# espresso3389/MioTTS-llama.cpp

Measured on AMD Instinct MI355X. Metric: realtime factor (audio s / wall s) + stage ms llm/codec/istft, 1.7B Q4_K_M, higher is better.
Workload: dtype int8-dot (q4_K/q6_K x q8_K) + f32/f16 codec; 1 GPU; MioTTS-1.7B Q4_K_M single utterance, 700 speech tokens -> MioCodec -> iSTFT (28.0 s audio each) per GPU; model=MioTTS-1.7B Q4_K_M, global_batch=1, seq_len=700, parallelism=utterance-sharded x1 (no collective), devices_visible=1

## Files before the change

### miotts-llama.cpp_amd/csrc/hip/llm_attention.h

```cpp
#pragma once
#include "llm_device.h"

namespace mio {
namespace {

__device__ inline float load_resid(const float *x, int lo, int hi) {
    const int lane = threadIdx.x & 63;
    return lo + lane < hi ? x[lo + lane] : 0.0f;
}
__device__ inline float lane_value(float v, int i) {
    return __int_as_float(__builtin_amdgcn_readlane(__float_as_int(v), i));
}

template <int HD, int G, bool DG, bool WQ = false>
__device__ __forceinline__ bool attention_wg(const LlmDims &d, const float *q_norm, const float *k_norm,
                                             const float *bqkv, _Float16 *kc, _Float16 *vc, const LlmBuffers &b,
                                             int ch, int kvh, int pos, int *rdy) {
    static_assert(!WQ || MIO_ATT_MFMA, "the q|k|v wait is on the MFMA attention path");
    constexpr bool kDiag = DG;
    using C = AttCfg<HD>;
    constexpr int PER = HD / 64;
    __shared__ float qs[G][HD];
    __shared__ float knew[HD], vnew[HD];
#if MIO_ATT_MFMA
    using A = AttM<HD>;
    static_assert(C::NT == A::NT, "attention workgroup size");
    __shared__ __attribute__((aligned(16))) char img[2 * A::IMG];
    __shared__ __attribute__((aligned(16))) _Float16 qh[G][HD];
#else
    __shared__ float wres[C::NW][G][HD + 2];
#endif

    const int t0 = ch * ATT_CHUNK;
    if (t0 > pos || b.st->done) return false;
    const int lane = threadIdx.x & 63, wave = threadIdx.x >> 6;
    const float2 *rope = b.rope + (size_t)pos * (HD / 2);
    const bool owner = pos < t0 + ATT_CHUNK;
    auto head_src = [&](int hh, HeadIn<HD> &in) {
        const bool isk = hh == G;
        const size_t so = isk ? (size_t)(d.n_head + kvh) * HD : (size_t)(kvh * G + hh) * HD;
        const size_t vo = (size_t)(d.n_head + d.n_kv + kvh) * HD;
        head_load<HD, WQ ? 16 : 0>(b.qkv + so, bqkv ? bqkv + so : nullptr, isk ? k_norm : q_norm, rope, d, in,
                                   isk ? b.qkv + vo : nullptr, isk && bqkv ? bqkv + vo : nullptr);
    };
    HeadIn<HD> hin;
#if MIO_ATT_MFMA
    h8 kr[A::VI], vr[A::VI];
    if constexpr (WQ) {
        kv_issue<HD>(kc + (size_t)kvh * d.n_ctx * HD, vc + (size_t)kvh * d.n_ctx * HD, t0, pos, kr, vr);
        kv_stage<HD>(kr, vr, owner ? pos - t0 : -1, img, img + A::IMG);
        MIO_TL_MARK(b, 4);
        if (MIO_TIDX == 0)
            wait_count(b.att_cnt + kQkvOff + kQkvStride * kvh, (G + 2) * HD, b.att_cnt + kRdyFlag);
        asm volatile("s_barrier" ::: "memory");
        MIO_TL_MARK(b, 3);
        if (wave < G + (owner ? 1 : 0)) head_src(wave, hin);
    } else {
        if (wave < G + (owner ? 1 : 0)) head_src(wave, hin);
        kv_issue<HD>(kc + (size_t)kvh * d.n_ctx * HD, vc + (size_t)kvh * d.n_ctx * HD, t0, pos, kr, vr);
    }
#else
    if (wave < G + (owner ? 1 : 0)) head_src(wave, hin);
    h8 kr[C::IT], vr[C::IT];
    load_kv_rows<HD>(kc + (size_t)kvh * d.n_ctx * HD, vc + (size_t)kvh * d.n_ctx * HD, t0, pos, kr, vr);
#endif
    MIO_TRACE(b, 1);
    MIO_TL_MARK1(b);
    for (int hh = wave; hh < G + (owner ? 1 : 0); hh += C::NW) {
        const bool isk = hh == G;
        if (hh != wave) head_src(hh, hin);
        head_prep<HD>(hin, d, isk ? knew : qs[hh]);
        if (isk) {
            _Float16 *kd = kc + ((size_t)kvh * d.n_ctx + pos) * HD;
            _Float16 *vd = vc + ((size_t)kvh * d.n_ctx + pos) * HD;
#pragma unroll
            for (int i = 0; i < PER; ++i) {
                const int p = lane + 64 * i;
                const float vr16 = f16r(hin.vv[i]);
                vnew[p] = vr16;
                kd[p] = (_Float16)knew[p];
                vd[p] = (_Float16)vr16;
            }
#if MIO_ATT_MFMA
            __builtin_amdgcn_wave_barrier();
            __builtin_amdgcn_fence(__ATOMIC_SEQ_CST, "wavefront");
            kv_stage_row<HD>(knew, vnew, pos - t0, img, img + A::IMG);
#endif
        }
#if MIO_ATT_MFMA
        else {
            q_to_f16<HD>(qs[hh], qh[hh]);
        }
#endif
    }
#if MIO_ATT_MFMA
    MIO_TRACE(b, 6);
    if constexpr (!WQ) kv_stage<HD>(kr, vr, owner ? pos - t0 : -1, img, img + A::IMG);
    MIO_TRACE(b, 7);
    lds_barrier();
    MIO_TRACE(b, 2);
    MIO_TL_MARK(b, 2);
    const uint32_t gs = (uint32_t)(d.max_splits * C::REC), head0 = (uint32_t)(kvh * G) * gs;
    attend_chunk_mfma<HD, G>(qh, img, img + A::IMG, t0, pos, d.scale, b.part + head0 + (uint32_t)ch * C::REC, gs,
                             DG ? b.trace : nullptr);
#else
    lds_barrier();
    MIO_TRACE(b, 2);
    MIO_TL_MARK(b, 2);
    if (owner) {
        const int sl = threadIdx.x / C::LP, lp = lane % C::LP, r = pos - t0;
        if (sl == r % C::NS) {
            h8 kn, vn;
#pragma unroll
            for (int i = 0; i < 8; ++i) kn[i] = (_Float16)knew[lp * 8 + i], vn[i] = (_Float16)vnew[lp * 8 + i];
#pragma unroll
            for (int it = 0; it < C::IT; ++it)
                if (it == r / C::NS) kr[it] = kn, vr[it] = vn;
        }
    }
    const uint32_t gs = (uint32_t)(d.max_splits * C::REC), head0 = (uint32_t)(kvh * G) * gs;
    attend_chunk<HD, G>(qs, kr, vr, t0, pos, d.scale, wres, b.part + head0 + (uint32_t)ch * C::REC, gs,
                        DG ? b.trace : nullptr, MIO_TL_DIAGSLOT(b));
#endif
    attn_merge_last<HD, G>(b.part, head0, gs, pos / ATT_CHUNK + 1, b.att_cnt + kvh, b.att + (size_t)kvh * G * HD, -1,
                           {}, 0, rdy, (kDiag && b.tl) ? MIO_TL_SLOT(b) : nullptr);
    return true;
}

__device__ __forceinline__ void signal_two_level(int *arr, int *rdy, int r, int n) {
    if (MIO_TIDX < 64) {
        int last = 0;
        if (MIO_TIDX == 0) {
            const int sh = r & (kFfnShards - 1), n_sh = (n - sh + kFfnShards - 1) / kFfnShards;
            last = __hip_atomic_fetch_add((__attribute__((address_space(1))) int *)(arr + kFfnStride * sh), 1,
                                          __ATOMIC_RELAXED, __HIP_MEMORY_SCOPE_AGENT) == n_sh - 1;
        }
        if (__builtin_amdgcn_readfirstlane(last) && MIO_TIDX < kFfnShards)
            __hip_atomic_fetch_add((__attribute__((address_space(1))) int *)(rdy + kFfnStride * MIO_TIDX), 1,
                                   __ATOMIC_RELAXED, __HIP_MEMORY_SCOPE_AGENT);
    }
}
__device__ __forceinline__ void wait_two_level(int *rdy, int r, int n, int *flag) {
    if (MIO_TIDX == 0) wait_count(rdy + kFfnStride * (r & (kFfnShards - 1)), min(n, kFfnShards), flag);
    asm volatile("s_barrier" ::: "memory");
}

__device__ __forceinline__ float load_resid_sc1(const float *x, int lo, int hi) {
    const int lane = threadIdx.x & 63;
    return __uint_as_float(
        __builtin_amdgcn_raw_buffer_load_b32(rsrc(x, (uint32_t)hi * 4u), (uint32_t)(lo + lane) * 4u, 0, 16));
}

template <int NP, int T, int SU, bool DG, bool XS = false>
__device__ __forceinline__ void o_consumer(const LlmDims &d, const QMat &wo, const LlmBuffers &b, int ob, int no) {
    constexpr bool kDiag = DG;
    extern __shared__ __attribute__((aligned(16))) char smem[];
    const int K = wo.k;
    const Smem s = carve(smem, K);
    int lo, hi;
    wave_range(wo.rows, lo, hi, ob, no);
    const float xres = load_resid(b.x, lo, hi);
    Frag ga[Cfg<NP, SU>::U], gb[Cfg<NP, SU>::U];
    load_first<T, NP, 1, SU, MIO_SMALL_AUX>(wo, wo, lo, hi, ga, gb);
    if (MIO_TIDX == 0)
        wait_count(b.att_cnt + kRdyOff + kRdyStride * (blockIdx.x & (kRdyShards - 1)), d.n_kv, b.att_cnt + kRdyFlag);
    asm volatile("s_barrier" ::: "memory");
    MIO_TL_MARK(b, 3);
    XRegs<NP> xr;
    load_x<NP, 16>(b.att, nullptr, K, xr);
    x_after_weights(xr);
    MIO_TL_MARK1(b);
    plain_quant(xr, K, akind(T), s, MIO_TL_DIAGSLOT(b));
    MIO_TL_MARK(b, 2);
    stream_rows<T, NP, 1, SU, MIO_SMALL_AUX>(wo, wo, lo, hi, ga, gb, s.a, [&](int row, float v, float) {
        const float r = lane_value(xres, row - lo);
        if ((threadIdx.x & 63) == 0) {
            if constexpr (XS)
                st1_sc1(b.x, (uint32_t)row * 4u, v + r);
            else
                b.x[row] = v + r;
        }
    });
    if constexpr (XS) {
        asm volatile("s_waitcnt vmcnt(0)" ::: "memory");
        __syncthreads();
        MIO_TL_MARK(b, 6);
        signal_two_level(b.att_cnt + kXOff, b.att_cnt + kXRdy, ob, no);
    }
}

}
}
```

### miotts-llama.cpp_amd/csrc/hip/llm_attn_in.hip

```cpp
#include "llm_device.h"

#pragma clang fp contract(off)

namespace mio {
namespace {

template <int NP, int TQ, int TV, int SU, bool DG, bool FS>
__global__ __launch_bounds__(MT) void k_attn_in(LlmDims d, const float *norm_w, QMat wq, QMat wk, QMat wv,
                                                int g_qk, LlmBuffers b, QMat emb, int nblk) {
    constexpr bool kDiag = DG;
    const int o1 = wq.rows, o2 = wq.rows + wk.rows;
    const int GW = matvec_grid_n(d.n_wg, o2 + wv.rows);
    extern __shared__ __attribute__((aligned(16))) char smem[];
    __shared__ float rs_[MW];
    __shared__ int ri_[MW];
    const int K = d.n_embd;
    const Smem s = carve(smem, K);
    MIO_TRACE(b, 0);
    MIO_TL_BEGIN(b);
    if (blockIdx.x == 2 && MIO_TIDX < 2 * kFfnShards)
        __hip_atomic_store((__attribute__((address_space(1))) int *)(b.att_cnt + kFfnOff + kFfnStride * MIO_TIDX), 0,
                           __ATOMIC_RELAXED, __HIP_MEMORY_SCOPE_AGENT);
    int pend = 0, step = 0;
    if constexpr (FS) {
        pend = b.st->pending;
        step = b.st->step;
        if (b.st->done) return;
    }
    uint32_t dn = 0;
    if constexpr (!FS) dn = done_issue(b);
    XRegs<NP> xr;
    load_x(pend ? nullptr : b.x, norm_w, K, xr);
    x_gate();
    auto sample_prologue = [&]() -> bool {
        if constexpr (FS) {
            if (pend) {
                const SampleCfg sc = *b.cfg;
                const int tok = sample_token<MT>(b.smp, nblk, sc, step, rs_, ri_);
                embed_regs(emb, tok, K, xr);
                if (blockIdx.x == 0) {
#pragma unroll
                    for (int i = 0; i < NP; ++i) {
                        const int e = (MIO_TIDX + i * MT) * 4;
                        if (e < K) *reinterpret_cast<float4 *>(b.x + e) = xr.v[i];
                    }
                    if (MIO_TIDX == 0) {
                        if (step < sc.max_steps) sc.out_tokens[step] = tok;
                        if (tok == sc.eos0 || tok == sc.eos1) b.st->done = 1, signal_host_done(sc);
                        b.st->token = tok;
                    }
                }
                return tok == sc.eos0 || tok == sc.eos1;
            }
        }
        return false;
    };
    auto put = [&](int row, float v) {
        if ((threadIdx.x & 63) == 0) b.qkv[row] = v;
    };
    Frag ga[Cfg<NP, SU>::U], gb[Cfg<NP, SU>::U];
    int lo, hi;
    if ((int)blockIdx.x < g_qk) {
        wave_range(o2, lo, hi, blockIdx.x, g_qk);
        load_first<TQ, NP, 1, SU, MIO_SMALL_AUX>(wq, wk, lo, hi, ga, gb, o1);
        if (sample_prologue()) return;
        x_after_weights(xr);
        if (!FS && done_now(dn)) return;
        MIO_TRACE(b, 1);
        MIO_TL_MARK1(b);
        rmsnorm_quant(xr, K, d.eps, akind(TQ), s, MIO_TL_DIAGSLOT(b));
        MIO_TRACE(b, 2);
        MIO_TL_MARK(b, 2);
        stream_rows<TQ, NP, 1, SU, MIO_SMALL_AUX>(wq, wk, lo, hi, ga, gb, s.a, [&](int row, float v, float) {
            put(row, v);
        }, o1);
        MIO_TL_END(b);
        MIO_TRACE(b, 15);
    } else {
        const int bv = (int)blockIdx.x - g_qk, gv = GW - g_qk;
        wave_range(wv.rows, lo, hi, bv, gv);
        load_first<TV, NP, 1, SU, MIO_SMALL_AUX>(wv, wv, lo, hi, ga, gb);
        if (sample_prologue()) return;
        x_after_weights(xr);
        if (!FS && done_now(dn)) return;
        rmsnorm_quant(xr, K, d.eps, akind(TV), s, MIO_TL_DIAGSLOT(b));
        stream_rows<TV, NP, 1, SU, MIO_SMALL_AUX>(wv, wv, lo, hi, ga, gb, s.a, [&](int row, float v, float) {
            put(o2 + row, v);
        });
        MIO_TL_END(b);
    }
}

template <bool DG>
void launch(const LlmDims &d, const LayerW &L, int il, const QMat &tok_embd, const LlmBuffers &b, hipStream_t s) {
    int GW, g_qk;
    attn_in_grid(d, L, GW, g_qk);
    const size_t lds = matvec_lds(d.n_embd);
    const int np = pick_np(d.n_embd);
    const int un = std::max(max_wave_units(L.wq.rows + L.wk.rows, g_qk, np, 1),
                            max_wave_units(L.wv.rows, GW - g_qk, np, 1));
    const int nblk = lm_head_blocks(d);
    const int grid = GW;
    dispatch_nt(d.n_embd, L.wq.type, [&]<int NP, int TQ>() {
        auto go = [&]<int TV>() {
            dispatch_su<NP>(pick_su(un, NP), [&]<int SU>() {
                if (il == 0)
                    hipLaunchKernelGGL((k_attn_in<NP, TQ, TV, SU, DG, true>), dim3(grid), dim3(MT), lds, s, d,
                                       L.attn_norm, L.wq, L.wk, L.wv, g_qk, b, tok_embd, nblk);
                else
                    hipLaunchKernelGGL((k_attn_in<NP, TQ, TV, SU, DG, false>), dim3(grid), dim3(MT), lds, s, d,
                                       L.attn_norm, L.wq, L.wk, L.wv, g_qk, b, tok_embd, nblk);
            });
        };
        dispatch_v<TQ>(L.wv.type, go);
    });
}

}

void launch_attn_in(const LlmDims &d, const LayerW &L, int il, const QMat &tok_embd, const LlmBuffers &b, bool dg,
                    hipStream_t s) {
    if (dg)
        launch<true>(d, L, il, tok_embd, b, s);
    else
        launch<false>(d, L, il, tok_embd, b, s);
}

}
```

### miotts-llama.cpp_amd/csrc/hip/llm_device.h

```cpp
#pragma once

#include <cfloat>
#include <climits>
#include <cstdio>
#include <cstdlib>
#include <type_traits>

#include "llm_kernels.h"

#pragma clang fp contract(off)

#ifndef MIO_TIDX
#define MIO_TIDX threadIdx.x
#endif

namespace mio {
namespace {
constexpr bool kDiag = true;
#define MIO_TRACE(bufs, k)                                                                    \
    do {                                                                                      \
        if (kDiag && (bufs).trace && blockIdx.x == 0 && blockIdx.y == 0 && MIO_TIDX == 0) { \
            asm volatile("" ::: "memory");                                                    \
            (bufs).trace[k] = __builtin_readcyclecounter();                                   \
            if ((k) == 0 || (k) == 15) (bufs).trace[16 + (k)] = __builtin_amdgcn_s_memrealtime(); \
        }                                                                                     \
    } while (0)

#define MIO_TL_SLOT(bufs) ((bufs).tl + 8 * ((size_t)(bufs).seq * kTlSlots + ((blockIdx.x + blockIdx.y * gridDim.x) & (kTlSlots - 1))))
#define MIO_TL_AT(bufs, k)                                                                      \
    do {                                                                                        \
        if (kDiag && (bufs).tl && MIO_TIDX == 0) MIO_TL_SLOT(bufs)[k] = __builtin_amdgcn_s_memrealtime(); \
    } while (0)
#ifdef MIO_TL_DIAG
#define MIO_TL_BEGIN(bufs)                                                                     \
    do {                                                                                       \
        MIO_TL_AT(bufs, 0);                                                                    \
        if (kDiag && (bufs).tl && MIO_TIDX == blockDim.x - 64) MIO_TL_SLOT(bufs)[6] = __builtin_amdgcn_s_memrealtime(); \
    } while (0)
#else
#define MIO_TL_BEGIN(bufs) MIO_TL_AT(bufs, 0)
#endif
#ifdef MIO_TL_WAVES
#define MIO_TL_MARK(bufs, k)
#define MIO_TL_END(bufs)
#else
#define MIO_TL_MARK(bufs, k) MIO_TL_AT(bufs, k)
#define MIO_TL_END(bufs) MIO_TL_AT(bufs, 7)
#endif
#ifndef MIO_DIAG_WAVE
#define MIO_DIAG_WAVE 7
#endif
#ifdef MIO_TL_DIAG
#define MIO_TL_DIAGSLOT(bufs) ((kDiag && (bufs).tl) ? MIO_TL_SLOT(bufs) : nullptr)
#define MIO_TL_MARK1(bufs)
#else
#define MIO_TL_DIAGSLOT(bufs) nullptr
#define MIO_TL_MARK1(bufs) MIO_TL_MARK(bufs, 1)
#endif
#ifdef MIO_TL_WAVES
#define MIO_DIAG_STAMP(diag, k, v)
#else
#define MIO_DIAG_STAMP(diag, k, v)                                                   \
    do {                                                                             \
        if ((diag) && MIO_TIDX == 0) {                                            \
            asm volatile("" ::"v"(v));                                               \
            (diag)[k] = __builtin_amdgcn_s_memrealtime();                            \
        }                                                                            \
    } while (0)
#endif

constexpr int NT = 256;
constexpr int NWAVE = NT / 64;
constexpr int MT = 512;
constexpr int MW = MT / 64;
constexpr int ATT_CHUNK = kAttChunk;
__host__ __device__ constexpr int part_rec(int hd) { return hd + 4; }

__device__ __forceinline__ float h2f(uint32_t bits16) {
    const uint16_t b = (uint16_t)bits16;
    return (float)__builtin_bit_cast(_Float16, b);
}
__device__ __forceinline__ float f16r(float f) { return (float)(_Float16)f; }
__device__ __forceinline__ int sdot4(int a, int b, int c) { return __builtin_amdgcn_sdot4(a, b, c, false); }
__device__ __forceinline__ uint4 ld16(const uint8_t *p) { return *reinterpret_cast<const uint4 *>(p); }
typedef uint32_t u32x4 __attribute__((ext_vector_type(4)));

__device__ __forceinline__ void lds_barrier() { asm volatile("s_waitcnt lgkmcnt(0)\n\ts_barrier" ::: "memory"); }

template <int CTRL, int RM = 0xF>
__device__ __forceinline__ int dpp_i(int v) {
    return __builtin_amdgcn_update_dpp(0, v, CTRL, RM, 0xF, false);
}
template <int CTRL, int RM = 0xF>
__device__ __forceinline__ float dpp_f(float v) {
    return __int_as_float(__builtin_amdgcn_update_dpp(0, __float_as_int(v), CTRL, RM, 0xF, false));
}
constexpr int ROW_SHR1 = 0x111, ROW_SHR2 = 0x112, ROW_SHR4 = 0x114, ROW_SHR8 = 0x118;
constexpr int ROW_BCAST15 = 0x142, ROW_BCAST31 = 0x143;

__device__ __forceinline__ float wave_max_f(float v, float id) {
    v = fmaxf(v, __int_as_float(__builtin_amdgcn_update_dpp(__float_as_int(id), __float_as_int(v), ROW_SHR1, 0xF, 0xF, false)));
    v = fmaxf(v, __int_as_float(__builtin_amdgcn_update_dpp(__float_as_int(id), __float_as_int(v), ROW_SHR2, 0xF, 0xF, false)));
    v = fmaxf(v, __int_as_float(__builtin_amdgcn_update_dpp(__float_as_int(id), __float_as_int(v), ROW_SHR4, 0xF, 0xF, false)));
    v = fmaxf(v, __int_as_float(__builtin_amdgcn_update_dpp(__float_as_int(id), __float_as_int(v), ROW_SHR8, 0xF, 0xF, false)));
    v = fmaxf(v, __int_as_float(__builtin_amdgcn_update_dpp(__float_as_int(id), __float_as_int(v), ROW_BCAST15, 0xA, 0xF, false)));
    v = fmaxf(v, __int_as_float(__builtin_amdgcn_update_dpp(__float_as_int(id), __float_as_int(v), ROW_BCAST31, 0xC, 0xF, false)));
    return __int_as_float(__builtin_amdgcn_readlane(__float_as_int(v), 63));
}
__device__ __forceinline__ int wave_min_i(int v) {
    const int id = INT_MAX;
    v = min(v, __builtin_amdgcn_update_dpp(id, v, ROW_SHR1, 0xF, 0xF, false));
    v = min(v, __builtin_amdgcn_update_dpp(id, v, ROW_SHR2, 0xF, 0xF, false));
    v = min(v, __builtin_amdgcn_update_dpp(id, v, ROW_SHR4, 0xF, 0xF, false));
    v = min(v, __builtin_amdgcn_update_dpp(id, v, ROW_SHR8, 0xF, 0xF, false));
    v = min(v, __builtin_amdgcn_update_dpp(id, v, ROW_BCAST15, 0xA, 0xF, false));
    v = min(v, __builtin_amdgcn_update_dpp(id, v, ROW_BCAST31, 0xC, 0xF, false));
    return __builtin_amdgcn_readlane(v, 63);
}
template <int CTRL, int RM = 0xF>
__device__ __forceinline__ double dpp_d(double v) {
    const int2 p = __builtin_bit_cast(int2, v);
    int2 r;
    r.x = __builtin_amdgcn_update_dpp(0, p.x, CTRL, RM, 0xF, false);
    r.y = __builtin_amdgcn_update_dpp(0, p.y, CTRL, RM, 0xF, false);
    return __builtin_bit_cast(double, r);
}
__device__ __forceinline__ double wave_sum_d(double v) {
    v += dpp_d<ROW_SHR1>(v);
    v += dpp_d<ROW_SHR2>(v);
    v += dpp_d<ROW_SHR4>(v);
    v += dpp_d<ROW_SHR8>(v);
    v += dpp_d<ROW_BCAST15, 0xA>(v);
    v += dpp_d<ROW_BCAST31, 0xC>(v);
    const int2 p = __builtin_bit_cast(int2, v);
    int2 r;
    r.x = __builtin_amdgcn_readlane(p.x, 63);
    r.y = __builtin_amdgcn_readlane(p.y, 63);
    return __builtin_bit_cast(double, r);
}
__device__ __forceinline__ float group8_max(float v) {
    v = fmaxf(v, dpp_f<0xB1>(v));
    v = fmaxf(v, dpp_f<0x4E>(v));
    v = fmaxf(v, dpp_f<0x141>(v));
    return v;
}
__device__ __forceinline__ int quad_sum_i(int v) {
    v += dpp_i<0xB1>(v);
    v += dpp_i<0x4E>(v);
    return v;
}

struct ActL {
    int8_t *qs;
    float *d;
    int16_t *bs;
};

struct Smem {
    ActL a;
    double *red;
};

__host__ __device__ inline size_t smem_bytes(int K) {
    return (size_t)K * 2 + (size_t)(K / 32 + 8) * 4 + (size_t)(K / 16 + 8) * 2 + 128;
}

__device__ inline Smem carve(char *base, int K) {
    Smem s;
    s.a.qs = (int8_t *)base;
    s.a.d = (float *)(base + (size_t)K * 2);
    s.a.bs = (int16_t *)(base + (size_t)K * 2 + (size_t)(K / 32 + 8) * 4);
    s.red = (double *)(base + smem_bytes(K) - 128);
    return s;
}

__host__ __device__ inline size_t act_bytes(int K) {
    return ((size_t)K + (size_t)(K / 32 + 8) * 4 + (size_t)(K / 16 + 8) * 2 + 15) & ~(size_t)15;
}
__host__ __device__ inline size_t act_base(int) { return 0; }
__device__ inline Smem carve_t(char *base, int K, int t) {
    Smem s;
    s.red = nullptr;
    char *a = base + act_base(K) + act_bytes(K) * t;
    s.a.qs = (int8_t *)a;
    s.a.d = (float *)(a + K);
    s.a.bs = (int16_t *)(a + K + (size_t)(K / 32 + 8) * 4);
    return s;
}

__device__ double block_sum(double v, double *red) {
    v = wave_sum_d(v);
    if ((MIO_TIDX & 63) == 0) red[MIO_TIDX >> 6] = v;
    lds_barrier();
    double t = 0.0;
#pragma unroll
    for (int w = 0; w < MW; ++w) t += red[w];
    return t;
}

__device__ __forceinline__ void q8k_store(const float (&v)[4], float am, int b, const ActL &a) {
    const int lane = MIO_TIDX & 63;
    int q[4] = {0, 0, 0, 0};
    float dd = 0.0f;
    if (am > 0.0f) {
        float sel = 0.0f;
        bool has = false;
#pragma unroll
        for (int i = 3; i >= 0; --i)
            if (fabsf(v[i]) == am) sel = v[i], has = true;
        const int src = __builtin_ctzll(__ballot(has));
        const float mx = __int_as_float(__builtin_amdgcn_readlane(__float_as_int(sel), src));
        const float iscale = -127.f / mx;
#pragma unroll
        for (int i = 0; i < 4; ++i) {
            const int t = (int)rintf(iscale * v[i]);
            q[i] = t < 127 ? t : 127;
        }
        dd = 1.0f / iscale;
    }
    const int packed = (q[0] & 0xFF) | ((q[1] & 0xFF) << 8) | ((q[2] & 0xFF) << 16) | ((q[3] & 0xFF) << 24);
    *reinterpret_cast<int *>(a.qs + b * 256 + 4 * lane) = packed;
    const int sm = quad_sum_i(q[0] + q[1] + q[2] + q[3]);
    if ((lane & 3) == 0) a.bs[b * 16 + (lane >> 2)] = (int16_t)sm;
    if (lane == 0) a.d[b] = dd;
}
__device__ __forceinline__ float abs_max4(const float (&v)[4]) {
    return wave_max_f(fmaxf(fmaxf(fabsf(v[0]), fabsf(v[1])), fmaxf(fabsf(v[2]), fabsf(v[3]))), 0.0f);
}

__device__ __forceinline__ void q80_store(const float (&v)[4], int b, bool ok, const ActL &a) {
    const int lane = MIO_TIDX & 63;
    float am = 0.0f;
#pragma unroll
    for (int i = 0; i < 4; ++i) am = fmaxf(am, fabsf(v[i]));
    am = group8_max(am);
    const float dd = am / 127.0f;
    const float id = dd != 0.0f ? 1.0f / dd : 0.0f;
    int q[4];
#pragma unroll
    for (int i = 0; i < 4; ++i) q[i] = (int)roundf(v[i] * id);
    if (ok) {
        *reinterpret_cast<int *>(a.qs + b * 32 + 4 * (lane & 7)) =
            (q[0] & 0xFF) | ((q[1] & 0xFF) << 8) | ((q[2] & 0xFF) << 16) | ((q[3] & 0xFF) << 24);
        if ((lane & 7) == 0) a.d[b] = f16r(dd);
    }
}

#ifndef MIO_X_FIRST
#define MIO_X_FIRST 0
#endif
__device__ __forceinline__ void x_gate() {
#if MIO_X_FIRST == 1
    asm volatile("s_waitcnt vmcnt(0)" ::: "memory");
#elif MIO_X_FIRST == 2
    asm volatile("s_barrier" ::: "memory");
#endif
}

template <int XV>
struct XRegs {
    float4 v[XV];
    float4 w[XV];
};

template <int XV>
__device__ __forceinline__ void x_after_weights(XRegs<XV> &xr) {
#pragma unroll
    for (int i = 0; i < XV; ++i)
        asm volatile("" : "+v"(xr.v[i].x), "+v"(xr.v[i].y), "+v"(xr.v[i].z), "+v"(xr.v[i].w), "+v"(xr.w[i].x),
                     "+v"(xr.w[i].y), "+v"(xr.w[i].z), "+v"(xr.w[i].w));
}

template <int XV, int XAUX = 0>
__device__ inline void load_x(const float *x, const float *w, int K, XRegs<XV> &xr) {
    const auto rx = __builtin_amdgcn_make_buffer_rsrc(const_cast<float *>(x), 0, x ? K * 4 : 0, 0x00020000);
    const auto rw = __builtin_amdgcn_make_buffer_rsrc(const_cast<float *>(w), 0, w ? K * 4 : 0, 0x00020000);
#pragma unroll
    for (int i = 0; i < XV; ++i) {
        const int e = (MIO_TIDX + i * MT) * 4;
        const u32x4 a = __builtin_amdgcn_raw_buffer_load_b128(rx, e * 4, 0, XAUX);
        const u32x4 c = __builtin_amdgcn_raw_buffer_load_b128(rw, e * 4, 0, 0);
        xr.v[i] = make_float4(__uint_as_float(a.x), __uint_as_float(a.y), __uint_as_float(a.z), __uint_as_float(a.w));
        xr.w[i] = make_float4(__uint_as_float(c.x), __uint_as_float(c.y), __uint_as_float(c.z), __uint_as_float(c.w));
    }
}

__host__ __device__ constexpr int akind(int T) { return T == 30 ? 2 : (T == 8 ? 0 : 1); }

__device__ __forceinline__ uint32_t f32_to_bf16(float f) {
    const uint32_t u = __float_as_uint(f);
    if ((u & 0x7fffffffu) > 0x7f800000u) return (u >> 16) | 64u;
    return (u + (0x7fffu + ((u >> 16) & 1u))) >> 16;
}

template <int XV>
__device__ __forceinline__ void quant_regs(const float4 (&v)[XV], int K, int ak, const ActL &a) {
    const int lane = MIO_TIDX & 63, wave = __builtin_amdgcn_readfirstlane(MIO_TIDX >> 6);
    if (ak == 1) {
        const int nsb = K >> 8;
#pragma unroll
        for (int j = 0; j < XV; ++j) {
            const int b = wave + MW * j;
            if (b >= nsb) break;
            const float vv[4] = {v[j].x, v[j].y, v[j].z, v[j].w};
            q8k_store(vv, abs_max4(vv), b, a);
        }
    } else if (ak == 2) {
#pragma unroll
        for (int j = 0; j < XV; ++j) {
            const int e = (MIO_TIDX + j * MT) * 4;
            if (e < K)
                *reinterpret_cast<uint2 *>(a.qs + 2 * e) =
                    make_uint2(f32_to_bf16(v[j].x) | (f32_to_bf16(v[j].y) << 16),
                               f32_to_bf16(v[j].z) | (f32_to_bf16(v[j].w) << 16));
        }
    } else {
        const int nb = K / 32;
#pragma unroll
        for (int j = 0; j < XV; ++j) {
            const int b = wave * 8 + MW * 8 * j + (lane >> 3);
            const float vv[4] = {v[j].x, v[j].y, v[j].z, v[j].w};
            q80_store(vv, b, b < nb, a);
        }
    }
    lds_barrier();
}

__device__ __forceinline__ float rms_scale(double tot, int K, float eps) {
    const float mean = (float)((K & (K - 1)) == 0 ? tot * (1.0 / K) : tot / K);
    return 1.0f / sqrtf(mean + eps);
}

template <int XV>
__device__ void rmsnorm_quant(const XRegs<XV> &xr, int K, float eps, int kquant, const Smem &s,
                              unsigned long long *diag = nullptr) {
    double acc = 0.0;
#pragma unroll
    for (int i = 0; i < XV; ++i) {
        const int e = (MIO_TIDX + i * MT) * 4;
        if (e < K) {
            const float4 v = xr.v[i];
            acc += (double)(v.x * v.x);
            acc += (double)(v.y * v.y);
            acc += (double)(v.z * v.z);
            acc += (double)(v.w * v.w);
        }
    }
#ifdef MIO_TL_WAVES
    if (diag && (MIO_TIDX & 63) == 0 && MIO_TIDX > 0) {
        asm volatile("" ::"v"(acc));
        diag[MIO_TIDX >> 6] = __builtin_amdgcn_s_memrealtime();
    }
    if (diag && MIO_TIDX == 0) {
        asm volatile("" ::"v"(acc));
        diag[0] = __builtin_amdgcn_s_memrealtime() - 0;
    }
#else
    MIO_DIAG_STAMP(diag, 3, acc);
    if (diag && MIO_TIDX == MIO_DIAG_WAVE * 64) {
        asm volatile("" ::"v"(acc));
        diag[1] = __builtin_amdgcn_s_memrealtime();
    }
#endif
    const double tot = block_sum(acc, s.red);
    MIO_DIAG_STAMP(diag, 4, tot);
    const float scale = rms_scale(tot, K, eps);
    float4 y[XV];
#pragma unroll
    for (int i = 0; i < XV; ++i) {
        const float4 v = xr.v[i], ww = xr.w[i];
        float t;
        t = v.x * scale, y[i].x = t * ww.x;
        t = v.y * scale, y[i].y = t * ww.y;
        t = v.z * scale, y[i].z = t * ww.z;
        t = v.w * scale, y[i].w = t * ww.w;
    }
    MIO_DIAG_STAMP(diag, 5, scale);
    quant_regs<XV>(y, K, kquant, s.a);
}

template <int XV>
__device__ inline void plain_quant(const XRegs<XV> &xr, int K, int kquant, const Smem &s,
                                   unsigned long long *diag = nullptr) {
    MIO_DIAG_STAMP(diag, 5, 0);
    quant_regs<XV>(xr.v, K, kquant, s.a);
}

struct ConvPrev {
    const float *p;
    int bcx;
};
template <int XV>
struct ConvRegs {
    float4 b[XV], c[XV], x[XV], p1[XV], p2[XV], w[XV][3];
};
__device__ __forceinline__ float4 ld4(const float *p) { return *reinterpret_cast<const float4 *>(p); }
__device__ __forceinline__ float4 mul4(float4 a, float4 b) {
    return make_float4(a.x * b.x, a.y * b.y, a.z * b.z, a.w * b.w);
}
__device__ __forceinline__ float4 conv_prev4(const ConvPrev &pv, int K, int e) {
    if (!pv.p) return make_float4(0.f, 0.f, 0.f, 0.f);
    if (!pv.bcx) return ld4(pv.p + e);
    return mul4(ld4(pv.p + e), ld4(pv.p + 2 * K + e));
}
template <int XV>
__device__ inline void conv_load(const float *bcx, const ConvPrev &p1, const ConvPrev &p2, const float *conv_w, int K,
                                 ConvRegs<XV> &r) {
#pragma unroll
    for (int i = 0; i < XV; ++i) {
        const int e = (MIO_TIDX + i * MT) * 4;
        if (e < K) {
            r.b[i] = ld4(bcx + e), r.c[i] = ld4(bcx + K + e), r.x[i] = ld4(bcx + 2 * K + e);
            r.p1[i] = conv_prev4(p1, K, e), r.p2[i] = conv_prev4(p2, K, e);
#pragma unroll
            for (int j = 0; j < 3; ++j) r.w[i][j] = ld4(conv_w + (size_t)e * kConvL + 4 * j);
        }
    }
}
template <int XV>
__device__ inline void conv_quant(const ConvRegs<XV> &r, int K, int kquant, const Smem &s, float *bx_out,
                                  unsigned long long *diag = nullptr) {
    float4 y[XV];
#pragma unroll
    for (int i = 0; i < XV; ++i) {
        const int e = (MIO_TIDX + i * MT) * 4;
        y[i] = make_float4(0.f, 0.f, 0.f, 0.f);
        if (e < K) {
            const float4 bx = mul4(r.b[i], r.x[i]);
            const float v2[4] = {r.p2[i].x, r.p2[i].y, r.p2[i].z, r.p2[i].w};
            const float v1[4] = {r.p1[i].x, r.p1[i].y, r.p1[i].z, r.p1[i].w};
            const float v0[4] = {bx.x, bx.y, bx.z, bx.w};
            const float c[4] = {r.c[i].x, r.c[i].y, r.c[i].z, r.c[i].w};
            const float w[12] = {r.w[i][0].x, r.w[i][0].y, r.w[i][0].z, r.w[i][0].w, r.w[i][1].x, r.w[i][1].y,
                                 r.w[i][1].z, r.w[i][1].w, r.w[i][2].x, r.w[i][2].y, r.w[i][2].z, r.w[i][2].w};
            float o[4];
#pragma unroll
            for (int j = 0; j < 4; ++j) {
                float acc = 0.0f;
                acc = acc + v2[j] * w[j * 3 + 0];
                acc = acc + v1[j] * w[j * 3 + 1];
                acc = acc + v0[j] * w[j * 3 + 2];
                o[j] = c[j] * acc;
            }
            y[i] = make_float4(o[0], o[1], o[2], o[3]);
            if (bx_out) *reinterpret_cast<float4 *>(bx_out + e) = bx;
        }
    }
    MIO_DIAG_STAMP(diag, 5, 0);
    quant_regs<XV>(y, K, kquant, s.a);
}
template <int XV>
__device__ __forceinline__ void conv_after_weights(ConvRegs<XV> &r) {
#pragma unroll
    for (int i = 0; i < XV; ++i) {
        asm volatile("" : "+v"(r.b[i].x), "+v"(r.b[i].y), "+v"(r.b[i].z), "+v"(r.b[i].w));
        asm volatile("" : "+v"(r.x[i].x), "+v"(r.x[i].y), "+v"(r.x[i].z), "+v"(r.x[i].w));
    }
}

__device__ __forceinline__ int sum8_i(int v) {
    v += dpp_i<ROW_SHR1>(v);
    v += dpp_i<ROW_SHR2>(v);
    v += dpp_i<ROW_SHR4>(v);
    return v;
}
__device__ __forceinline__ float sum8_f(float v) {
    v += dpp_f<ROW_SHR1>(v);
    v += dpp_f<ROW_SHR2>(v);
    v += dpp_f<ROW_SHR4>(v);
    return v;
}
__device__ __forceinline__ float sum_lanes7(float v) {
    v += dpp_f<ROW_SHR8>(v);
    v += dpp_f<ROW_BCAST15, 0xA>(v);
    v += dpp_f<ROW_BCAST31, 0xC>(v);
    return __int_as_float(__builtin_amdgcn_readlane(__float_as_int(v), 63));
}

__device__ inline float wave_sum(float v) {
#pragma unroll
    for (int o = 32; o >= 1; o >>= 1) v += __shfl_xor(v, o);
    return v;
}

constexpr uint32_t M4 = 0x0F0F0F0Fu, M2 = 0x03030303u;

struct Frag {
    uint4 a, b;
    uint32_t c, e;
    uint4 a2, b2;
};

struct ALane {
    int4 lo, hi;
    int b0, b1;
    float d;
    int4 lo2, hi2;
};

__device__ __forceinline__ __amdgpu_buffer_rsrc_t rsrc(const void *p, uint32_t bytes) {
    return __builtin_amdgcn_make_buffer_rsrc(const_cast<void *>(p), 0, (int)min(bytes, 0x7FFFFFF0u), 0x00020000);
}
#ifndef MIO_WEIGHT_AUX
#define MIO_WEIGHT_AUX 2
#endif
#ifndef MIO_LM_AUX
#define MIO_LM_AUX MIO_WEIGHT_AUX
#endif
#ifndef MIO_SMALL_AUX
#define MIO_SMALL_AUX MIO_WEIGHT_AUX
#endif
template <int AUX = MIO_WEIGHT_AUX>
__device__ __forceinline__ uint4 bld16(const uint8_t *base, uint32_t bytes, uint32_t voff, uint32_t soff) {
    const u32x4 v = __builtin_amdgcn_raw_buffer_load_b128(rsrc(base, bytes), voff, soff, AUX);
    return make_uint4(v.x, v.y, v.z, v.w);
}
template <int AUX = MIO_WEIGHT_AUX>
__device__ __forceinline__ uint32_t bld4(const uint8_t *base, uint32_t bytes, uint32_t voff, uint32_t soff) {
    return __builtin_amdgcn_raw_buffer_load_b32(rsrc(base, bytes), voff, soff, AUX);
}
template <int AUX = MIO_WEIGHT_AUX>
__device__ __forceinline__ uint32_t bld2(const uint8_t *base, uint32_t bytes, uint32_t voff, uint32_t soff) {
    return __builtin_amdgcn_raw_buffer_load_b16(rsrc(base, bytes), voff, soff, AUX);
}

template <int T, int AUX = MIO_WEIGHT_AUX>
__device__ __forceinline__ Frag load_frag(const QMat W, int row, int pass) {
    const int lane = MIO_TIDX & 63;
    const uint32_t R = (uint32_t)W.rows,
                   r = (uint32_t)__builtin_amdgcn_readfirstlane(min(max(row, 0), W.rows - 1));
    Frag f;
    if constexpr (T == 12) {
        const int nsb = W.k >> 8, sb = min(pass * 8 + (lane >> 3), nsb - 1), pc = lane & 7;
        const uint32_t qb = (uint32_t)(W.k / 2), hb = (uint32_t)nsb * 16;
        f.a = bld16<AUX>(W.p0, R * qb, sb * 128 + pc * 16, r * qb);
        f.c = bld4<AUX>(W.p1, R * hb, sb * 16 + 4 * (pc & 3), r * hb);
        f.b = make_uint4(0, 0, 0, 0);
        f.e = 0;
    } else if constexpr (T == 13) {
        const int nsb = W.k >> 8, sb = min(pass * 8 + (lane >> 3), nsb - 1), pc = lane & 7;
        const uint32_t qb = (uint32_t)(W.k / 2), fb = (uint32_t)(W.k / 8), hb = (uint32_t)nsb * 16;
        f.a = bld16<AUX>(W.p0, R * qb, sb * 128 + pc * 16, r * qb);
        f.b = bld16<AUX>(W.p1, R * fb, sb * 32 + 16 * (pc & 1), r * fb);
        f.c = bld4<AUX>(W.p2, R * hb, sb * 16 + 4 * (pc & 3), r * hb);
        f.e = 0;
    } else if constexpr (T == 14) {
        const int nsb = W.k >> 8, sb = min(pass * 8 + (lane >> 3), nsb - 1), pc = lane & 7;
        const uint32_t lb = (uint32_t)(W.k / 2), hb = (uint32_t)(W.k / 4), sbb = (uint32_t)(W.k / 16),
                       db = (uint32_t)nsb * 2;
        f.a = bld16<AUX>(W.p0, R * lb, sb * 128 + pc * 16, r * lb);
        f.b = bld16<AUX>(W.p1, R * hb, sb * 64 + 32 * (pc >> 2) + 16 * (pc & 1), r * hb);
        f.c = bld2<AUX>(W.p2, R * sbb, sb * 16 + 2 * pc, r * sbb);
        f.e = bld2<AUX>(W.p3, R * db, sb * 2, r * db);
    } else if constexpr (T == 30) {
        const uint32_t rb = (uint32_t)W.k * 2;
        auto off = [&](int i) { return (uint32_t)min(pass * 2048 + 512 * i + 8 * lane, W.k - 8) * 2u; };
        f.a = bld16<AUX>(W.p0, R * rb, off(0), r * rb);
        f.b = bld16<AUX>(W.p0, R * rb, off(1), r * rb);
        f.a2 = bld16<AUX>(W.p0, R * rb, off(2), r * rb);
        f.b2 = bld16<AUX>(W.p0, R * rb, off(3), r * rb);
        f.c = 0;
        f.e = 0;
    } else {
        const int nb = W.k >> 5, b = min(pass * 64 + lane, nb - 1);
        const uint32_t qb = (uint32_t)W.k, db = (uint32_t)nb * 2;
        f.a = bld16<AUX>(W.p0, R * qb, 32 * b, r * qb);
        f.b = bld16<AUX>(W.p0, R * qb, 32 * b + 16, r * qb);
        f.c = 0;
        f.e = bld2<AUX>(W.p1, R * db, 2 * b, r * db);
    }
    return f;
}

template <int T>
__device__ __forceinline__ ALane load_alane(const ActL &a, int K, int pass) {
    const int lane = MIO_TIDX & 63;
    ALane r;
    if constexpr (T == 12 || T == 13 || T == 14) {
        const int nsb = K >> 8, sb = pass * 8 + (lane >> 3), pc = lane & 7;
        const int sbc = sb < nsb ? sb : 0;
        int e, e2;
        if constexpr (T == 12 || T == 13) {
            e = sbc * 256 + 64 * (pc >> 1) + 16 * (pc & 1);
            e2 = e + 32;
        } else {
            const int n = pc >> 2, qq = pc & 3;
            e = sbc * 256 + 128 * n + 32 * (qq >> 1) + 16 * (qq & 1);
            e2 = e + 64;
        }
        r.lo = *reinterpret_cast<const int4 *>(a.qs + e);
        r.hi = *reinterpret_cast<const int4 *>(a.qs + e2);
        r.b0 = a.bs[e >> 4];
        r.b1 = a.bs[e2 >> 4];
        r.d = a.d[sbc];
    } else if constexpr (T == 30) {
        auto at = [&](int i) {
            const int e = min(pass * 2048 + 512 * i + 8 * lane, K - 8);
            return *reinterpret_cast<const int4 *>(a.qs + 2 * e);
        };
        r.lo = at(0), r.hi = at(1), r.lo2 = at(2), r.hi2 = at(3);
        r.b0 = r.b1 = 0;
        r.d = 0.0f;
    } else {
        const int nb = K >> 5, b = pass * 64 + lane, bc = b < nb ? b : 0;
        r.lo = *reinterpret_cast<const int4 *>(a.qs + 32 * bc);
        r.hi = *reinterpret_cast<const int4 *>(a.qs + 32 * bc + 16);
        r.b0 = r.b1 = 0;
        r.d = a.d[bc];
    }
    return r;
}

template <int T>
__device__ __forceinline__ float dot_frag(const Frag &f, const ALane &al, int K, int pass) {
    const int lane = MIO_TIDX & 63;
    if constexpr (T == 12 || T == 13) {
        const int jj = (lane & 7) >> 1;
        uint4 h;
        h.x = (uint32_t)dpp_i<0x00>((int)f.c);
        h.y = (uint32_t)dpp_i<0x55>((int)f.c);
        h.z = (uint32_t)dpp_i<0xAA>((int)f.c);
        h.w = (uint32_t)dpp_i<0xFF>((int)f.c);
        const uint32_t wlo = jj < 2 ? h.y : (jj == 2 ? h.z : h.w);
        const uint32_t whi = jj < 2 ? h.z : h.w;
        const uint32_t F = __builtin_amdgcn_alignbit(whi, wlo, (24 * jj) & 31);
        const int sc0 = F & 63, m0 = (F >> 6) & 63, sc1 = (F >> 12) & 63, m1 = (F >> 18) & 63;
        auto lo = [&](uint32_t q, uint32_t h) {
            if constexpr (T == 13) return (int)((q & M4) | (((h >> (2 * jj)) & 0x01010101u) << 4));
            else return (int)(q & M4);
        };
        auto hi = [&](uint32_t q, uint32_t h) {
            if constexpr (T == 13) return (int)(((q >> 4) & M4) | (((h >> (2 * jj + 1)) & 0x01010101u) << 4));
            else return (int)((q >> 4) & M4);
        };
        int dlo = 0, dhi = 0;
        dlo = sdot4(lo(f.a.x, f.b.x), al.lo.x, dlo);
        dlo = sdot4(lo(f.a.y, f.b.y), al.lo.y, dlo);
        dlo = sdot4(lo(f.a.z, f.b.z), al.lo.z, dlo);
        dlo = sdot4(lo(f.a.w, f.b.w), al.lo.w, dlo);
        dhi = sdot4(hi(f.a.x, f.b.x), al.hi.x, dhi);
        dhi = sdot4(hi(f.a.y, f.b.y), al.hi.y, dhi);
        dhi = sdot4(hi(f.a.z, f.b.z), al.hi.z, dhi);
        dhi = sdot4(hi(f.a.w, f.b.w), al.hi.w, dhi);
        int isum = __mul24(sc0, dlo) + __mul24(sc1, dhi);
        int imin = __mul24(m0, al.b0) + __mul24(m1, al.b1);
        isum = sum8_i(isum);
        imin = sum8_i(imin);
        const float d = h2f(h.x & 0xFFFF) * al.d;
        const float dmin = h2f(h.x >> 16) * al.d;
        float v = d * (float)isum;
        v = v - dmin * (float)imin;
        return pass * 8 + (lane >> 3) < (K >> 8) ? v : 0.0f;
    } else if constexpr (T == 14) {
        const int shl = 2 * ((lane & 3) >> 1);
        auto lo = [&](uint32_t l, uint32_t h) { return (int)((l & M4) | ((h << (4 - shl)) & 0x30303030u)); };
        auto hi = [&](uint32_t l, uint32_t h) { return (int)(((l >> 4) & M4) | ((h >> shl) & 0x30303030u)); };
        int dlo = 0, dhi = 0;
        dlo = sdot4(lo(f.a.x, f.b.x), al.lo.x, dlo);
        dlo = sdot4(lo(f.a.y, f.b.y), al.lo.y, dlo);
        dlo = sdot4(lo(f.a.z, f.b.z), al.lo.z, dlo);
        dlo = sdot4(lo(f.a.w, f.b.w), al.lo.w, dlo);
        dhi = sdot4(hi(f.a.x, f.b.x), al.hi.x, dhi);
        dhi = sdot4(hi(f.a.y, f.b.y), al.hi.y, dhi);
        dhi = sdot4(hi(f.a.z, f.b.z), al.hi.z, dhi);
        dhi = sdot4(hi(f.a.w, f.b.w), al.hi.w, dhi);
        const int sa = (int)(int8_t)(f.c & 0xFF), sb = (int)(int8_t)(f.c >> 8);
        int isum = __mul24(sa, dlo - 32 * al.b0) + __mul24(sb, dhi - 32 * al.b1);
        isum = sum8_i(isum);
        const float d = h2f(f.e) * al.d;
        const float v = d * (float)isum;
        return pass * 8 + (lane >> 3) < (K >> 8) ? v : 0.0f;
    } else if constexpr (T == 30) {
        typedef __bf16 bf2 __attribute__((ext_vector_type(2)));
        float acc = 0.0f;
        auto dot8 = [&](const uint4 &w, const int4 &x, int i) {
            const bool ok = pass * 2048 + 512 * i + 8 * lane < K;
            const uint4 ww = ok ? w : make_uint4(0, 0, 0, 0);
            const uint4 xx = ok ? make_uint4((uint32_t)x.x, (uint32_t)x.y, (uint32_t)x.z, (uint32_t)x.w)
                                : make_uint4(0, 0, 0, 0);
            acc = __builtin_amdgcn_fdot2_f32_bf16(__builtin_bit_cast(bf2, ww.x), __builtin_bit_cast(bf2, xx.x), acc, false);
            acc = __builtin_amdgcn_fdot2_f32_bf16(__builtin_bit_cast(bf2, ww.y), __builtin_bit_cast(bf2, xx.y), acc, false);
            acc = __builtin_amdgcn_fdot2_f32_bf16(__builtin_bit_cast(bf2, ww.z), __builtin_bit_cast(bf2, xx.z), acc, false);
            acc = __builtin_amdgcn_fdot2_f32_bf16(__builtin_bit_cast(bf2, ww.w), __builtin_bit_cast(bf2, xx.w), acc, false);
        };
        dot8(f.a, al.lo, 0);
        dot8(f.b, al.hi, 1);
        dot8(f.a2, al.lo2, 2);
        dot8(f.b2, al.hi2, 3);
        return acc;
    } else {
        int s = 0;
        s = sdot4((int)f.a.x, al.lo.x, s);
        s = sdot4((int)f.a.y, al.lo.y, s);
        s = sdot4((int)f.a.z, al.lo.z, s);
        s = sdot4((int)f.a.w, al.lo.w, s);
        s = sdot4((int)f.b.x, al.hi.x, s);
        s = sdot4((int)f.b.y, al.hi.y, s);
        s = sdot4((int)f.b.z, al.hi.z, s);
        s = sdot4((int)f.b.w, al.hi.w, s);
        const float v = (float)s * (h2f(f.e) * al.d);
        return pass * 64 + lane < (K >> 5) ? v : 0.0f;
    }
}

template <int T>
__device__ __forceinline__ float row_total(float acc) {
    if constexpr (T == 8 || T == 30) acc = sum8_f(acc);
    return sum_lanes7(acc);
}

template <int NP, int SU = 0>
struct Cfg {
    static constexpr int U = SU ? SU : (NP == 1 ? 4 : 3);
    static constexpr int NG = SU ? 1 : 2;
    static constexpr bool AREG = NP <= 3;
};

template <int T, int NP, int NM, int SU = 0, int AUX = MIO_WEIGHT_AUX>
__device__ __forceinline__ void load_group(const QMat W0, const QMat W1, int lo, int n, int u0,
                                           Frag (&f)[Cfg<NP, SU>::U], int split = INT_MAX) {
#pragma unroll
    for (int j = 0; j < Cfg<NP, SU>::U; ++j) {
        const int u = __builtin_amdgcn_readfirstlane(max(0, min(u0 + j, n - 1)));
        const int p = u % NP, m = (u / NP) % NM, i = u / (NP * NM);
        if constexpr (NM == 1) {
            const int r = __builtin_amdgcn_readfirstlane(lo + i);
            f[j] = load_frag<T, AUX>(r >= split ? W1 : W0, r >= split ? r - split : r, p);
        } else {
            f[j] = load_frag<T, AUX>(m ? W1 : W0, lo + i, p);
        }
    }
}

template <int T, int NP, int NM, int SU = 0, int AUX = MIO_WEIGHT_AUX, class Epi>
__device__ __forceinline__ void stream_rows(const QMat W0, const QMat W1, int lo, int hi, Frag (&A)[Cfg<NP, SU>::U],
                                            Frag (&B)[Cfg<NP, SU>::U], const ActL &a, Epi &&epi, int split = INT_MAX,
                                            unsigned long long *trace = nullptr) {
    constexpr int U = Cfg<NP, SU>::U;
    const int K = W0.k;
    const int n = (hi - lo) * NM * NP;
    if (n <= 0) return;
    ALane al[Cfg<NP, SU>::AREG ? NP : 1];
    if constexpr (Cfg<NP, SU>::AREG) {
#pragma unroll
        for (int p = 0; p < NP; ++p) al[p] = load_alane<T>(a, K, p);
    }
    float acc = 0.0f, g = 0.0f;
    auto consume = [&](const Frag (&F)[U], int u0) {
#pragma unroll
        for (int j = 0; j < U; ++j) {
            const int u = u0 + j;
            if (u < n) {
                int p;
                ALane av;
                if constexpr (NP == 1) {
                    p = 0;
                    av = al[0];
                } else if constexpr (NP == U) {
                    p = j;
                    av = al[j];
                } else {
                    p = u % NP;
                    av = load_alane<T>(a, K, p);
                }
                acc += dot_frag<T>(F[j], av, K, p);
                if (p == NP - 1) {
                    const float v = row_total<T>(acc);
                    acc = 0.0f;
                    const int i = u / (NP * NM);
                    if constexpr (NM == 1) {
                        epi(lo + i, v, 0.0f);
                    } else {
                        if ((u / NP) % NM == 0)
                            g = v;
                        else
                            epi(lo + i, g, v);
                    }
                }
            }
        }
    };
    for (int u0 = 0;;) {
        consume(A, u0);
        if (trace && u0 == 0 && blockIdx.x == 0 && MIO_TIDX == 0) trace[3] = __builtin_readcyclecounter();
        if constexpr (Cfg<NP, SU>::NG == 1) break;
        u0 += U;
        if (u0 >= n) break;
        load_group<T, NP, NM, SU, AUX>(W0, W1, lo, n, u0 + U, A, split);
        consume(B, u0);
        u0 += U;
        if (u0 >= n) break;
        load_group<T, NP, NM, SU, AUX>(W0, W1, lo, n, u0 + U, B, split);
    }
}

template <int T, int NP, int NM, int SU = 0, int AUX = MIO_WEIGHT_AUX>
__device__ __forceinline__ void load_first(const QMat W0, const QMat W1, int lo, int hi, Frag (&A)[Cfg<NP, SU>::U],
                                           Frag (&B)[Cfg<NP, SU>::U], int split = INT_MAX) {
    const int n = (hi - lo) * NM * NP;
    load_group<T, NP, NM, SU, AUX>(W0, W1, lo, n, 0, A, split);
    if constexpr (Cfg<NP, SU>::NG == 2) load_group<T, NP, NM, SU, AUX>(W0, W1, lo, n, Cfg<NP, SU>::U, B, split);
}

__device__ inline void wave_range(int R, int &lo, int &hi, int b, int G) {
    const int w = __builtin_amdgcn_readfirstlane(MIO_TIDX >> 6);
    const int ra = (R * b) / G, rb = (R * (b + 1)) / G;
    lo = ra + (rb - ra) * w / MW;
    hi = ra + (rb - ra) * (w + 1) / MW;
}
__device__ inline void wave_range_n(int R, int &lo, int &hi, int b, int G, int w0, int NW) {
    const int w = __builtin_amdgcn_readfirstlane(MIO_TIDX >> 6) - w0;
    const int ra = (R * b) / G, rb = (R * (b + 1)) / G;
    if (w < 0 || w >= NW) {
        lo = hi = ra;
        return;
    }
    lo = ra + (rb - ra) * w / NW;
    hi = ra + (rb - ra) * (w + 1) / NW;
}
__device__ inline void wave_range(const LlmDims &d, int R, int &lo, int &hi) {
    wave_range(R, lo, hi, blockIdx.x, matvec_grid_n(d.n_wg, R));
}


__device__ float dequant_elem(const QMat &W, int row, int e) {
    if (W.type == 12 || W.type == 13) {
        const int nsb = W.k >> 8, sb = e >> 8, c = e & 255, j = c >> 6, w = c & 63, hi = w >> 5, l = w & 31;
        const uint8_t q = W.p0[(size_t)row * (W.k / 2) + sb * 128 + 32 * j + l];
        const uint8_t *hd = (W.type == 13 ? W.p2 : W.p1) + ((size_t)row * nsb + sb) * 16;
        const uint32_t F = (uint32_t)hd[4 + 3 * j] | ((uint32_t)hd[5 + 3 * j] << 8) | ((uint32_t)hd[6 + 3 * j] << 16);
        const int sc = (F >> (12 * hi)) & 63, m = (F >> (12 * hi + 6)) & 63;
        const float d1 = h2f(hd[0] | (hd[1] << 8)) * sc, m1 = h2f(hd[2] | (hd[3] << 8)) * m;
        int code = hi ? (q >> 4) : (q & 0xF);
        if (W.type == 13) code += ((W.p1[(size_t)row * (W.k / 8) + sb * 32 + l] >> (2 * j + hi)) & 1) << 4;
        return d1 * (float)code - m1;
    } else if (W.type == 14) {
        const int nsb = W.k >> 8, sb = e >> 8, c = e & 255, n = c >> 7, w = c & 127, g = w >> 5, l = w & 31;
        const uint8_t ql = W.p0[(size_t)row * (W.k / 2) + sb * 128 + 64 * n + l + 32 * (g & 1)];
        const uint8_t qh = W.p1[(size_t)row * (W.k / 4) + sb * 64 + 32 * n + l];
        const int q = (int)((g < 2 ? (ql & 0xF) : (ql >> 4)) | (((qh >> (2 * g)) & 3) << 4)) - 32;
        const int is = c >> 4, sn = is >> 3, sw = is & 7;
        const int sc = ((const int8_t *)W.p2)[(size_t)row * (W.k / 16) + sb * 16 + 2 * (4 * sn + (sw & 3)) + (sw >> 2)];
        const float dd = h2f(((const uint16_t *)W.p3)[(size_t)row * nsb + sb]);
        return dd * (float)sc * (float)q;
    } else if (W.type == 30) {
        const uint16_t h = ((const uint16_t *)W.p0)[(size_t)row * W.k + e];
        return __uint_as_float((uint32_t)h << 16);
    } else {
        const int nb = W.k >> 5;
        const int8_t q = ((const int8_t *)W.p0)[(size_t)row * W.k + e];
        return (float)q * h2f(((const uint16_t *)W.p1)[(size_t)row * nb + (e >> 5)]);
    }
}

constexpr int ST = 1024;

__device__ inline void embed_row(const QMat &emb, int tok, int n, float *x) {
    float v[4];
#pragma unroll
    for (int i = 0; i < 4; ++i) {
        const int e = MIO_TIDX + i * ST;
        v[i] = e < n ? dequant_elem(emb, tok, e) : 0.0f;
    }
#pragma unroll
    for (int i = 0; i < 4; ++i) {
        const int e = MIO_TIDX + i * ST;
        if (e < n) x[e] = v[i];
    }
}


inline void attn_in_grid(const LlmDims &d, const LayerW &L, int &G, int &g_qk) {
    const int rows = L.wq.rows + L.wk.rows + L.wv.rows, qk = L.wq.rows + L.wk.rows;
    G = matvec_grid(d, rows);
    g_qk = (G * qk + rows / 2) / rows;
    g_qk = g_qk < 1 ? 1 : (g_qk > G - 1 ? G - 1 : g_qk);
}


template <int LP>
__device__ __forceinline__ float group_sum(float v) {
    v += dpp_f<0xB1>(v);
    v += dpp_f<0x4E>(v);
    v += dpp_f<0x141>(v);
    if constexpr (LP == 16) v += dpp_f<0x140>(v);
    return v;
}

__device__ inline float silu_f(float x) { return x / (1.0f + expf(-x)); }

__device__ inline uint64_t mix64(uint64_t x) {
    x += 0x9E3779B97F4A7C15ull;
    x = (x ^ (x >> 30)) * 0xBF58476D1CE4E5B9ull;
    x = (x ^ (x >> 27)) * 0x94D049BB133111EBull;
    return x ^ (x >> 31);
}

__device__ inline float gumbel(uint64_t seed, int step, int idx) {
    const uint64_t h = mix64(seed ^ mix64(((uint64_t)(uint32_t)step << 32) | (uint32_t)idx));
    const float u = fminf(((float)(h >> 40) + 0.5f) * (1.0f / 16777216.0f), 0x1.fffffep-1f);
    return -logf(-logf(u));
}



__device__ __forceinline__ int cur_pos(const StepState *st, const LlmDims &d) {
    return min(st->pos + st->pending, d.n_ctx - 1);
}

template <class B>
__device__ __forceinline__ uint32_t done_issue(const B &b) {
    return __builtin_amdgcn_raw_buffer_load_b32(rsrc(&b.st->done, 4), 0, 0, 0);
}
__device__ __forceinline__ bool done_now(uint32_t v) { return __builtin_amdgcn_readfirstlane(v) != 0; }
__device__ __forceinline__ void signal_host_done(const SampleCfg &sc) {
    if (sc.host_done) __hip_atomic_store(sc.host_done, 1, __ATOMIC_RELAXED, __HIP_MEMORY_SCOPE_SYSTEM);
}

template <int NTH>
__device__ int sample_token(const float *smp, int nblk, const SampleCfg &sc, int step, float *rs, int *ri) {
    const int tid = MIO_TIDX, lane = tid & 63, wave = tid >> 6;
    float best = -INFINITY;
    int bi = INT_MAX;
    const bool forced = sc.force && step < sc.n_force;
    const int ft = forced ? sc.force[step] : -1;
    for (int i = tid; i < nblk; i += NTH) {
        const float v = smp[2 * i];
        const int ix = __float_as_int(smp[2 * i + 1]);
        if (v > best || (v == best && ix < bi)) best = v, bi = ix;
    }
#pragma unroll
    for (int o = 32; o >= 1; o >>= 1) {
        const float v = __shfl_xor(best, o);
        const int ix = __shfl_xor(bi, o);
        if (v > best || (v == best && ix < bi)) best = v, bi = ix;
    }
    if (lane == 0) rs[wave] = best, ri[wave] = bi;
    lds_barrier();
    best = rs[0], bi = ri[0];
    for (int w = 1; w < NTH / 64; ++w)
        if (rs[w] > best || (rs[w] == best && ri[w] < bi)) best = rs[w], bi = ri[w];
    int tok = bi == INT_MAX ? sc.lo : bi;
    if (ft >= 0) tok = ft;
    return tok;
}

template <int XV>
__device__ inline void embed_regs(const QMat &emb, int tok, int K, XRegs<XV> &xr) {
#pragma unroll
    for (int i = 0; i < XV; ++i) {
        const int e = (MIO_TIDX + i * MT) * 4;
        float v[4] = {0.f, 0.f, 0.f, 0.f};
        if (e < K)
#pragma unroll
            for (int q = 0; q < 4; ++q) v[q] = dequant_elem(emb, tok, e + q);
        xr.v[i] = make_float4(v[0], v[1], v[2], v[3]);
    }
}

[[noreturn]] inline void no_kernel(const char *what, int type, int k) {
    fprintf(stderr, "miotts: no %s kernel for ggml type %d (%d)\n", what, type, k);
    abort();
}

template <bool BF = true, class F>
void dispatch_nt(int K, int type, F &&f) {
    const int np = pick_np(K);
#define NT_CASE(NPV, TV) \
    if (np == NPV && type == TV) return f.template operator()<NPV, TV>();
    NT_CASE(1, 8) NT_CASE(1, 12) NT_CASE(1, 13) NT_CASE(1, 14) NT_CASE(3, 8) NT_CASE(3, 12) NT_CASE(3, 13)
    NT_CASE(3, 14) NT_CASE(6, 8) NT_CASE(6, 12) NT_CASE(6, 13) NT_CASE(6, 14)
    if constexpr (BF) {
        NT_CASE(1, 30) NT_CASE(3, 30) NT_CASE(6, 30)
    }
#undef NT_CASE
    no_kernel("matvec", type, K);
}

template <int TQ, class F>
void dispatch_v(int tv, F &&f) {
    if (tv == TQ) return f.template operator()<TQ>();
    if constexpr (TQ == 12 || TQ == 13) {
        if (tv == 14) return f.template operator()<14>();
    }
    if constexpr (TQ == 14) {
        if (tv == 12) return f.template operator()<12>();
    }
    no_kernel("attn_v beside q|k", tv, TQ);
}


typedef _Float16 h8 __attribute__((ext_vector_type(8)));

#ifndef MIO_ATT_NT
#define MIO_ATT_NT 256
#endif
template <int HD>
struct AttCfg {
    static constexpr int LP = HD / 8;
    static constexpr int NT = ATT_CHUNK * LP < MIO_ATT_NT ? ATT_CHUNK * LP : MIO_ATT_NT;
    static constexpr int NW = NT / 64;
    static constexpr int NS = NT / LP;
    static constexpr int IT = ATT_CHUNK / NS;
    static constexpr int REC = part_rec(HD);
};

__device__ __forceinline__ void st1_sc1(float *base, uint32_t off, float v) {
    __builtin_amdgcn_raw_buffer_store_b32(__float_as_uint(v), rsrc(base, 0x7FFFFFF0u), off, 0, 16);
}
__device__ __forceinline__ void st4_sc1(float *base, uint32_t off, float4 v) {
    u32x4 u;
    u.x = __float_as_uint(v.x), u.y = __float_as_uint(v.y), u.z = __float_as_uint(v.z), u.w = __float_as_uint(v.w);
    __builtin_amdgcn_raw_buffer_store_b128(u, rsrc(base, 0x7FFFFFF0u), off, 0, 16);
}
__device__ __forceinline__ void wait_count(int *c, int target, int *flag) {
    auto *p = (__attribute__((address_space(1))) int *)c;
    auto *f = (__attribute__((address_space(1))) int *)flag;
    for (int it = 0; it < (1 << 16); ++it) {
        if (__hip_atomic_load(p, __ATOMIC_RELAXED, __HIP_MEMORY_SCOPE_AGENT) >= target) return;
        if ((it & 1023) == 1023 && __hip_atomic_load(f, __ATOMIC_RELAXED, __HIP_MEMORY_SCOPE_AGENT)) return;
        __builtin_amdgcn_s_sleep(1);
    }
    __hip_atomic_store(f, 1, __ATOMIC_RELAXED, __HIP_MEMORY_SCOPE_AGENT);
}
__device__ __forceinline__ float4 ld4_sc1(const float *base, uint32_t off) {
    const u32x4 v = __builtin_amdgcn_raw_buffer_load_b128(rsrc(base, 0x7FFFFFF0u), off, 0, 16);
    return make_float4(__uint_as_float(v.x), __uint_as_float(v.y), __uint_as_float(v.z), __uint_as_float(v.w));
}
__device__ __forceinline__ float2 ld2_sc1(const float *base, uint32_t off) {
    const auto v = __builtin_amdgcn_raw_buffer_load_b64(rsrc(base, 0x7FFFFFF0u), off, 0, 16);
    return make_float2(__uint_as_float(v[0]), __uint_as_float(v[1]));
}

__device__ __forceinline__ float4 merge_out4(const float *part, uint32_t head, int nch, int rec, int hd, int dd) {
    float M = -INFINITY, L = 0.0f;
    float4 O = make_float4(0.f, 0.f, 0.f, 0.f);
    constexpr int CB = 8;
    for (int c0 = 0; c0 < nch; c0 += CB) {
        float2 ml[CB];
        float4 oc[CB];
#pragma unroll
        for (int j = 0; j < CB; ++j) {
            const int c = c0 + j;
            if (c < nch) {
                ml[j] = ld2_sc1(part, (head + (uint32_t)(c * rec + hd)) * 4u);
                oc[j] = ld4_sc1(part, (head + (uint32_t)(c * rec + dd)) * 4u);
            } else {
                ml[j] = make_float2(-INFINITY, 0.0f);
                oc[j] = make_float4(0.f, 0.f, 0.f, 0.f);
            }
        }
        float mb = M;
#pragma unroll
        for (int j = 0; j < CB; ++j) mb = fmaxf(mb, ml[j].x);
        const float a = M == -INFINITY ? 0.0f : expf(M - mb);
        L *= a;
        O.x *= a, O.y *= a, O.z *= a, O.w *= a;
#pragma unroll
        for (int j = 0; j < CB; ++j) {
            const float w = c0 + j < nch ? expf(ml[j].x - mb) : 0.0f;
            L += w * ml[j].y;
            O.x += w * oc[j].x, O.y += w * oc[j].y, O.z += w * oc[j].z, O.w += w * oc[j].w;
        }
        M = mb;
    }
    return make_float4(O.x / L, O.y / L, O.z / L, O.w / L);
}

template <int O>
__device__ __forceinline__ float xor_lane(float v) {
    const int lane = MIO_TIDX & 63;
    if constexpr (O == 32) {
        const auto r = __builtin_amdgcn_permlane32_swap(__float_as_uint(v), __float_as_uint(v), false, false);
        return __uint_as_float(lane < 32 ? r[1] : r[0]);
    } else if constexpr (O == 16) {
        const auto r = __builtin_amdgcn_permlane16_swap(__float_as_uint(v), __float_as_uint(v), false, false);
        return __uint_as_float(((lane >> 4) & 1) == 0 ? r[1] : r[0]);
    } else {
        return __shfl_xor(v, O);
    }
}

template <int HD>
struct HeadIn {
    static constexpr int PER = HD / 64;
    float v[PER], w[PER], vv[PER];
    float2 cs[PER];
};
template <int HD, int AUX = 0>
__device__ __forceinline__ void head_load(const float *src, const float *bias, const float *nw, const float2 *rope,
                                          const LlmDims &d, HeadIn<HD> &in, const float *vsrc = nullptr,
                                          const float *vbias = nullptr) {
    constexpr int PER = HD / 64;
    const int lane = MIO_TIDX & 63;
    auto ld = [&](const float *base, int p) {
        if constexpr (AUX == 0) return base[p];
        return __uint_as_float(__builtin_amdgcn_raw_buffer_load_b32(rsrc(base, HD * 4), p * 4, 0, AUX));
    };
// ... 465 lines not shown
```

### miotts-llama.cpp_amd/csrc/hip/llm_kernels.h

```cpp
#pragma once

#include <hip/hip_runtime.h>

#include <cstdint>

namespace mio {

#ifndef MIO_ATT_CHUNK
#define MIO_ATT_CHUNK 64
#endif
constexpr int kAttChunk = MIO_ATT_CHUNK;
constexpr int kTlSlots = 2048;
static_assert(kAttChunk == 32 || kAttChunk == 64 || kAttChunk == 128, "attention chunk");

struct QMat {
    int type;
    int rows, k;
    const uint8_t *p0, *p1, *p2, *p3;
};

inline QMat qmat_rows(const QMat &q, int r0, int n) {
    size_t rb[4] = {0, 0, 0, 0};
    switch (q.type) {
        case 8: rb[0] = (size_t)q.k, rb[1] = (size_t)q.k / 32 * 2; break;
        case 12: rb[0] = (size_t)q.k / 2, rb[1] = (size_t)q.k / 256 * 16; break;
        case 13: rb[0] = (size_t)q.k / 2, rb[1] = (size_t)q.k / 8, rb[2] = (size_t)q.k / 256 * 16; break;
        case 14: rb[0] = (size_t)q.k / 2, rb[1] = (size_t)q.k / 4, rb[2] = (size_t)q.k / 16, rb[3] = (size_t)q.k / 256 * 2; break;
        default: break;
    }
    QMat v = q;
    v.rows = n;
    v.p0 = q.p0 + rb[0] * r0, v.p1 = q.p1 + rb[1] * r0, v.p2 = q.p2 + rb[2] * r0, v.p3 = q.p3 + rb[3] * r0;
    return v;
}

inline bool attn_v_supported(int tq, int tv) {
    return tv == tq || ((tq == 12 || tq == 13) && tv == 14) || (tq == 14 && tv == 12);
}

struct StepState {
    int pos;
    int step;
    int token;
    int done;
    int pending;
};

struct SampleCfg {
    float temp;
    uint32_t seed_lo, seed_hi;
    int lo, hi;
    int eos0, eos1;
    const int *force;
    int n_force;
    int *out_tokens;
    int max_steps;
    int *host_done;
    int top_k;
    float top_p, min_p;
    float repeat_penalty, frequency_penalty, presence_penalty;
    int repeat_last_n;
    int first_step;
};
constexpr int kChainHistMax = 256;

constexpr int kConvL = 3;
constexpr int kConvSlots = 4;

struct LayerW {
    const float *attn_norm, *q_norm, *k_norm, *ffn_norm;
    const float *bqkv;
    QMat wq, wk, wv, wo, gate, up, down;
    int conv;
    QMat in_proj, out_proj;
    const float *conv_w;
};

struct LlmDims {
    int n_embd, n_head, n_kv, hd, n_ff, n_vocab, n_ctx;
    float eps, scale;
    int neox, qk_norm;
    int split;
    int max_splits;
    int n_wg;
    int n_layer;
};

struct LlmBuffers {
    float *x;
    float *qkv;
    float *h;
    float *logits;
    float *part;
    float *att;
    int *att_cnt;
    float *smp;
    const float2 *rope;
    StepState *st;
    const SampleCfg *cfg;
    unsigned long long *trace;
    unsigned long long *tl;
    int seq;
    float *ring;
};

constexpr int kPrefillB = 128;
constexpr int kBatchMax = 16;

struct PrefillBuffers {
    float *x;
    float *qkv;
    float *h;
    float *part;
    float *att;
    int *att_cnt;
    const float2 *rope;
    const int *tokens;
    const int *pos;
    const int *seq;
    int pos_stride, seq_stride;
    size_t seq_kv;
    float *ring;
    size_t seq_ring;
    char *act;
    int *qcnt;
};
constexpr int kQcntFlag = 1024, kQcntInts = kQcntFlag + 64;
size_t prefill_act_bytes(int k_max);
int prefill_rec_k(int K, int type);

void launch_prefill_chunk(const LlmDims &d, const LayerW *layers, int n_layer, _Float16 *kcache,
                          _Float16 *vcache, const QMat &tok_embd, const PrefillBuffers &pb, int p0, int nt,
                          int n_chunks, hipStream_t s);

struct BatchBuffers {
    StepState *st;
    const SampleCfg *cfg;
    float *logits;
    float *smp;
};
void launch_batch_step(const LlmDims &d, const LayerW *layers, int n_layer, _Float16 *kcache, _Float16 *vcache,
                       const float *out_norm, const QMat &lm, const QMat &tok_embd, const PrefillBuffers &pb,
                       const BatchBuffers &bb, int B, bool chain, hipStream_t s);
bool batch_supported(const LlmDims &d, int B, int lm_type);
void launch_batch_embed(const LlmDims &d, const QMat &tok_embd, const PrefillBuffers &pb, const BatchBuffers &bb,
                        int B, hipStream_t s);

enum StepKind : int {
    kAttnIn = 0,
    kAttention = 1,
    kAttnOut = 2,
    kFfnIn = 3,
    kFfnDown = 4,
    kLmHead = 6,
    kSample = 7,
    kConvIn = 8,
    kConvOut = 9,
    kAttO = 10,
    kLayerAtt = 11,
    kFfn = 12,
    kLayer = 13,
    kSampleChain = 14,
    kStepKindEnd = 15,
};
struct StepCtx {
    LlmDims dims;
    const LayerW *layers;
    _Float16 *kc, *vc;
    const float *out_norm;
    QMat lm, tok;
};
struct ChainArgs {
    float *logits;
    size_t stride;
    const StepState *st;
    const SampleCfg *cfg;
    float *smp;
    int nblk;
    int *dbg;
    int keep;
};
void launch_sample_chain(const ChainArgs &a, int B, hipStream_t s);
void launch_nop(hipStream_t s);
void launch_step_kernel(StepKind which, const StepCtx &c, int il, const LlmBuffers &b, hipStream_t s);
void launch_embed_token(const LlmDims &d, const QMat &tok_embd, const LlmBuffers &b, hipStream_t s);
int lm_head_blocks(const LlmDims &d);
__host__ __device__ inline int matvec_grid_n(int n_wg, int rows) {
    int g = rows / 8;
    g = g < n_wg ? g : n_wg;
    return g < 2 ? 2 : g;
}
int matvec_grid(const LlmDims &d, int rows);
bool att_o_supported(int hd, int G);
bool layer_att_supported(const LlmDims &d, const LayerW &L);
bool ffn_fused_supported(const LlmDims &d, const LayerW &L);
void launch_layer_att(const LlmDims &d, const LayerW &L, _Float16 *kc, _Float16 *vc, const LlmBuffers &b, bool dg,
                      hipStream_t s);
bool layer_fused_supported(const LlmDims &d, const LayerW &L);
void launch_layer(const LlmDims &d, const LayerW &L, int il, _Float16 *kc, _Float16 *vc, const LlmBuffers &b,
                  bool dg, hipStream_t s);
int layer_ffn_gate();
constexpr int kRdyOff = 64, kRdyShards = 8, kRdyStride = 64;
constexpr int kRdyFlag = kRdyOff + kRdyShards * kRdyStride;
constexpr int kQkvOff = kRdyFlag + 64, kQkvStride = 64, kQkvMax = 64;
constexpr int kFfnOff = kQkvOff + kQkvStride * kQkvMax, kFfnShards = 8, kFfnStride = 64;
constexpr int kFfnRdy = kFfnOff + kFfnShards * kFfnStride;
constexpr int kXOff = kFfnRdy + kFfnShards * kFfnStride, kXRdy = kXOff + kFfnShards * kFfnStride;
constexpr int kLaySet = kXRdy + kFfnShards * kFfnStride;
constexpr int kLayOff = kLaySet;
constexpr int kAttCntInts = kLayOff + 2 * kLaySet;
int pick_np(int K);
size_t matvec_lds(int K);
int max_wave_units(int rows, int grid, int np, int nm);
int pick_su(int units, int np);
void launch_attn_in(const LlmDims &d, const LayerW &L, int il, const QMat &tok_embd, const LlmBuffers &b, bool dg,
                    hipStream_t s);
void launch_debug_matvec(const QMat &W, const float *x, float *y, int n_wg, hipStream_t s);
size_t debug_act_bytes(int K);
void launch_debug_mmq(const QMat &W, const QMat &up, int mode, const float *x, int nt, char *act, float *y,
                      hipStream_t s);

}
```

### miotts-llama.cpp_amd/csrc/hip/llm_kernels.hip

```cpp
#include "llm_attention.h"

#include <algorithm>
#include <cstdlib>

#pragma clang fp contract(off)

namespace mio {
namespace {



template <int NP, int T, int SU, bool DG>
__global__ __launch_bounds__(MT) void k_attn_out(LlmDims d, QMat wo, LlmBuffers b) {
    constexpr bool kDiag = DG;
    extern __shared__ __attribute__((aligned(16))) char smem[];
    MIO_TRACE(b, 0);
    MIO_TL_BEGIN(b);
    const int K = wo.k;
    const Smem s = carve(smem, K);
    int lo, hi;
    wave_range(d, wo.rows, lo, hi);
    const uint32_t dn = done_issue(b);
    XRegs<NP> xr;
    load_x(b.att, nullptr, K, xr);
    const float xres = load_resid(b.x, lo, hi);
    x_gate();
    Frag ga[Cfg<NP, SU>::U], gb[Cfg<NP, SU>::U];
    load_first<T, NP, 1, SU, MIO_SMALL_AUX>(wo, wo, lo, hi, ga, gb);
    x_after_weights(xr);
    if (done_now(dn)) return;
    MIO_TRACE(b, 1);
    MIO_TL_MARK1(b);
    plain_quant(xr, K, akind(T), s, MIO_TL_DIAGSLOT(b));
    MIO_TRACE(b, 2);
    MIO_TL_MARK(b, 2);
    stream_rows<T, NP, 1, SU, MIO_SMALL_AUX>(wo, wo, lo, hi, ga, gb, s.a, [&](int row, float v, float) {
        const float r = lane_value(xres, row - lo);
        if ((threadIdx.x & 63) == 0) b.x[row] = v + r;
    });
    MIO_TL_END(b);
    MIO_TRACE(b, 15);
}

template <int NP, int T, int SU, bool DG>
__global__ __launch_bounds__(MT) void k_conv_out(LlmDims d, QMat wo, const float *conv_w, float *ring, LlmBuffers b) {
    constexpr bool kDiag = DG;
    extern __shared__ __attribute__((aligned(16))) char smem[];
    MIO_TRACE(b, 0);
    MIO_TL_BEGIN(b);
    const int K = wo.k;
    const Smem s = carve(smem, K);
    const uint32_t dn = done_issue(b);
    const int pos = cur_pos(b.st, d);
    const ConvPrev p1{pos >= 1 ? ring + (size_t)((pos - 1) & (kConvSlots - 1)) * K : nullptr, 0};
    const ConvPrev p2{pos >= 2 ? ring + (size_t)((pos - 2) & (kConvSlots - 1)) * K : nullptr, 0};
    ConvRegs<NP> cr;
    conv_load(b.qkv, p1, p2, conv_w, K, cr);
    int lo, hi;
    wave_range(d, wo.rows, lo, hi);
    const float xres = load_resid(b.x, lo, hi);
    x_gate();
    Frag ga[Cfg<NP, SU>::U], gb[Cfg<NP, SU>::U];
    load_first<T, NP, 1, SU>(wo, wo, lo, hi, ga, gb);
    conv_after_weights(cr);
    if (done_now(dn)) return;
    MIO_TRACE(b, 1);
    MIO_TL_MARK1(b);
    conv_quant(cr, K, akind(T), s, blockIdx.x == 0 ? ring + (size_t)(pos & (kConvSlots - 1)) * K : nullptr,
               MIO_TL_DIAGSLOT(b));
    MIO_TRACE(b, 2);
    MIO_TL_MARK(b, 2);
    stream_rows<T, NP, 1, SU>(wo, wo, lo, hi, ga, gb, s.a, [&](int row, float v, float) {
        const float r = lane_value(xres, row - lo);
        if ((threadIdx.x & 63) == 0) b.x[row] = v + r;
    });
    MIO_TL_END(b);
    MIO_TRACE(b, 15);
}

__device__ __forceinline__ void advance_state(StepState *st, const LlmDims &d) {
    const int p = st->pending;
    st->pos = min(st->pos + p, d.n_ctx - 1);
    st->step = st->step + p;
    st->pending = 0;
}

__device__ __forceinline__ void zero_layer_sets(int *cnt) {
    constexpr int n = kRdyShards + kQkvMax + 4 * kFfnShards;
    for (int i = MIO_TIDX; i < 2 * n; i += MT) {
        const int j = i % n;
        const int o = j < kRdyShards ? kRdyOff + kRdyStride * j
                    : j < kRdyShards + kQkvMax ? kQkvOff + kQkvStride * (j - kRdyShards)
                                               : kFfnOff + kFfnStride * (j - kRdyShards - kQkvMax);
        __hip_atomic_store((__attribute__((address_space(1))) int *)(cnt + kLayOff + (i / n) * kLaySet + o), 0,
                           __ATOMIC_RELAXED, __HIP_MEMORY_SCOPE_AGENT);
    }
}

template <int NP, int T, int SU, bool DG>
__global__ __launch_bounds__(MT) void k_ffn_in(LlmDims d, const float *norm_w, QMat gate, QMat up,
                                               LlmBuffers b, int adv) {
    constexpr bool kDiag = DG;
    extern __shared__ __attribute__((aligned(16))) char smem[];
    MIO_TRACE(b, 0);
    MIO_TL_BEGIN(b);
    const int K = d.n_embd;
    const Smem s = carve(smem, K);
    const uint32_t dn = done_issue(b);
    XRegs<NP> xr;
    load_x(b.x, norm_w, K, xr);
    x_gate();
    if (blockIdx.x == 0 && MIO_TIDX < kRdyShards)
        __hip_atomic_store((__attribute__((address_space(1))) int *)(b.att_cnt + kRdyOff + kRdyStride * MIO_TIDX), 0,
                           __ATOMIC_RELAXED, __HIP_MEMORY_SCOPE_AGENT);
    if (blockIdx.x == 1 && MIO_TIDX < d.n_kv)
        __hip_atomic_store((__attribute__((address_space(1))) int *)(b.att_cnt + kQkvOff + kQkvStride * MIO_TIDX), 0,
                           __ATOMIC_RELAXED, __HIP_MEMORY_SCOPE_AGENT);
    int lo, hi;
    wave_range(d, gate.rows, lo, hi);
    Frag ga[Cfg<NP, SU>::U], gb[Cfg<NP, SU>::U];
    load_first<T, NP, 2, SU>(gate, up, lo, hi, ga, gb);
    x_after_weights(xr);
    if (done_now(dn)) {
        if (adv && blockIdx.x == 0 && MIO_TIDX == 0) advance_state(b.st, d);
        return;
    }
    MIO_TRACE(b, 1);
    MIO_TL_MARK1(b);
    rmsnorm_quant(xr, K, d.eps, akind(T), s, MIO_TL_DIAGSLOT(b));
    MIO_TRACE(b, 2);
    MIO_TL_MARK(b, 2);
    stream_rows<T, NP, 2, SU>(gate, up, lo, hi, ga, gb, s.a, [&](int row, float g, float u) {
        if ((threadIdx.x & 63) == 0) b.h[row] = silu_f(g) * u;
    }, INT_MAX, DG ? b.trace : nullptr);
    if (adv && blockIdx.x == 0 && MIO_TIDX == 0) advance_state(b.st, d);
    MIO_TL_END(b);
    MIO_TRACE(b, 15);
}

template <int NP, int T, int SU, bool DG>
__global__ __launch_bounds__(MT) void k_ffn_down(LlmDims d, QMat down, LlmBuffers b) {
    constexpr bool kDiag = DG;
    extern __shared__ __attribute__((aligned(16))) char smem[];
    MIO_TRACE(b, 0);
    MIO_TL_BEGIN(b);
    const int K = down.k;
    const Smem s = carve(smem, K);
    const uint32_t dn = done_issue(b);
    XRegs<NP> xr;
    load_x(b.h, nullptr, K, xr);
    int lo, hi;
    wave_range(d, down.rows, lo, hi);
    const float xres = load_resid(b.x, lo, hi);
    x_gate();
    Frag ga[Cfg<NP, SU>::U], gb[Cfg<NP, SU>::U];
    load_first<T, NP, 1, SU>(down, down, lo, hi, ga, gb);
    x_after_weights(xr);
    if (done_now(dn)) return;
    MIO_TRACE(b, 1);
    MIO_TL_MARK1(b);
    plain_quant(xr, K, akind(T), s, MIO_TL_DIAGSLOT(b));
    MIO_TRACE(b, 2);
    MIO_TL_MARK(b, 2);
    stream_rows<T, NP, 1, SU>(down, down, lo, hi, ga, gb, s.a, [&](int row, float v, float) {
        const float r = lane_value(xres, row - lo);
        if ((threadIdx.x & 63) == 0) b.x[row] = v + r;
    }, INT_MAX, DG ? b.trace : nullptr);
    MIO_TL_END(b);
    MIO_TRACE(b, 15);
}

template <int NP, int T, int SU, int NPD, int TD, int SUD, bool DG>
__global__ __launch_bounds__(MT) void k_ffn(LlmDims d, const float *norm_w, QMat gate, QMat up, QMat down,
                                            LlmBuffers b, int adv, int GI) {
    constexpr bool kDiag = DG;
    extern __shared__ __attribute__((aligned(16))) char smem[];
    MIO_TRACE(b, 0);
    MIO_TL_BEGIN(b);
    const uint32_t dn = done_issue(b);
    if ((int)blockIdx.x < GI) {
        const int K = d.n_embd;
        const Smem s = carve(smem, K);
        XRegs<NP> xr;
        load_x(b.x, norm_w, K, xr);
        x_gate();
        if (blockIdx.x == 0 && MIO_TIDX < kRdyShards)
            __hip_atomic_store((__attribute__((address_space(1))) int *)(b.att_cnt + kRdyOff + kRdyStride * MIO_TIDX),
                               0, __ATOMIC_RELAXED, __HIP_MEMORY_SCOPE_AGENT);
        if (blockIdx.x == 1 && MIO_TIDX < d.n_kv)
            __hip_atomic_store((__attribute__((address_space(1))) int *)(b.att_cnt + kQkvOff + kQkvStride * MIO_TIDX),
                               0, __ATOMIC_RELAXED, __HIP_MEMORY_SCOPE_AGENT);
        int lo, hi;
        wave_range(gate.rows, lo, hi, blockIdx.x, GI);
        Frag ga[Cfg<NP, SU>::U], gb[Cfg<NP, SU>::U];
        load_first<T, NP, 2, SU>(gate, up, lo, hi, ga, gb);
        x_after_weights(xr);
        if (done_now(dn)) {
            if (adv && blockIdx.x == 0 && MIO_TIDX == 0) advance_state(b.st, d);
            return;
        }
        MIO_TL_MARK1(b);
        rmsnorm_quant(xr, K, d.eps, akind(T), s, MIO_TL_DIAGSLOT(b));
        MIO_TL_MARK(b, 2);
        stream_rows<T, NP, 2, SU>(gate, up, lo, hi, ga, gb, s.a, [&](int row, float g, float u) {
            if ((threadIdx.x & 63) == 0) st1_sc1(b.h, (uint32_t)row * 4u, silu_f(g) * u);
        });
        if (adv && blockIdx.x == 0 && MIO_TIDX == 0) advance_state(b.st, d);
        asm volatile("s_waitcnt vmcnt(0)" ::: "memory");
        __syncthreads();
        if (MIO_TIDX < 64) {
            int last = 0;
            if (MIO_TIDX == 0) {
                const int sh = blockIdx.x & (kFfnShards - 1), n_sh = (GI - sh + kFfnShards - 1) / kFfnShards;
                last = __hip_atomic_fetch_add((__attribute__((address_space(1))) int *)(b.att_cnt + kFfnOff + kFfnStride * sh),
                                              1, __ATOMIC_RELAXED, __HIP_MEMORY_SCOPE_AGENT) == n_sh - 1;
            }
            if (__builtin_amdgcn_readfirstlane(last) && MIO_TIDX < kFfnShards)
                __hip_atomic_fetch_add((__attribute__((address_space(1))) int *)(b.att_cnt + kFfnRdy + kFfnStride * MIO_TIDX),
                                       1, __ATOMIC_RELAXED, __HIP_MEMORY_SCOPE_AGENT);
        }
    } else {
        const int K = down.k;
        const Smem s = carve(smem, K);
        const int GD = (int)gridDim.x - GI, ob = (int)blockIdx.x - GI;
        int lo, hi;
        wave_range(down.rows, lo, hi, ob, GD);
        const float xres = load_resid(b.x, lo, hi);
        Frag ga[Cfg<NPD, SUD>::U], gb[Cfg<NPD, SUD>::U];
        load_first<TD, NPD, 1, SUD>(down, down, lo, hi, ga, gb);
        if (done_now(dn)) return;
        if (MIO_TIDX == 0)
            wait_count(b.att_cnt + kFfnRdy + kFfnStride * (blockIdx.x & (kFfnShards - 1)), min(GI, kFfnShards),
                       b.att_cnt + kRdyFlag);
        asm volatile("s_barrier" ::: "memory");
        MIO_TL_MARK(b, 3);
        XRegs<NPD> xr;
        load_x<NPD, 16>(b.h, nullptr, K, xr);
        x_after_weights(xr);
        MIO_TL_MARK1(b);
        plain_quant(xr, K, akind(TD), s, MIO_TL_DIAGSLOT(b));
        MIO_TL_MARK(b, 2);
        stream_rows<TD, NPD, 1, SUD>(down, down, lo, hi, ga, gb, s.a, [&](int row, float v, float) {
            const float r = lane_value(xres, row - lo);
            if ((threadIdx.x & 63) == 0) b.x[row] = v + r;
        });
    }
    MIO_TL_END(b);
    MIO_TRACE(b, 15);
}

#define MIO_FFN_SHAPES(X) \
    X(1, 12, 6, 3, 12, 3)  \
    X(1, 12, 6, 3, 14, 3)  \
    X(1, 13, 6, 3, 13, 3)  \
    X(1, 13, 6, 3, 14, 3)  \
    X(1, 30, 6, 3, 30, 3)  \
    X(1, 8, 2, 1, 8, 1)    \
    X(1, 8, 0, 6, 8, 0)

struct FfnShape {
    int np, t, su, npd, td, sud, GI, GD;
};
FfnShape ffn_shape(const LlmDims &d, const LayerW &L) {
    FfnShape f{};
    f.GI = matvec_grid(d, L.gate.rows), f.GD = matvec_grid(d, L.down.rows);
    f.np = pick_np(d.n_embd), f.t = L.gate.type;
    f.su = pick_su(max_wave_units(L.gate.rows, f.GI, f.np, 2), f.np);
    f.npd = pick_np(L.down.k), f.td = L.down.type;
    f.sud = pick_su(max_wave_units(L.down.rows, f.GD, f.npd, 1), f.npd);
    return f;
}

template <bool DG>
bool launch_ffn(const LlmDims &d, const LayerW &L, const LlmBuffers &b, int adv, hipStream_t st, bool dry) {
    if (L.up.type != L.gate.type) return false;
    const FfnShape f = ffn_shape(d, L);
    const size_t lds = std::max(smem_bytes(d.n_embd), smem_bytes(L.down.k));
    bool found = false;
#define MIO_FFN_CASE(NP, T, SU, NPD, TD, SUD)                                                                     \
    if (!found && f.np == NP && f.t == T && f.su == SU && f.npd == NPD && f.td == TD && f.sud == SUD) {          \
        found = true;                                                                                            \
        if (!dry)                                                                                                \
            hipLaunchKernelGGL((k_ffn<NP, T, SU, NPD, TD, SUD, DG>), dim3(f.GI + f.GD), dim3(MT), lds, st, d,       \
                               L.ffn_norm, L.gate, L.up, L.down, b, adv, f.GI);                                  \
    }
    MIO_FFN_SHAPES(MIO_FFN_CASE)
#undef MIO_FFN_CASE
    return found;
}

template <int NP, int T, bool DG>
__global__ __launch_bounds__(MT) void k_lm_head(LlmDims d, const float *norm_w, QMat lm, LlmBuffers b) {
    constexpr bool kDiag = DG;
    extern __shared__ __attribute__((aligned(16))) char smem[];
    __shared__ float bs_[MW];
    __shared__ int bi_[MW];
    const int K = d.n_embd;
    MIO_TRACE(b, 0);
    MIO_TL_BEGIN(b);
    if (blockIdx.x == 2 && MIO_TIDX < 2 * kFfnShards)
        __hip_atomic_store((__attribute__((address_space(1))) int *)(b.att_cnt + kFfnOff + kFfnStride * MIO_TIDX), 0,
                           __ATOMIC_RELAXED, __HIP_MEMORY_SCOPE_AGENT);
    if (blockIdx.x == 3) zero_layer_sets(b.att_cnt);
    const Smem s = carve(smem, K);
    XRegs<NP> xr;
    load_x(b.x, norm_w, K, xr);
    x_gate();
    int lo, hi;
    wave_range(d, lm.rows, lo, hi);
    Frag ga[Cfg<NP>::U], gb[Cfg<NP>::U];
    load_first<T, NP, 1, 0, MIO_LM_AUX>(lm, lm, lo, hi, ga, gb);
    x_after_weights(xr);
    asm volatile("" ::: "memory");
    const SampleCfg sc = *b.cfg;
    const int step = b.st->step;
    if (b.st->done) return;
    MIO_TRACE(b, 1);
    MIO_TL_MARK1(b);
    rmsnorm_quant(xr, K, d.eps, akind(T), s, MIO_TL_DIAGSLOT(b));
    MIO_TRACE(b, 2);
    MIO_TL_MARK(b, 2);
    const int lane = threadIdx.x & 63;
    float r0 = -INFINITY, r1 = -INFINITY;
    stream_rows<T, NP, 1, 0, MIO_LM_AUX>(lm, lm, lo, hi, ga, gb, s.a, [&](int row, float v, float) {
        const int k = row - lo;
        r0 = lane == k ? v : r0;
        r1 = lane + 64 == k ? v : r1;
    });
    MIO_TRACE(b, 3);
    const uint64_t seed = ((uint64_t)sc.seed_hi << 32) | sc.seed_lo;
    float best = -INFINITY;
    int bi = INT_MAX;
#pragma unroll
    for (int h = 0; h < 2; ++h) {
        const int row = lo + lane + 64 * h;
        const float v = h ? r1 : r0;
        if (row < hi) {
            b.logits[row] = v;
            if (row >= sc.lo && row < sc.hi) {
                const float t = sc.temp > 0.0f ? v / sc.temp + gumbel(seed, step, row) : v;
                if (t > best || (t == best && row < bi)) best = t, bi = row;
            }
        }
    }
#pragma unroll
    for (int o = 32; o >= 1; o >>= 1) {
        const float ov = __shfl_xor(best, o);
        const int oi = __shfl_xor(bi, o);
        if (ov > best || (ov == best && oi < bi)) best = ov, bi = oi;
    }
    const int wave = threadIdx.x >> 6;
    if (lane == 0) bs_[wave] = best, bi_[wave] = bi;
    lds_barrier();
    if (threadIdx.x == 0) {
        for (int w = 1; w < MW; ++w)
            if (bs_[w] > best || (bs_[w] == best && bi_[w] < bi)) best = bs_[w], bi = bi_[w];
        b.smp[2 * blockIdx.x] = best;
        b.smp[2 * blockIdx.x + 1] = __int_as_float(bi);
        if (blockIdx.x == 0) b.st->pending = 1;
    }
    MIO_TL_END(b);
    MIO_TRACE(b, 15);
}

template <int HD, int G, bool DG>
__global__ __launch_bounds__(AttCfg<HD>::NT) void k_attention(LlmDims d, const float *q_norm, const float *k_norm,
                                                      const float *bqkv, _Float16 *kc, _Float16 *vc, LlmBuffers b) {
    constexpr bool kDiag = DG;
    MIO_TRACE(b, 0);
    MIO_TL_BEGIN(b);
    asm volatile("" ::"s"(kc), "s"(vc), "s"(d.n_ctx), "s"(b.qkv), "s"(b.rope), "s"(q_norm), "s"(k_norm),
                 "s"(b.part), "s"(d.max_splits), "s"(bqkv), "s"(b.att), "s"(b.att_cnt));
    const int pos = cur_pos(b.st, d);
    if (!attention_wg<HD, G, DG>(d, q_norm, k_norm, bqkv, kc, vc, b, blockIdx.x, blockIdx.y, pos, nullptr)) return;
    MIO_TL_END(b);
    MIO_TRACE(b, 15);
}

template <int HD, bool DG>
void launch_attention(int G, dim3 grid, hipStream_t s, const LlmDims &d, const LayerW &L, _Float16 *kc,
                      _Float16 *vc, const LlmBuffers &b) {
    const float *qn = L.q_norm, *kn = L.k_norm, *bi = L.bqkv;
    switch (G) {
        case 1: hipLaunchKernelGGL((k_attention<HD, 1, DG>), grid, dim3(AttCfg<HD>::NT), 0, s, d, qn, kn, bi, kc, vc, b); break;
        case 2: hipLaunchKernelGGL((k_attention<HD, 2, DG>), grid, dim3(AttCfg<HD>::NT), 0, s, d, qn, kn, bi, kc, vc, b); break;
        case 3: hipLaunchKernelGGL((k_attention<HD, 3, DG>), grid, dim3(AttCfg<HD>::NT), 0, s, d, qn, kn, bi, kc, vc, b); break;
        case 4: hipLaunchKernelGGL((k_attention<HD, 4, DG>), grid, dim3(AttCfg<HD>::NT), 0, s, d, qn, kn, bi, kc, vc, b); break;
        case 8: hipLaunchKernelGGL((k_attention<HD, 8, DG>), grid, dim3(AttCfg<HD>::NT), 0, s, d, qn, kn, bi, kc, vc, b); break;
        default: break;
    }
}

template <int HD, int G, int NP, int T, int SU, bool DG>
__global__ __launch_bounds__(MT) void k_att_o(LlmDims d, const float *q_norm, const float *k_norm, const float *bqkv,
                                              _Float16 *kc, _Float16 *vc, QMat wo, LlmBuffers b) {
    constexpr bool kDiag = DG;
    MIO_TRACE(b, 0);
    MIO_TL_BEGIN(b);
    asm volatile("" ::"s"(kc), "s"(vc), "s"(d.n_ctx), "s"(b.qkv), "s"(b.rope), "s"(q_norm), "s"(k_norm),
                 "s"(b.part), "s"(d.max_splits), "s"(bqkv), "s"(b.att), "s"(b.att_cnt));
    const int pos = cur_pos(b.st, d);
    if (b.st->done) return;
    const int bid = blockIdx.x, n_act = (pos / ATT_CHUNK + 1) * d.n_kv;
    if (bid < n_act) {
        if (MIO_TIDX >= AttCfg<HD>::NT) return;
        if (!attention_wg<HD, G, DG>(d, q_norm, k_norm, bqkv, kc, vc, b, bid / d.n_kv, bid % d.n_kv, pos,
                                     b.att_cnt + kRdyOff))
            return;
    } else {
        const int no = matvec_grid_n(d.n_wg, wo.rows), ob = bid - n_act;
        if (ob >= no) return;
        o_consumer<NP, T, SU, DG>(d, wo, b, ob, no);
    }
    MIO_TL_END(b);
    MIO_TRACE(b, 15);
}

template <int NP, int T, int SU, bool DG>
void launch_att_o(int G, int grid, size_t lds, hipStream_t s, const LlmDims &d, const LayerW &L, _Float16 *kc,
                  _Float16 *vc, const LlmBuffers &b) {
    const float *qn = L.q_norm, *kn = L.k_norm, *bi = L.bqkv;
#define MIO_ATT_O(HH, GG) \
    hipLaunchKernelGGL((k_att_o<HH, GG, NP, T, SU, DG>), dim3(grid), dim3(MT), lds, s, d, qn, kn, bi, kc, vc, L.wo, b)
    if (d.hd == 128 && G == 2) MIO_ATT_O(128, 2);
    if (d.hd == 64 && G == 3) MIO_ATT_O(64, 3);
    if (d.hd == 64 && G == 4) MIO_ATT_O(64, 4);
#undef MIO_ATT_O
}

template <bool DG>
__global__ __launch_bounds__(ST) void k_sample(LlmDims d, QMat emb, int nblk, LlmBuffers b) {
    constexpr bool kDiag = DG;
    __shared__ float rs_[ST / 64];
    __shared__ int ri_[ST / 64];
    MIO_TRACE(b, 0);
    MIO_TL_BEGIN(b);
    StepState *st = b.st;
    if (!st->pending) return;
    const SampleCfg sc = *b.cfg;
    const int step = st->step;
    const int tok = sample_token<ST>(b.smp, nblk, sc, step, rs_, ri_);
    MIO_TRACE(b, 1);
    MIO_TL_MARK1(b);
    embed_row(emb, tok, d.n_embd, b.x);
    MIO_TL_END(b);
    MIO_TRACE(b, 15);
    if (MIO_TIDX == 0) {
        if (step < sc.max_steps) sc.out_tokens[step] = tok;
        if (tok == sc.eos0 || tok == sc.eos1) st->done = 1, signal_host_done(sc);
        st->token = tok;
        st->pos = min(st->pos + 1, d.n_ctx - 1);
        st->step = step + 1;
        st->pending = 0;
    }
}

__global__ __launch_bounds__(ST) void k_embed(LlmDims d, QMat emb, LlmBuffers b) {
    embed_row(emb, b.st->token, d.n_embd, b.x);
}

}

int pick_np(int K) { return K <= 2048 ? 1 : (K <= 6144 ? 3 : 6); }

static_assert(MW == 8, "matvec_grid_n assumes 8 waves per workgroup");
bool att_o_supported(int hd, int G) { return (hd == 128 && G == 2) || (hd == 64 && (G == 3 || G == 4)); }
bool ffn_fused_supported(const LlmDims &d, const LayerW &L) {
    return launch_ffn<false>(d, L, LlmBuffers{}, 0, nullptr, true);
}

int matvec_grid(const LlmDims &d, int rows) { return matvec_grid_n(d.n_wg, rows); }

LlmDims lm_dims(const LlmDims &d) {
    static const int mult = [] {
        const char *e = getenv("MIO_LM_WGM");
        const int v = e ? atoi(e) : 2;
        return v < 1 ? 1 : (v > 4 ? 4 : v);
    }();
    LlmDims l = d;
    l.n_wg = d.n_wg * mult;
    return l;
}
int lm_head_blocks(const LlmDims &d) { const LlmDims l = lm_dims(d); return matvec_grid(l, l.n_vocab); }

size_t matvec_lds(int K) { return smem_bytes(K); }


__global__ void k_nop() {}
void launch_nop(hipStream_t s) { hipLaunchKernelGGL(k_nop, dim3(1), dim3(64), 0, s); }

void launch_embed_token(const LlmDims &d, const QMat &tok_embd, const LlmBuffers &b, hipStream_t s) {
    hipLaunchKernelGGL(k_embed, dim3(1), dim3(ST), 0, s, d, tok_embd, b);
}

inline size_t mv_lds(int K) { return smem_bytes(K); }
size_t lm_lds(int K) {
    static const size_t kb = [] {
        const char *e = getenv("MIO_LM_LDS_KB");
        return e ? (size_t)atoi(e) : (size_t)0;
    }();
    const size_t b = smem_bytes(K);
    return kb * 1024 > b ? std::min(kb * 1024, (size_t)64 * 1024) : b;
}

int max_wave_units(int rows, int grid, int np, int nm) {
    const int rg = (rows + grid - 1) / grid, rw = (rg + MW - 1) / MW;
    return rw * np * nm;
}
int pick_su(int units, int np) {
    if (np == 1 && units <= 4) return units;
    if (np == 1 && units <= 6) return 6;
    if (np == 3 && units <= 3) return 3;
    return 0;
}
void launch_step_kernel(StepKind which, const StepCtx &c, int il, const LlmBuffers &b, hipStream_t s) {
    const LlmDims &d = c.dims;
    const LayerW *layers = c.layers;
    _Float16 *kcache = c.kc, *vcache = c.vc;
    const float *out_norm = c.out_norm;
    const QMat &lm = c.lm, &tok_embd = c.tok;
    const size_t layer_kv = (size_t)d.n_kv * d.n_ctx * d.hd;
    const int G = d.n_head / d.n_kv;
    auto go_dg = [&]<bool DG>() {
    switch (which) {
        case kAttnIn: {
            launch_attn_in(d, layers[il], il, tok_embd, b, DG, s);
            break;
        }
        case kAttention: {
            const LayerW &L = layers[il];
            const dim3 grid(d.max_splits, d.n_kv);
            if (d.hd == 128)
                launch_attention<128, DG>(G, grid, s, d, L, kcache + il * layer_kv, vcache + il * layer_kv, b);
            else
                launch_attention<64, DG>(G, grid, s, d, L, kcache + il * layer_kv, vcache + il * layer_kv, b);
            break;
        }
        case kAttnOut: {
            const LayerW &L = layers[il];
            const int grid = matvec_grid(d, L.wo.rows);
            dispatch_nt(L.wo.k, L.wo.type, [&]<int NP, int T>() {
                dispatch_su<NP>(pick_su(max_wave_units(L.wo.rows, grid, NP, 1), NP), [&]<int SU>() {
                    hipLaunchKernelGGL((k_attn_out<NP, T, SU, DG>), dim3(grid), dim3(MT), mv_lds(L.wo.k), s, d, L.wo, b);
                });
            });
            break;
        }
// ... 92 lines not shown
```

### miotts-llama.cpp_amd/csrc/hip/llm_layer_att.hip

```cpp
#include "llm_attention.h"

#pragma clang fp contract(off)

namespace mio {
#if MIO_ATT_MFMA
namespace {

template <int NP, int TQ, int TV, int SU, int HD, int G, bool DG>
__device__ __forceinline__ void qkv_producer(const LlmDims &d, const float *norm_w, const QMat &wq, const QMat &wk,
                                             const QMat &wv, int g_qk, int GW, const LlmBuffers &b) {
    constexpr bool kDiag = DG;
    const int o1 = wq.rows, o2 = wq.rows + wk.rows;
    extern __shared__ __attribute__((aligned(16))) char smem[];
    const int K = d.n_embd;
    const Smem s = carve(smem, K);
    const uint32_t dn = done_issue(b);
    XRegs<NP> xr;
    load_x(b.x, norm_w, K, xr);
    x_gate();
    auto put = [&](int row, float v) {
        if ((threadIdx.x & 63) == 0) st1_sc1(b.qkv, (uint32_t)row * 4, v);
    };
    Frag ga[Cfg<NP, SU>::U], gb[Cfg<NP, SU>::U];
    int lo, hi, ra, rb;
    const int bid = blockIdx.x;
    if (bid < g_qk) {
        wave_range(o2, lo, hi, bid, g_qk);
        ra = o2 * bid / g_qk, rb = o2 * (bid + 1) / g_qk;
        load_first<TQ, NP, 1, SU, MIO_SMALL_AUX>(wq, wk, lo, hi, ga, gb, o1);
        x_after_weights(xr);
        if (done_now(dn)) return;
        MIO_TL_MARK1(b);
        rmsnorm_quant(xr, K, d.eps, akind(TQ), s, MIO_TL_DIAGSLOT(b));
        MIO_TL_MARK(b, 2);
        stream_rows<TQ, NP, 1, SU, MIO_SMALL_AUX>(wq, wk, lo, hi, ga, gb, s.a, [&](int row, float v, float) {
            put(row, v);
        }, o1);
    } else {
        const int bv = bid - g_qk, gv = GW - g_qk;
        wave_range(wv.rows, lo, hi, bv, gv);
        ra = o2 + wv.rows * bv / gv, rb = o2 + wv.rows * (bv + 1) / gv;
        load_first<TV, NP, 1, SU, MIO_SMALL_AUX>(wv, wv, lo, hi, ga, gb);
        x_after_weights(xr);
        if (done_now(dn)) return;
        MIO_TL_MARK1(b);
        rmsnorm_quant(xr, K, d.eps, akind(TV), s, MIO_TL_DIAGSLOT(b));
        MIO_TL_MARK(b, 2);
        stream_rows<TV, NP, 1, SU, MIO_SMALL_AUX>(wv, wv, lo, hi, ga, gb, s.a, [&](int row, float v, float) {
            put(o2 + row, v);
        });
    }
    asm volatile("s_waitcnt vmcnt(0)" ::: "memory");
    __syncthreads();
    if (MIO_TIDX < 64) {
        const int i = MIO_TIDX, r = ra + i;
        auto head_of = [&](int rr) { return rr < o1 ? rr / (HD * G) : (rr < o2 ? (rr - o1) / HD : (rr - o2) / HD); };
        const bool ok = r < rb;
        const int h = ok ? head_of(r) : -1;
        const bool start = ok && (i == 0 || head_of(r - 1) != h);
        const uint64_t m = __ballot(start);
        if (start) {
            const uint64_t nx = i < 63 ? m >> (i + 1) : 0;
            const int end = nx ? i + 1 + __builtin_ctzll(nx) : rb - ra;
            __hip_atomic_fetch_add((__attribute__((address_space(1))) int *)(b.att_cnt + kQkvOff + kQkvStride * h),
                                   end - i, __ATOMIC_RELAXED, __HIP_MEMORY_SCOPE_AGENT);
        }
    }
}

template <int NP, int TQ, int TV, int SU, int HD, int G, int TO, int SUO, bool DG>
__global__ __launch_bounds__(MT) void k_layer_att(LlmDims d, const float *norm_w, QMat wq, QMat wk, QMat wv, int g_qk,
                                                  int GW, const float *q_norm, const float *k_norm, const float *bqkv,
                                                  _Float16 *kc, _Float16 *vc, QMat wo, LlmBuffers b) {
    constexpr bool kDiag = DG;
    MIO_TRACE(b, 0);
    MIO_TL_BEGIN(b);
    if (blockIdx.x == 2 && MIO_TIDX < 2 * kFfnShards)
        __hip_atomic_store((__attribute__((address_space(1))) int *)(b.att_cnt + kFfnOff + kFfnStride * MIO_TIDX), 0,
                           __ATOMIC_RELAXED, __HIP_MEMORY_SCOPE_AGENT);
    const int bid = blockIdx.x;
    if (bid < GW) {
        qkv_producer<NP, TQ, TV, SU, HD, G, DG>(d, norm_w, wq, wk, wv, g_qk, GW, b);
    } else {
        asm volatile("" ::"s"(kc), "s"(vc), "s"(d.n_ctx), "s"(b.qkv), "s"(b.rope), "s"(q_norm), "s"(k_norm),
                     "s"(b.part), "s"(d.max_splits), "s"(bqkv), "s"(b.att), "s"(b.att_cnt));
        const int pos = cur_pos(b.st, d);
        if (b.st->done) return;
        const int ab = bid - GW, n_act = (pos / ATT_CHUNK + 1) * d.n_kv;
        if (ab < n_act) {
            if (MIO_TIDX >= AttCfg<HD>::NT) return;
            if (!attention_wg<HD, G, DG, true>(d, q_norm, k_norm, bqkv, kc, vc, b, ab / d.n_kv, ab % d.n_kv, pos,
                                               b.att_cnt + kRdyOff))
                return;
        } else {
            const int no = matvec_grid_n(d.n_wg, wo.rows), ob = ab - n_act;
            if (ob >= no) return;
            o_consumer<1, TO, SUO, DG>(d, wo, b, ob, no);
        }
    }
    MIO_TL_END(b);
    MIO_TRACE(b, 15);
}

template <int NP, int T, int SU, bool DG>
__device__ __forceinline__ void gate_up_role(const LlmDims &d, const float *norm_w, const QMat &gate, const QMat &up,
                                             const LlmBuffers &b, int r, int GI, int no, int fgate) {
    constexpr bool kDiag = DG;
    extern __shared__ __attribute__((aligned(16))) char smem[];
    const int K = d.n_embd;
    const Smem s = carve(smem, K);
    if (fgate == 1) {
        const int kvh = r % d.n_kv;
        if (MIO_TIDX == 0)
            wait_count(b.att_cnt + kQkvOff + kQkvStride * kvh, (d.n_head / d.n_kv + 2) * d.hd, b.att_cnt + kRdyFlag);
        asm volatile("s_barrier" ::: "memory");
    } else if (fgate == 2) {
        if (MIO_TIDX == 0)
            wait_count(b.att_cnt + kRdyOff + kRdyStride * (r & (kRdyShards - 1)), d.n_kv, b.att_cnt + kRdyFlag);
        asm volatile("s_barrier" ::: "memory");
    }
    int lo, hi;
    wave_range(gate.rows, lo, hi, r, GI);
    Frag ga[Cfg<NP, SU>::U], gb[Cfg<NP, SU>::U];
    load_first<T, NP, 2, SU>(gate, up, lo, hi, ga, gb);
    wait_two_level(b.att_cnt + kXRdy, r, no, b.att_cnt + kRdyFlag);
    MIO_TL_MARK(b, 3);
    XRegs<NP> xr;
    load_x<NP, 16>(b.x, norm_w, K, xr);
    x_after_weights(xr);
    MIO_TL_MARK1(b);
    rmsnorm_quant(xr, K, d.eps, akind(T), s, MIO_TL_DIAGSLOT(b));
    MIO_TL_MARK(b, 2);
    stream_rows<T, NP, 2, SU>(gate, up, lo, hi, ga, gb, s.a, [&](int row, float g, float u) {
        if ((threadIdx.x & 63) == 0) st1_sc1(b.h, (uint32_t)row * 4u, silu_f(g) * u);
    });
    asm volatile("s_waitcnt vmcnt(0)" ::: "memory");
    __syncthreads();
    signal_two_level(b.att_cnt + kFfnOff, b.att_cnt + kFfnRdy, r, GI);
}

template <int NP, int T, int SU, bool DG>
__device__ __forceinline__ void down_role(const LlmDims &d, const QMat &down, const LlmBuffers &b, int r, int GD,
                                          int GI, int no, int fgate) {
    constexpr bool kDiag = DG;
    extern __shared__ __attribute__((aligned(16))) char smem[];
    const int K = down.k;
    const Smem s = carve(smem, K);
    if (fgate == 1) {
        const int kvh = r % d.n_kv;
        if (MIO_TIDX == 0)
            wait_count(b.att_cnt + kQkvOff + kQkvStride * kvh, (d.n_head / d.n_kv + 2) * d.hd, b.att_cnt + kRdyFlag);
        asm volatile("s_barrier" ::: "memory");
    } else if (fgate == 2) {
        wait_two_level(b.att_cnt + kXRdy, r, no, b.att_cnt + kRdyFlag);
    }
    int lo, hi;
    wave_range(down.rows, lo, hi, r, GD);
    Frag ga[Cfg<NP, SU>::U], gb[Cfg<NP, SU>::U];
    load_first<T, NP, 1, SU>(down, down, lo, hi, ga, gb);
    wait_two_level(b.att_cnt + kFfnRdy, r, GI, b.att_cnt + kRdyFlag);
    MIO_TL_MARK(b, 3);
    const float xres = load_resid_sc1(b.x, lo, hi);
    XRegs<NP> xr;
    load_x<NP, 16>(b.h, nullptr, K, xr);
    x_after_weights(xr);
    MIO_TL_MARK1(b);
    plain_quant(xr, K, akind(T), s, MIO_TL_DIAGSLOT(b));
    MIO_TL_MARK(b, 2);
    stream_rows<T, NP, 1, SU>(down, down, lo, hi, ga, gb, s.a, [&](int row, float v, float) {
        const float rr = lane_value(xres, row - lo);
        if ((threadIdx.x & 63) == 0) b.x[row] = v + rr;
    });
}

template <int NP, int TQ, int TV, int SU, int HD, int G, int TO, int SUO, int FNP, int FT, int FSU, int FNPD, int FTD,
          int FSUD, bool DG>
__global__ __launch_bounds__(MT) void k_layer(LlmDims d, const float *norm_w, QMat wq, QMat wk, QMat wv, int g_qk,
                                              int GW, const float *q_norm, const float *k_norm, const float *bqkv,
                                              _Float16 *kc, _Float16 *vc, QMat wo, const float *ffn_norm, QMat gate,
                                              QMat up, QMat down, int GI, int GD, int *base_cnt, int *other_set,
                                              int fgate, LlmBuffers b) {
    constexpr bool kDiag = DG;
    MIO_TRACE(b, 0);
    MIO_TL_BEGIN(b);
    if (blockIdx.x == 2 && MIO_TIDX < 2 * kFfnShards)
        __hip_atomic_store((__attribute__((address_space(1))) int *)(base_cnt + kFfnOff + kFfnStride * MIO_TIDX), 0,
                           __ATOMIC_RELAXED, __HIP_MEMORY_SCOPE_AGENT);
    if (blockIdx.x == 3) {
        for (int i = MIO_TIDX; i < kRdyShards + kQkvMax + 4 * kFfnShards; i += MT) {
            const int o = i < kRdyShards ? kRdyOff + kRdyStride * i
                        : i < kRdyShards + kQkvMax ? kQkvOff + kQkvStride * (i - kRdyShards)
                                                   : kFfnOff + kFfnStride * (i - kRdyShards - kQkvMax);
            __hip_atomic_store((__attribute__((address_space(1))) int *)(other_set + o), 0, __ATOMIC_RELAXED,
                               __HIP_MEMORY_SCOPE_AGENT);
        }
    }
    const int bid = blockIdx.x;
    if (bid < GW) {
        qkv_producer<NP, TQ, TV, SU, HD, G, DG>(d, norm_w, wq, wk, wv, g_qk, GW, b);
    } else {
        asm volatile("" ::"s"(kc), "s"(vc), "s"(d.n_ctx), "s"(b.qkv), "s"(b.rope), "s"(q_norm), "s"(k_norm),
                     "s"(b.part), "s"(d.max_splits), "s"(bqkv), "s"(b.att), "s"(b.att_cnt));
        const int pos = cur_pos(b.st, d);
        if (b.st->done) return;
        const int ab = bid - GW, n_act = (pos / ATT_CHUNK + 1) * d.n_kv;
        const int no = matvec_grid_n(d.n_wg, wo.rows);
        if (ab < n_act) {
            if (MIO_TIDX >= AttCfg<HD>::NT) return;
            if (!attention_wg<HD, G, DG, true>(d, q_norm, k_norm, bqkv, kc, vc, b, ab / d.n_kv, ab % d.n_kv, pos,
                                               b.att_cnt + kRdyOff))
                return;
        } else if (ab < n_act + no) {
            o_consumer<1, TO, SUO, DG, true>(d, wo, b, ab - n_act, no);
        } else if (ab < n_act + no + GI) {
            gate_up_role<FNP, FT, FSU, DG>(d, ffn_norm, gate, up, b, ab - n_act - no, GI, no, fgate);
        } else if (ab < n_act + no + GI + GD) {
            down_role<FNPD, FTD, FSUD, DG>(d, down, b, ab - n_act - no - GI, GD, GI, no, fgate);
        } else {
            return;
        }
    }
    MIO_TL_END(b);
    MIO_TRACE(b, 15);
}

#define MIO_LAYER_ATT_SHAPES(X)   \
    X(1, 12, 12, 2, 128, 2, 12, 1) \
    X(1, 12, 14, 2, 128, 2, 12, 1) \
    X(1, 13, 13, 2, 128, 2, 13, 1) \
    X(1, 13, 14, 2, 128, 2, 13, 1) \
    X(1, 30, 30, 2, 128, 2, 30, 1) \
    X(1, 8, 8, 1, 64, 3, 8, 1)     \
    X(1, 8, 8, 2, 64, 4, 8, 1)

struct Shape {
    int np, tq, tv, su, hd, g, to, suo;
    int GW, g_qk;
};

Shape shape_of(const LlmDims &d, const LayerW &L) {
    Shape s{};
    attn_in_grid(d, L, s.GW, s.g_qk);
    s.np = pick_np(d.n_embd);
    s.tq = L.wq.type, s.tv = L.wv.type, s.to = L.wo.type;
    s.su = pick_su(std::max(max_wave_units(L.wq.rows + L.wk.rows, s.g_qk, s.np, 1),
                            max_wave_units(L.wv.rows, s.GW - s.g_qk, s.np, 1)),
                   s.np);
    s.suo = pick_su(max_wave_units(L.wo.rows, matvec_grid(d, L.wo.rows), pick_np(L.wo.k), 1), pick_np(L.wo.k));
    s.hd = d.hd, s.g = d.n_head / d.n_kv;
    if (pick_np(L.wo.k) != 1) s.suo = -1;
    return s;
}

template <bool DG>
bool launch(const LlmDims &d, const LayerW &L, _Float16 *kc, _Float16 *vc, const LlmBuffers &b, hipStream_t st,
            bool dry) {
    const Shape s = shape_of(d, L);
    const int rows = L.wq.rows + L.wk.rows + L.wv.rows;
    if ((L.wq.rows + L.wk.rows + s.g_qk - 1) / s.g_qk > 64 || (L.wv.rows + s.GW - s.g_qk - 1) / (s.GW - s.g_qk) > 64 ||
        d.n_kv > kQkvMax || rows != (d.n_head + 2 * d.n_kv) * d.hd || L.conv)
        return false;
    const int grid = s.GW + d.max_splits * d.n_kv + matvec_grid(d, L.wo.rows);
    const size_t lds = std::max(matvec_lds(d.n_embd), matvec_lds(L.wo.k));
    bool found = false;
#define MIO_LA_CASE(NP, TQ, TV, SU, HD, G, TO, SUO)                                                                   \
    if (!found && s.np == NP && s.tq == TQ && s.tv == TV && s.su == SU && s.hd == HD && s.g == G && s.to == TO &&   \
        s.suo == SUO) {                                                                                                \
        found = true;                                                                                                  \
        if (!dry)                                                                                                      \
            hipLaunchKernelGGL((k_layer_att<NP, TQ, TV, SU, HD, G, TO, SUO, DG>), dim3(grid), dim3(MT), lds, st, d,   \
                               L.attn_norm, L.wq, L.wk, L.wv, s.g_qk, s.GW, L.q_norm, L.k_norm, L.bqkv, kc, vc, L.wo, \
                               b);                                                                                     \
    }
    MIO_LAYER_ATT_SHAPES(MIO_LA_CASE)
#undef MIO_LA_CASE
    return found;
}

#define MIO_LAYER_SHAPES(X)                             \
    X(1, 12, 12, 2, 128, 2, 12, 1, 1, 12, 6, 3, 12, 3) \
    X(1, 12, 14, 2, 128, 2, 12, 1, 1, 12, 6, 3, 14, 3) \
    X(1, 12, 12, 2, 128, 2, 12, 1, 1, 12, 6, 3, 14, 3) \
    X(1, 12, 14, 2, 128, 2, 12, 1, 1, 12, 6, 3, 12, 3)

template <bool DG>
bool launch_whole(const LlmDims &d, const LayerW &L, int il, _Float16 *kc, _Float16 *vc, const LlmBuffers &b,
                  hipStream_t st, bool dry) {
    const Shape s = shape_of(d, L);
    const int rows = L.wq.rows + L.wk.rows + L.wv.rows;
    if ((L.wq.rows + L.wk.rows + s.g_qk - 1) / s.g_qk > 64 || (L.wv.rows + s.GW - s.g_qk - 1) / (s.GW - s.g_qk) > 64 ||
        d.n_kv > kQkvMax || rows != (d.n_head + 2 * d.n_kv) * d.hd || L.conv || L.up.type != L.gate.type)
        return false;
    const int GI = matvec_grid(d, L.gate.rows), GD = matvec_grid(d, L.down.rows);
    const int fnp = pick_np(d.n_embd), fsu = pick_su(max_wave_units(L.gate.rows, GI, fnp, 2), fnp);
    const int fnpd = pick_np(L.down.k), fsud = pick_su(max_wave_units(L.down.rows, GD, fnpd, 1), fnpd);
    const int grid = s.GW + d.max_splits * d.n_kv + matvec_grid(d, L.wo.rows) + GI + GD;
    const size_t lds = std::max({matvec_lds(d.n_embd), matvec_lds(L.wo.k), matvec_lds(L.down.k)});
    LlmBuffers lb = b;
    int *base = b.att_cnt, *other = nullptr;
    if (!dry) lb.att_cnt = base + kLayOff + (il & 1) * kLaySet, other = base + kLayOff + ((il & 1) ^ 1) * kLaySet;
    const int fgate = layer_ffn_gate();
    bool found = false;
#define MIO_LY_CASE(NP, TQ, TV, SU, HD, G, TO, SUO, FNP, FT, FSU, FNPD, FTD, FSUD)                                  \
    if (!found && s.np == NP && s.tq == TQ && s.tv == TV && s.su == SU && s.hd == HD && s.g == G && s.to == TO &&   \
        s.suo == SUO && fnp == FNP && L.gate.type == FT && fsu == FSU && fnpd == FNPD && L.down.type == FTD &&      \
        fsud == FSUD) {                                                                                             \
        found = true;                                                                                               \
        if (!dry)                                                                                                   \
            hipLaunchKernelGGL((k_layer<NP, TQ, TV, SU, HD, G, TO, SUO, FNP, FT, FSU, FNPD, FTD, FSUD, DG>), dim3(grid), \
                               dim3(MT), lds, st, d, L.attn_norm, L.wq, L.wk, L.wv, s.g_qk, s.GW, L.q_norm, L.k_norm,   \
                               L.bqkv, kc, vc, L.wo, L.ffn_norm, L.gate, L.up, L.down, GI, GD, base, other, fgate, lb); \
    }
    MIO_LAYER_SHAPES(MIO_LY_CASE)
#undef MIO_LY_CASE
    return found;
}

}

int layer_ffn_gate() {
    static const int v = [] {
        const char *e = getenv("MIO_LAYER_GATE");
        return e ? atoi(e) : 0;
    }();
    return v;
}

bool layer_fused_supported(const LlmDims &d, const LayerW &L) {
    return launch_whole<false>(d, L, 0, nullptr, nullptr, LlmBuffers{}, nullptr, true);
}

void launch_layer(const LlmDims &d, const LayerW &L, int il, _Float16 *kc, _Float16 *vc, const LlmBuffers &b, bool dg,
                  hipStream_t s) {
    if (dg)
        launch_whole<true>(d, L, il, kc, vc, b, s, false);
    else
        launch_whole<false>(d, L, il, kc, vc, b, s, false);
}

bool layer_att_supported(const LlmDims &d, const LayerW &L) {
    return launch<false>(d, L, nullptr, nullptr, LlmBuffers{}, nullptr, true);
}

void launch_layer_att(const LlmDims &d, const LayerW &L, _Float16 *kc, _Float16 *vc, const LlmBuffers &b, bool dg,
                      hipStream_t s) {
    if (dg)
        launch<true>(d, L, kc, vc, b, s, false);
    else
        launch<false>(d, L, kc, vc, b, s, false);
}
#else
bool layer_att_supported(const LlmDims &, const LayerW &) { return false; }
void launch_layer_att(const LlmDims &, const LayerW &, _Float16 *, _Float16 *, const LlmBuffers &, bool, hipStream_t) {}
int layer_ffn_gate() { return 0; }
bool layer_fused_supported(const LlmDims &, const LayerW &) { return false; }
void launch_layer(const LlmDims &, const LayerW &, int, _Float16 *, _Float16 *, const LlmBuffers &, bool, hipStream_t) {}
#endif

}
```

### miotts-llama.cpp_amd/csrc/testlib/debug_capi.cpp

```cpp
#include <vector>

#include "common.h"
#include "gguf.h"
#include "llm.h"
#include "llm_kernels.h"
#include "mio_hip_test.h"
#include "quant.h"

extern "C" int mio_hip_debug_matvec(mio_hip_device *d, uint32_t type, const void *gguf_rows, int rows, int k,
                                    const float *x, float *y) {
    MIO_REQUIRE(d && gguf_rows && x && y && rows > 0 && k > 0, MIO_ERR_INVALID, "debug_matvec: bad args");
    MIO_REQUIRE(type == mio::GGML_Q8_0 || type == mio::GGML_Q4_K || type == mio::GGML_Q5_K ||
                    type == mio::GGML_Q6_K || type == mio::GGML_BF16 || mio::repacks_to_q8_0(type),
                MIO_ERR_UNSUPPORTED, "debug_matvec: type %u", type);
    const bool k32 = type == mio::GGML_Q8_0 || type == mio::GGML_BF16 || mio::repacks_to_q8_0(type);
    MIO_REQUIRE(k % (k32 ? 32 : 256) == 0, MIO_ERR_INVALID, "debug_matvec: k %d", k);
    int rc = mio::bind(d);
    if (rc) return rc;
    std::vector<uint8_t> q80;
    if (mio::repacks_to_q8_0(type)) {
        q80.resize((size_t)rows * (k / 32) * sizeof(mio::BlockQ8_0));
        mio::repack_to_q8_0(type, gguf_rows, rows, k, q80.data());
        gguf_rows = q80.data();
        type = mio::GGML_Q8_0;
    }
    const mio::SplitLayout L = mio::split_layout(type, rows, k);
    std::vector<uint8_t> host(L.bytes);
    mio::to_split(type, gguf_rows, rows, k, host.data());
    uint8_t *dw = nullptr;
    float *dx = nullptr, *dy = nullptr;
    MIO_HIP_CHECK(hipMalloc(&dw, L.bytes));
    MIO_HIP_CHECK(hipMalloc(&dx, (size_t)k * 4));
    MIO_HIP_CHECK(hipMalloc(&dy, (size_t)rows * 4));
    hipMemcpy(dw, host.data(), L.bytes, hipMemcpyHostToDevice);
    hipMemcpy(dx, x, (size_t)k * 4, hipMemcpyHostToDevice);
    mio::QMat q{(int)type, rows, k, dw + L.off[0], dw + L.off[1], dw + L.off[2], dw + L.off[3]};
    mio::launch_debug_matvec(q, dx, dy, d->n_cu > 0 ? d->n_cu : 256, d->stream);
    hipError_t e = hipStreamSynchronize(d->stream);
    if (e == hipSuccess) e = hipMemcpy(y, dy, (size_t)rows * 4, hipMemcpyDeviceToHost);
    hipFree(dw), hipFree(dx), hipFree(dy);
    MIO_HIP_CHECK(e);
    return MIO_OK;
}

extern "C" int mio_hip_debug_mmq(mio_hip_device *d, uint32_t type, const void *gguf_rows, int rows, int k,
                                 const float *x, int nt, int mode, const void *gguf_up, float *y) {
    MIO_REQUIRE(d && gguf_rows && x && y && rows > 0 && k > 0 && nt > 0 && nt <= 4096 && mode >= 0 && mode <= 2 &&
                    (mode != 2 || gguf_up),
                MIO_ERR_INVALID, "debug_mmq: bad args");
    MIO_REQUIRE(type == mio::GGML_Q8_0 || type == mio::GGML_Q4_K || type == mio::GGML_Q5_K ||
                    type == mio::GGML_Q6_K,
                MIO_ERR_UNSUPPORTED, "debug_mmq: type %u", type);
    MIO_REQUIRE(k % (type == mio::GGML_Q8_0 ? 32 : 256) == 0, MIO_ERR_INVALID, "debug_mmq: k %d", k);
    int rc = mio::bind(d);
    if (rc) return rc;
    const mio::SplitLayout L = mio::split_layout(type, rows, k);
    const int nm = mode == 2 ? 2 : 1;
    std::vector<uint8_t> host(L.bytes * nm);
    mio::to_split(type, gguf_rows, rows, k, host.data());
    if (nm == 2) mio::to_split(type, gguf_up, rows, k, host.data() + L.bytes);
    uint8_t *dw = nullptr;
    float *dx = nullptr, *dy = nullptr;
    char *da = nullptr;
    MIO_HIP_CHECK(hipMalloc(&dw, L.bytes * nm));
    MIO_HIP_CHECK(hipMalloc(&dx, (size_t)nt * k * 4));
    MIO_HIP_CHECK(hipMalloc(&dy, (size_t)nt * rows * 4));
    MIO_HIP_CHECK(hipMalloc(&da, (size_t)nt * mio::debug_act_bytes(k)));
    hipMemcpy(dw, host.data(), L.bytes * nm, hipMemcpyHostToDevice);
    hipMemcpy(dx, x, (size_t)nt * k * 4, hipMemcpyHostToDevice);
    hipMemcpy(dy, y, (size_t)nt * rows * 4, hipMemcpyHostToDevice);
    auto qm = [&](uint8_t *base) {
        return mio::QMat{(int)type, rows, k, base + L.off[0], base + L.off[1], base + L.off[2], base + L.off[3]};
    };
    const mio::QMat q = qm(dw), up = nm == 2 ? qm(dw + L.bytes) : mio::QMat{};
    mio::launch_debug_mmq(q, up, mode, dx, nt, da, dy, d->stream);
    hipError_t e = hipGetLastError();
    if (e == hipSuccess) e = hipStreamSynchronize(d->stream);
    if (e == hipSuccess) e = hipMemcpy(y, dy, (size_t)nt * rows * 4, hipMemcpyDeviceToHost);
    hipFree(dw), hipFree(dx), hipFree(dy), hipFree(da);
    MIO_HIP_CHECK(e);
    return MIO_OK;
}

extern "C" int mio_hip_llm_set_kv_rows(mio_hip_llm *m, int il, int p0, int n_pos, const uint16_t *k,
                                       const uint16_t *v) {
    return mio::llm_set_kv_rows(m, il, p0, n_pos, k, v);
}

extern "C" int mio_hip_llm_debug_attention(mio_hip_llm *m, int il, int pos, int which, const float *qkv,
                                           float *att) {
    return mio::llm_debug_attention(m, il, pos, which, qkv, att);
}

extern "C" int mio_hip_llm_debug_sample_chain(mio_hip_llm *m, const float *logits, const int32_t *history,
                                              int n_history, const mio_sampling *s, float temperature, uint64_t seed,
                                              int step, int32_t lo, int32_t hi, int32_t *token, int32_t *kept,
                                              int32_t *cut_id, float *penalised) {
    MIO_REQUIRE(m && s, MIO_ERR_INVALID, "llm_debug_sample_chain: null argument");
    int info[8];
    if (int rc = mio_hip_llm_info(m, info)) return rc;
    MIO_REQUIRE(lo >= 0 && lo < info[0] && hi <= info[0], MIO_ERR_INVALID,
                "llm_debug_sample_chain: window [%d, %d) outside the %d-id vocabulary", lo, hi, info[0]);
    mio::SamplingParams sp;
    sp.temperature = temperature, sp.seed = seed, sp.allow_lo = lo, sp.allow_hi = hi < 0 ? 0 : hi;
    sp.top_k = s->top_k, sp.top_p = s->top_p, sp.min_p = s->min_p, sp.repeat_penalty = s->repeat_penalty;
    sp.frequency_penalty = s->frequency_penalty, sp.presence_penalty = s->presence_penalty;
    sp.repeat_last_n = s->repeat_last_n;
    return mio::llm_debug_sample_chain(m, logits, history, n_history, sp, step, token, kept, cut_id, penalised);
}

extern "C" int mio_quantize_rows(uint32_t type, const float *x, int rows, int k, void *out) {
    MIO_REQUIRE(x && out && rows > 0 && k > 0, MIO_ERR_INVALID, "quantize_rows: bad args");
    const size_t rb = mio::ggml_row_bytes(type, k);
    MIO_REQUIRE(rb, MIO_ERR_UNSUPPORTED, "quantize_rows: type %u / k %d", type, k);
    for (int r = 0; r < rows; ++r)
        if (!mio::quantize_row(type, x + (size_t)r * k, (uint8_t *)out + r * rb, k)) return MIO_ERR_UNSUPPORTED;
    return MIO_OK;
}

extern "C" int mio_dequantize_rows(uint32_t type, const void *rows_bytes, int rows, int k, float *out) {
    MIO_REQUIRE(rows_bytes && out && rows > 0 && k > 0, MIO_ERR_INVALID, "dequantize_rows: bad args");
    const size_t rb = mio::ggml_row_bytes(type, k);
    MIO_REQUIRE(rb, MIO_ERR_UNSUPPORTED, "dequantize_rows: type %u / k %d", type, k);
    for (int r = 0; r < rows; ++r)
        if (!mio::dequantize_row(type, (const uint8_t *)rows_bytes + r * rb, out + (size_t)r * k, k))
            return MIO_ERR_UNSUPPORTED;
    return MIO_OK;
}
```

### miotts-llama.cpp_amd/csrc/testlib/debug_kernels.hip

```cpp
#include "llm_device.h"

#pragma clang fp contract(off)

namespace mio {
namespace {
template <int NP, int T>
__global__ __launch_bounds__(MT) void k_debug_matvec(QMat W, const float *x, float *y) {
    extern __shared__ __attribute__((aligned(16))) char smem[];
    const int K = W.k;
    const Smem s = carve(smem, K);
    XRegs<NP> xr;
    load_x(x, nullptr, K, xr);
    int lo, hi;
    wave_range(W.rows, lo, hi, blockIdx.x, gridDim.x);
    Frag ga[Cfg<NP>::U], gb[Cfg<NP>::U];
    load_first<T, NP, 1>(W, W, lo, hi, ga, gb);
    plain_quant(xr, K, akind(T), s);
    stream_rows<T, NP, 1>(W, W, lo, hi, ga, gb, s.a, [&](int row, float v, float) {
        if ((threadIdx.x & 63) == 0) y[row] = v;
    });
}
}

void launch_debug_matvec(const QMat &W, const float *x, float *y, int n_wg, hipStream_t s) {
    LlmDims d{};
    d.n_wg = n_wg;
    dispatch_nt(W.k, W.type, [&]<int NP, int T>() {
        hipLaunchKernelGGL((k_debug_matvec<NP, T>), dim3(matvec_grid(d, W.rows)), dim3(MT), matvec_lds(W.k), s, W, x,
                           y);
    });
}

}
```

### miotts-llama.cpp_amd/python/miotts_amd/__init__.py

```python
from __future__ import annotations

import ctypes
import os
from typing import Optional

import numpy as np

PKG_ROOT = os.path.dirname(os.path.dirname(os.path.dirname(os.path.abspath(__file__))))
REPO_ROOT = os.path.dirname(PKG_ROOT)
BUILD_DIR = os.environ.get("MIO_BUILD_DIR") or os.path.join(PKG_ROOT, "build")
LIB_PATH = os.path.join(BUILD_DIR, "libmiotts.so")
TEST_LIB_PATH = os.path.join(BUILD_DIR, "libmiotts_test.so")
INCLUDE_DIR = os.path.join(REPO_ROOT, "include")

MIO_IN_DEVICE = 1
MIO_OUT_DEVICE = 2
MIO_CODEC_INCREMENTAL = 4

_lib = None

_f32p = ctypes.POINTER(ctypes.c_float)
_i32p = ctypes.POINTER(ctypes.c_int32)
_vp = ctypes.c_void_p


class HipError(RuntimeError):
    pass


class Sampling(ctypes.Structure):
    _fields_ = [("top_k", ctypes.c_int32), ("top_p", ctypes.c_float), ("min_p", ctypes.c_float),
                ("repeat_penalty", ctypes.c_float), ("frequency_penalty", ctypes.c_float),
                ("presence_penalty", ctypes.c_float), ("repeat_last_n", ctypes.c_int32)]

    def __init__(self, top_k=0, top_p=1.0, min_p=0.0, repeat_penalty=1.0, frequency_penalty=0.0,
                 presence_penalty=0.0, repeat_last_n=64):
        super().__init__(top_k, top_p, min_p, repeat_penalty, frequency_penalty, presence_penalty, repeat_last_n)

    def as_dict(self) -> dict:
        return {k: getattr(self, k) for k, _ in self._fields_}


class _Libs:

    def __init__(self, product: ctypes.CDLL, test: Optional[ctypes.CDLL]):
        self.product, self.test = product, test

    def __getattr__(self, name):
        f = getattr(self.product, name, None)
        if f is None and self.test is not None:
            f = getattr(self.test, name, None)
        if f is None:
            raise AttributeError(name)
        return f


def lib() -> _Libs:
    global _lib
    if _lib is None:
        if not os.path.exists(LIB_PATH):
            raise ImportError(
                f"{LIB_PATH} not built: run `make -C miotts-llama.cpp_amd` "
                "(or __graft_entry__.build()); there is no CPU fallback")
        L = ctypes.CDLL(LIB_PATH, mode=ctypes.RTLD_GLOBAL)
        T = ctypes.CDLL(TEST_LIB_PATH, mode=ctypes.RTLD_GLOBAL) if os.path.exists(TEST_LIB_PATH) else None
        _declare(L)
        if T is not None:
            _declare(T)
        _lib = _Libs(L, T)
    return _lib


def _declare(L: ctypes.CDLL) -> None:
    c_int, c_size = ctypes.c_int, ctypes.c_size_t
    sig = {
        "mio_hip_last_error": (ctypes.c_char_p, []),
        "mio_hip_device_count": (c_int, [ctypes.POINTER(c_int)]),
        "mio_hip_device_open": (c_int, [c_int, ctypes.POINTER(_vp)]),
        "mio_hip_device_close": (None, [_vp]),
        "mio_hip_device_sync": (c_int, [_vp]),
        "mio_hip_device_cu_count": (c_int, [_vp, ctypes.POINTER(c_int)]),
        "mio_hip_malloc": (c_int, [_vp, c_size, ctypes.POINTER(_vp)]),
        "mio_hip_free": (c_int, [_vp, _vp]),
        "mio_hip_memcpy_h2d": (c_int, [_vp, _vp, _vp, c_size]),
        "mio_hip_memcpy_d2h": (c_int, [_vp, _vp, _vp, c_size]),
        "mio_hip_memset": (c_int, [_vp, _vp, c_int, c_size]),
        "mio_hip_timer_mark": (c_int, [_vp, _vp, c_int]),
        "mio_hip_timer_elapsed": (c_int, [_vp, c_int, c_int, _f32p]),
        "mio_hip_pcm_finish": (c_int, [_vp, _vp, ctypes.c_int64, c_int, _vp, _f32p, _vp]),
        "mio_hip_pcm_normalize": (c_int, [_vp, _vp, ctypes.c_int64, _vp, _f32p, _vp]),
        "mio_hip_istft_create": (c_int, [_vp, c_int, c_int, ctypes.POINTER(_vp)]),
        "mio_hip_istft_destroy": (None, [_vp]),
        "mio_hip_istft_out_len": (c_int, [_vp, c_int, c_int, ctypes.POINTER(c_int)]),
        "mio_hip_istft_run": (c_int, [_vp, _vp, c_int, c_int, _vp, ctypes.POINTER(c_int),
                                      ctypes.c_uint, _vp]),
        "mio_hip_codec_load": (c_int, [_vp, ctypes.c_char_p, ctypes.POINTER(_vp)]),
        "mio_hip_codec_free": (None, [_vp]),
        "mio_hip_codec_info": (c_int, [_vp, _i32p]),
        "mio_hip_codec_decode": (c_int, [_vp, _vp, c_int, _vp, _vp, ctypes.POINTER(c_int),
                                         ctypes.c_uint, _vp]),
        "mio_hip_codec_decode_pcm": (c_int, [_vp, _vp, c_int, _vp, _vp, ctypes.POINTER(c_int),
                                             ctypes.c_uint, _vp]),
        "mio_hip_codec_decode_pcm_batch": (c_int, [_vp, _vp, _vp, c_int, _vp, _vp, _vp, ctypes.c_uint, _vp]),
        "mio_hip_codec_decode_stage": (c_int, [_vp, _vp, c_int, _vp, c_int, _vp,
                                               ctypes.POINTER(c_int), ctypes.POINTER(c_int)]),
        "mio_synth_codec_gguf": (c_int, [ctypes.c_char_p, c_int, ctypes.c_uint64]),
        "mio_synth_voice_gguf": (c_int, [ctypes.c_char_p, ctypes.c_uint64]),
        "mio_synth_llm_gguf": (c_int, [ctypes.c_char_p, c_int, ctypes.c_uint64]),
        "mio_hip_llm_load": (c_int, [_vp, ctypes.c_char_p, c_int, ctypes.POINTER(_vp)]),
        "mio_hip_llm_free": (None, [_vp]),
        "mio_normalize_tts_text": (c_int, [ctypes.c_char_p, _vp, c_int, ctypes.POINTER(c_int)]),
        "mio_parse_speech_tokens": (c_int, [ctypes.c_char_p, _vp, c_int, ctypes.POINTER(c_int)]),
        "mio_wav_encode": (c_int, [_vp, c_int, c_int, _vp, c_int, ctypes.POINTER(c_int)]),
        "mio_hip_llm_time_kernel": (c_int, [_vp, c_int, c_int, _f32p, ctypes.POINTER(ctypes.c_uint64)]),
        "mio_hip_llm_trace_kernel": (c_int, [_vp, c_int, _vp]),
        "mio_tokenizer_load": (c_int, [ctypes.c_char_p, ctypes.POINTER(_vp)]),
        "mio_stream_cadence": (c_int, [c_int, ctypes.POINTER(c_int), ctypes.POINTER(ctypes.c_int64)]),
        "mio_tokenizer_free": (None, [_vp]),
        "mio_tokenizer_info": (c_int, [_vp, ctypes.POINTER(c_int)]),
        "mio_tokenize": (c_int, [_vp, ctypes.c_char_p, c_int, c_int, _vp, c_int, ctypes.POINTER(c_int)]),
        "mio_token_piece": (c_int, [_vp, ctypes.c_int32, ctypes.c_char_p, c_int, ctypes.POINTER(c_int)]),
        "mio_hip_llm_timeline": (c_int, [_vp, _vp, c_int, ctypes.POINTER(c_int)]),
        "mio_hip_codec_last_timings": (c_int, [_vp, _f32p]),
        "mio_hip_codec_last_reused": (c_int, [_vp, ctypes.POINTER(c_int)]),
        "mio_hip_codec_last_flops": (c_int, [_vp, ctypes.POINTER(ctypes.c_double)]),
        "mio_hip_llm_load_ms": (c_int, [_vp, ctypes.POINTER(ctypes.c_double)]),
        "mio_hip_llm_steps_issued": (c_int, [_vp, ctypes.POINTER(c_int)]),
        "mio_hip_llm_tail": (c_int, [_vp, ctypes.POINTER(c_int), ctypes.POINTER(c_int), ctypes.POINTER(ctypes.c_float)]),
        "mio_hip_llm_step_kinds": (c_int, [_vp, _vp, c_int, ctypes.POINTER(c_int)]),
        "mio_hip_llm_conv_ring": (c_int, [_vp, c_int, _vp, c_int]),
        "mio_hip_llm_eval_layers": (c_int, [_vp, ctypes.c_int32, c_int, _vp, _vp]),
        "mio_hip_llm_kv_rows": (c_int, [_vp, c_int, c_int, _vp, _vp]),
        "mio_hip_llm_set_kv_rows": (c_int, [_vp, c_int, c_int, c_int, _vp, _vp]),
        "mio_hip_llm_debug_attention": (c_int, [_vp, c_int, c_int, c_int, _vp, _vp]),
        "mio_hip_llm_set_sampling": (c_int, [_vp, ctypes.POINTER(Sampling)]),
        "mio_hip_llm_get_sampling": (c_int, [_vp, ctypes.POINTER(Sampling)]),
        "mio_hip_llm_debug_sample_chain": (c_int, [_vp, _vp, _vp, c_int, ctypes.POINTER(Sampling), ctypes.c_float,
                                                   ctypes.c_uint64, c_int, ctypes.c_int32, ctypes.c_int32, _i32p,
                                                   _i32p, _i32p, _vp]),
        "mio_hip_debug_matvec": (c_int, [_vp, ctypes.c_uint32, _vp, c_int, c_int, _vp, _vp]),
        "mio_quantize_rows": (c_int, [ctypes.c_uint32, _vp, c_int, c_int, _vp]),
        "mio_dequantize_rows": (c_int, [ctypes.c_uint32, _vp, c_int, c_int, _vp]),
        "mio_hip_debug_mmq": (c_int, [_vp, ctypes.c_uint32, _vp, c_int, c_int, _vp, c_int, c_int, _vp, _vp]),
        "mio_hip_debug_codec_gemm": (c_int, [_vp, _vp, _vp, _vp, _vp, _vp, _vp, _vp, ctypes.POINTER(c_int)]),
        "mio_hip_debug_codec_conv": (c_int, [_vp, _vp, c_int, c_int, c_int, c_int, _vp, c_int, _vp, c_int, _vp, _vp,
                                             ctypes.POINTER(c_int)]),
        "mio_hip_debug_codec_rownorm": (c_int, [_vp, _vp, c_int, c_int, ctypes.c_float, c_int, _vp, _vp, c_int, _vp,
                                                ctypes.POINTER(c_int)]),
        "mio_hip_debug_codec_groupnorm": (c_int, [_vp, _vp, c_int, c_int, c_int, ctypes.c_float, _vp, _vp, _vp,
                                                  ctypes.POINTER(c_int)]),
        "mio_hip_debug_codec_band_attention": (c_int, [_vp, _vp, c_int, c_int, c_int, _vp, _vp,
                                                       ctypes.POINTER(c_int)]),
        "mio_hip_debug_codec_cond_gemv": (c_int, [_vp, _vp, _vp, _vp, c_int, c_int, c_int, _vp,
                                                  ctypes.POINTER(c_int)]),
        "mio_hip_debug_codec_embed": (c_int, [_vp, _vp, c_int, c_int, _vp, c_int, _vp, ctypes.POINTER(c_int)]),
        "mio_hip_llm_info": (c_int, [_vp, _i32p]),
        "mio_hip_llm_weight_bytes": (c_int, [_vp, ctypes.POINTER(ctypes.c_uint64)]),
        "mio_hip_llm_eval": (c_int, [_vp, ctypes.c_int32, c_int, _vp]),
        "mio_hip_llm_prefill": (c_int, [_vp, _vp, c_int, _vp]),
        "mio_hip_llm_logits": (c_int, [_vp, _vp]),
        "mio_hip_llm_generate": (c_int, [_vp, _vp, c_int, c_int, ctypes.c_float, ctypes.c_uint64,
                                         ctypes.c_int32, ctypes.c_int32, ctypes.c_int32,
                                         ctypes.c_int32, ctypes.c_int32, _vp,
                                         ctypes.POINTER(c_int)]),
        "mio_hip_llm_generate_batch": (c_int, [_vp, _vp, _vp, c_int, c_int, ctypes.c_float, _vp,
                                               ctypes.c_int32, ctypes.c_int32, ctypes.c_int32,
                                               ctypes.c_int32, ctypes.c_int32, _vp, _vp]),
    }
    for name, (res, args) in sig.items():
        fn = getattr(L, name, None)
        if fn is None:
            continue
        fn.restype = res
        fn.argtypes = args


def check(rc: int) -> None:
    if rc != 0:
        msg = lib().mio_hip_last_error()
        raise HipError(f"rc={rc}: {msg.decode() if msg else ''}")


def _ptr(a: np.ndarray) -> int:
    return a.ctypes.data


def device_count() -> int:
    n = ctypes.c_int(0)
    check(lib().mio_hip_device_count(ctypes.byref(n)))
    return n.value


class Device:

    def __init__(self, dev: int = 0):
        h = _vp()
        check(lib().mio_hip_device_open(dev, ctypes.byref(h)))
        self.h = h
        self.dev = dev

    def close(self) -> None:
        if self.h:
            lib().mio_hip_device_close(self.h)
            self.h = None

    def __del__(self):
        try:
            self.close()
        except Exception:
            pass

    def sync(self) -> None:
        check(lib().mio_hip_device_sync(self.h))

    def cu_count(self) -> int:
        n = ctypes.c_int(0)
        check(lib().mio_hip_device_cu_count(self.h, ctypes.byref(n)))
        return n.value

    def malloc(self, nbytes: int) -> int:
        p = _vp()
        check(lib().mio_hip_malloc(self.h, nbytes, ctypes.byref(p)))
        return p.value

    def free(self, p: int) -> None:
        check(lib().mio_hip_free(self.h, p))

    def upload(self, a: np.ndarray) -> "DeviceArray":
        a = np.ascontiguousarray(a)
        buf = DeviceArray(self, a.nbytes, a.dtype, a.shape)
        check(lib().mio_hip_memcpy_h2d(self.h, buf.ptr, _ptr(a), a.nbytes))
        return buf

    def empty(self, shape, dtype) -> "DeviceArray":
        dtype = np.dtype(dtype)
        n = int(np.prod(shape)) * dtype.itemsize
        return DeviceArray(self, n, dtype, tuple(shape) if not isinstance(shape, int) else (shape,))

    def mark(self, slot: int, stream: int = 0) -> None:
        check(lib().mio_hip_timer_mark(self.h, stream or None, slot))

    def elapsed_ms(self, a: int, b: int) -> float:
        ms = ctypes.c_float(0)
        check(lib().mio_hip_timer_elapsed(self.h, a, b, ctypes.byref(ms)))
        return ms.value


class DeviceArray:
    def __init__(self, dev: Device, nbytes: int, dtype, shape):
        self.dev = dev
        self.nbytes = nbytes
        self.dtype = np.dtype(dtype)
        self.shape = tuple(shape)
        self.ptr = dev.malloc(nbytes)

    def numpy(self) -> np.ndarray:
        out = np.empty(self.shape, self.dtype)
        if self.nbytes:
            check(lib().mio_hip_memcpy_d2h(self.dev.h, _ptr(out), self.ptr, self.nbytes))
        return out

    def free(self) -> None:
        if self.ptr:
            self.dev.free(self.ptr)
            self.ptr = 0

    def __del__(self):
        try:
            self.free()
        except Exception:
            pass


def pcm_finish(dev: "Device", samples: "DeviceArray", n: int, normalize: bool,
               out: Optional["DeviceArray"] = None):
    if out is None:
        out = dev.empty((max(n, 1),), np.int16)
    peak = ctypes.c_float(0)
    check(lib().mio_hip_pcm_finish(dev.h, samples.ptr if n else None, n, 1 if normalize else 0,
                                   out.ptr if n else None, ctypes.byref(peak), None))
    return out.numpy()[:n], peak.value


class Istft:

    def __init__(self, dev: Device, n_fft: int = 392, win_length: Optional[int] = None):
        self.dev = dev
        self.n_fft = n_fft
        self.win = n_fft if win_length is None else win_length
        h = _vp()
        check(lib().mio_hip_istft_create(dev.h, n_fft, self.win, ctypes.byref(h)))
        self.h = h

    def __del__(self):
        try:
            if self.h:
                lib().mio_hip_istft_destroy(self.h)
                self.h = None
        except Exception:
            pass

    def out_len(self, n_frames: int, hop: int) -> int:
        n = ctypes.c_int(0)
        check(lib().mio_hip_istft_out_len(self.h, n_frames, hop, ctypes.byref(n)))
        return n.value

    def __call__(self, spec: np.ndarray, hop: int = 98) -> np.ndarray:
        spec = np.ascontiguousarray(spec, dtype=np.float32)
        n_frames = spec.shape[0] if spec.size else 0
        out = np.empty(max(self.out_len(n_frames, hop), 1), np.float32)
        n = ctypes.c_int(0)
        check(lib().mio_hip_istft_run(self.h, _ptr(spec) if spec.size else None, n_frames, hop,
                                      _ptr(out), ctypes.byref(n), 0, None))
        return out[: n.value]

    def run_device(self, spec: DeviceArray, n_frames: int, hop: int, out: DeviceArray,
                   stream: int = 0) -> int:
        n = ctypes.c_int(0)
        check(lib().mio_hip_istft_run(self.h, spec.ptr, n_frames, hop, out.ptr, ctypes.byref(n),
                                      MIO_IN_DEVICE | MIO_OUT_DEVICE, stream or None))
        return n.value


def synth_codec(path: str, preset: int = 0, seed: int = 1) -> str:
    check(lib().mio_synth_codec_gguf(path.encode(), preset, seed))
    return path


def synth_voice(path: str, seed: int = 7) -> str:
    check(lib().mio_synth_voice_gguf(path.encode(), seed))
    return path


def read_voice(path: str) -> np.ndarray:
    from . import gguf_np
    g = gguf_np.GGUFReader(path)
    t = g.tensors[0]
    assert t.type == 0, "voice embedding must be F32"
    return t.array().astype(np.float32)


class Codec:

    def __init__(self, dev: Device, path: str):
        self.dev = dev
        h = _vp()
        check(lib().mio_hip_codec_load(dev.h, path.encode(), ctypes.byref(h)))
        self.h = h
        info = np.zeros(8, np.int32)
        check(lib().mio_hip_codec_info(h, info.ctypes.data_as(_i32p)))
        (self.sample_rate, self.n_fft, self.hop_length, self.samples_per_token, self.n_freq,
         self.up_stages, self.frames_per_code, self.n_codes) = [int(x) for x in info]

    def close(self):
        if self.h:
            lib().mio_hip_codec_free(self.h)
            self.h = None

    def __del__(self):
        try:
            self.close()
        except Exception:
            pass

    def decode(self, codes, emb) -> np.ndarray:
        codes = np.ascontiguousarray(codes, dtype=np.int32)
        emb = np.ascontiguousarray(emb, dtype=np.float32)
        out = np.empty((len(codes) * self.frames_per_code, self.n_freq, 2), np.float32)
        nf = ctypes.c_int(0)
        check(lib().mio_hip_codec_decode(self.h, _ptr(codes), len(codes), _ptr(emb), _ptr(out),
                                         ctypes.byref(nf), 0, None))
        return out[: nf.value]

    def decode_pcm(self, codes, emb, incremental: bool = False) -> np.ndarray:
        codes = np.ascontiguousarray(codes, dtype=np.int32)
        emb = np.ascontiguousarray(emb, dtype=np.float32)
        out = np.empty(len(codes) * self.frames_per_code * self.hop_length + self.n_fft, np.float32)
        n = ctypes.c_int(0)
        check(lib().mio_hip_codec_decode_pcm(self.h, _ptr(codes), len(codes), _ptr(emb), _ptr(out),
                                             ctypes.byref(n), MIO_CODEC_INCREMENTAL if incremental else 0, None))
        return out[: n.value]

    def last_reused(self) -> int:
        r = ctypes.c_int(0)
        check(lib().mio_hip_codec_last_reused(self.h, ctypes.byref(r)))
        return r.value

    def last_flops(self) -> float:
        f = ctypes.c_double(0)
        check(lib().mio_hip_codec_last_flops(self.h, ctypes.byref(f)))
        return f.value

    def decode_pcm_device(self, codes: DeviceArray, n_codes: int, emb: DeviceArray,
                          out: DeviceArray, stream: int = 0) -> int:
        n = ctypes.c_int(0)
        check(lib().mio_hip_codec_decode_pcm(self.h, codes.ptr, n_codes, emb.ptr, out.ptr,
                                             ctypes.byref(n), MIO_IN_DEVICE | MIO_OUT_DEVICE,
                                             stream or None))
        return n.value

    def decode_pcm_batch_device(self, codes, n_codes, emb: DeviceArray, outs, stream: int = 0):
        B = len(codes)
        cp = (ctypes.c_void_p * B)(*[c.ptr for c in codes])
        op = (ctypes.c_void_p * B)(*[o.ptr for o in outs])
        nc = (ctypes.c_int * B)(*[int(n) for n in n_codes])
        ln = (ctypes.c_int * B)()
        check(lib().mio_hip_codec_decode_pcm_batch(self.h, ctypes.cast(cp, _vp), ctypes.cast(nc, _vp), B, emb.ptr,
                                                   ctypes.cast(op, _vp), ctypes.cast(ln, _vp),
                                                   MIO_IN_DEVICE | MIO_OUT_DEVICE, stream or None))
        return [int(x) for x in ln]

    def decode_pcm_batch(self, codes, emb, host: bool = False):
        dev = self.dev
        if host:
            B = len(codes)
            hc = [np.ascontiguousarray(c, np.int32) for c in codes]
            he = np.ascontiguousarray(emb, np.float32)
            ho = [np.empty(len(c) * self.samples_per_token + self.n_fft, np.float32) for c in hc]
            cp = (ctypes.c_void_p * B)(*[_ptr(c) for c in hc])
            op = (ctypes.c_void_p * B)(*[_ptr(o) for o in ho])
            nc = (ctypes.c_int * B)(*[len(c) for c in hc])
            ln = (ctypes.c_int * B)()
            check(lib().mio_hip_codec_decode_pcm_batch(self.h, ctypes.cast(cp, _vp), ctypes.cast(nc, _vp), B, _ptr(he),
                                                       ctypes.cast(op, _vp), ctypes.cast(ln, _vp), 0, None))
            return [o[:int(n)] for o, n in zip(ho, ln)]
        d_codes = [dev.upload(np.ascontiguousarray(c, np.int32)) for c in codes]
        d_emb = dev.upload(np.ascontiguousarray(emb, np.float32))
        outs = [dev.empty((len(c) * self.samples_per_token + self.n_fft,), np.float32) for c in codes]
        lens = self.decode_pcm_batch_device(d_codes, [len(c) for c in codes], d_emb, outs)
        dev.sync()
        return [o.numpy()[:n] for o, n in zip(outs, lens)]

    def last_timings(self):
        ms = np.zeros(2, np.float32)
        check(lib().mio_hip_codec_last_timings(self.h, ms.ctypes.data_as(_f32p)))
        return float(ms[0]), float(ms[1])

    def decode_stage(self, codes, emb, stage: int, max_elems: int) -> np.ndarray:
        codes = np.ascontiguousarray(codes, dtype=np.int32)
        emb = np.ascontiguousarray(emb, dtype=np.float32)
        out = np.empty(max_elems, np.float32)
        r, c = ctypes.c_int(0), ctypes.c_int(0)
        check(lib().mio_hip_codec_decode_stage(self.h, _ptr(codes), len(codes), _ptr(emb), stage,
                                               _ptr(out), ctypes.byref(r), ctypes.byref(c)))
        return out[: r.value * c.value].reshape(r.value, c.value)


SYNTH_SPEECH0 = 260
SYNTH_IM_END = 258
SYNTH_EOT = 259
STEP_KIND_NAMES = {0: "attn_in", 1: "attention", 2: "attn_out", 3: "ffn_in", 4: "ffn_down", 6: "lm_head",
                   7: "sample", 8: "conv_in", 9: "conv_out", 10: "att_o", 11: "layer_att", 12: "ffn", 13: "layer",
                   14: "sample_chain"}


def synth_llm(path: str, preset: int = 0, seed: int = 1) -> str:
    check(lib().mio_synth_llm_gguf(path.encode(), preset, seed))
    return path


class Llm:

    def __init__(self, dev: Device, path: str, n_ctx: int = 2048):
        self.dev = dev
        h = _vp()
        check(lib().mio_hip_llm_load(dev.h, path.encode(), n_ctx, ctypes.byref(h)))
        self.h = h
        info = np.zeros(8, np.int32)
        check(lib().mio_hip_llm_info(h, info.ctypes.data_as(_i32p)))
        (self.n_vocab, self.n_embd, self.n_layer, self.n_head, self.n_kv, self.head_dim,
         self.n_ff, self.n_ctx) = [int(x) for x in info]

    def close(self):
        if self.h:
            lib().mio_hip_llm_free(self.h)
            self.h = None

    def __del__(self):
        try:
            self.close()
        except Exception:
            pass

    def weight_bytes(self) -> int:
        b = ctypes.c_uint64(0)
        check(lib().mio_hip_llm_weight_bytes(self.h, ctypes.byref(b)))
        return b.value

    def load_ms(self) -> float:
        v = ctypes.c_double(0)
        check(lib().mio_hip_llm_load_ms(self.h, ctypes.byref(v)))
        return v.value

    def steps_issued(self) -> int:
        v = ctypes.c_int(0)
        check(lib().mio_hip_llm_steps_issued(self.h, ctypes.byref(v)))
        return v.value

    def tail(self):
        a, b, ms = ctypes.c_int(0), ctypes.c_int(0), ctypes.c_float(0)
        check(lib().mio_hip_llm_tail(self.h, ctypes.byref(a), ctypes.byref(b), ctypes.byref(ms)))
        return a.value, b.value, ms.value

    def eval(self, token: int, pos: int) -> np.ndarray:
        out = np.empty(self.n_vocab, np.float32)
        check(lib().mio_hip_llm_eval(self.h, token, pos, _ptr(out)))
        return out

    def prefill(self, tokens) -> np.ndarray:
        t = np.ascontiguousarray(tokens, np.int32)
        out = np.empty(self.n_vocab, np.float32)
        check(lib().mio_hip_llm_prefill(self.h, _ptr(t), int(t.size), _ptr(out)))
        return out

    def logits(self) -> np.ndarray:
        out = np.empty(self.n_vocab, np.float32)
        check(lib().mio_hip_llm_logits(self.h, _ptr(out)))
        return out

    def time_kernel(self, which: int, iters: int = 50):
        ms = ctypes.c_float(0)
        b = ctypes.c_uint64(0)
        check(lib().mio_hip_llm_time_kernel(self.h, which, iters, ctypes.byref(ms), ctypes.byref(b)))
        return ms.value, b.value

    def trace_kernel(self, which: int) -> np.ndarray:
        out = np.zeros(32, np.uint64)
        check(lib().mio_hip_llm_trace_kernel(self.h, which, _ptr(out)))
        return out

    def timeline(self) -> np.ndarray:
        slots = 2048
        out = np.zeros(256 * slots * 8, np.uint64)
        n = ctypes.c_int(0)
        check(lib().mio_hip_llm_timeline(self.h, _ptr(out), 256, ctypes.byref(n)))
        t = out[: n.value * slots * 8].astype(np.float64).reshape(n.value, slots, 8)
        t[t == 0] = np.nan
        return (t - np.nanmin(t[0, :, 0])) * 0.01

    def eval_layers(self, token: int, pos: int):
        xs = np.empty((self.n_layer + 1, self.n_embd), np.float32)
        lg = np.empty(self.n_vocab, np.float32)
        check(lib().mio_hip_llm_eval_layers(self.h, token, pos, _ptr(xs), _ptr(lg)))
        return xs, lg

    def kv_rows(self, il: int, n_pos: int):
        k = np.empty((self.n_kv, n_pos, self.head_dim), np.float16)
        v = np.empty_like(k)
        check(lib().mio_hip_llm_kv_rows(self.h, il, n_pos, _ptr(k), _ptr(v)))
        return k, v

    def set_kv_rows(self, il: int, p0: int, k: np.ndarray, v: np.ndarray) -> None:
        k = np.ascontiguousarray(k, np.float16)
        v = np.ascontiguousarray(v, np.float16)
        assert k.shape == v.shape and k.ndim == 3 and k.shape[0] == self.n_kv and k.shape[2] == self.head_dim, k.shape
        check(lib().mio_hip_llm_set_kv_rows(self.h, il, p0, k.shape[1], _ptr(k), _ptr(v)))

    def debug_attention(self, il: int, pos: int, which: int, qkv: np.ndarray) -> np.ndarray:
        qkv = np.ascontiguousarray(qkv, np.float32).reshape(-1)
        assert qkv.size == (self.n_head + 2 * self.n_kv) * self.head_dim, qkv.size
        att = np.empty((self.n_head, self.head_dim), np.float32)
        check(lib().mio_hip_llm_debug_attention(self.h, il, pos, which, _ptr(qkv), _ptr(att)))
        return att

    def set_sampling(self, sampling=None, **knobs) -> None:
        assert sampling is None or not knobs
        s = Sampling(**knobs) if knobs else sampling
        check(lib().mio_hip_llm_set_sampling(self.h, ctypes.byref(s) if s is not None else None))

    def get_sampling(self) -> dict:
        s = Sampling()
        check(lib().mio_hip_llm_get_sampling(self.h, ctypes.byref(s)))
        return s.as_dict()

    def debug_sample_chain(self, logits, history, sampling: Sampling, temperature: float, seed: int, step: int,
                           lo: int, hi: int, penalised: bool = False):
        logits = np.ascontiguousarray(logits, np.float32).reshape(-1)
        assert logits.size == self.n_vocab, logits.size
        history = np.ascontiguousarray(history, np.int32).reshape(-1)
        tok, kept, cut = ctypes.c_int32(0), ctypes.c_int32(0), ctypes.c_int32(0)
        pen = np.empty(self.n_vocab, np.float32) if penalised else None
        check(lib().mio_hip_llm_debug_sample_chain(self.h, _ptr(logits), _ptr(history) if history.size else None,
                                                   history.size, ctypes.byref(sampling), temperature, seed, step, lo,
                                                   hi, ctypes.byref(tok), ctypes.byref(kept), ctypes.byref(cut),
                                                   _ptr(pen) if penalised else None))
        return (tok.value, kept.value, cut.value, pen) if penalised else (tok.value, kept.value, cut.value)

    def step_kinds(self) -> list:
        n = ctypes.c_int(0)
        check(lib().mio_hip_llm_step_kinds(self.h, None, 0, ctypes.byref(n)))
        k = np.zeros(n.value, np.int32)
        check(lib().mio_hip_llm_step_kinds(self.h, _ptr(k), n.value, ctypes.byref(n)))
        return [int(v) for v in k]

    def conv_ring(self, il: int, ring=None):
        if ring is None:
            r = np.empty((4, self.n_embd), np.float32)
            check(lib().mio_hip_llm_conv_ring(self.h, il, _ptr(r), 0))
            return r
        r = np.ascontiguousarray(ring, np.float32)
        check(lib().mio_hip_llm_conv_ring(self.h, il, _ptr(r), 1))

    def generate(self, prompt, max_tokens: int, temperature: float = 0.8, seed: int = 42,
                 allow=(-1, -1), eos=(-1, -1), check_interval: int = 20) -> np.ndarray:
        prompt = np.ascontiguousarray(prompt, dtype=np.int32)
        out = np.empty(max_tokens, np.int32)
        n = ctypes.c_int(0)
        check(lib().mio_hip_llm_generate(self.h, _ptr(prompt), len(prompt), max_tokens,
                                         temperature, seed, allow[0], allow[1], eos[0], eos[1],
                                         check_interval, _ptr(out), ctypes.byref(n)))
        return out[: n.value]

    def generate_batch(self, prompts, max_tokens: int, temperature: float = 0.8, seeds=None,
                       allow=(-1, -1), eos=(-1, -1), check_interval: int = 32):
        B = len(prompts)
        seeds = [42 + b for b in range(B)] if seeds is None else list(seeds)
        lens = np.array([len(p) for p in prompts], np.int32)
        flat = np.ascontiguousarray(np.concatenate([np.asarray(p, np.int32) for p in prompts]), np.int32)
        sd = np.array(seeds, np.uint64)
        out = np.empty((B, max_tokens), np.int32)
        n = np.zeros(B, np.int32)
        check(lib().mio_hip_llm_generate_batch(self.h, _ptr(flat), _ptr(lens), B, max_tokens, temperature,
                                               _ptr(sd), allow[0], allow[1], eos[0], eos[1],
                                               check_interval, _ptr(out), _ptr(n)))
        return [out[b, : n[b]].copy() for b in range(B)]


GGML_BLOCK = {2: (32, 18), 6: (32, 22), 8: (32, 34), 12: (256, 144), 13: (256, 176), 14: (256, 210),
              30: (1, 2)}


def quantize_rows(qtype: int, x: np.ndarray) -> np.ndarray:
    x = np.ascontiguousarray(x, dtype=np.float32)
    rows, k = x.shape
    be, bb = GGML_BLOCK[qtype]
    out = np.zeros((rows, k // be * bb), np.uint8)
    check(lib().mio_quantize_rows(qtype, _ptr(x), rows, k, _ptr(out)))
    return out


def dequantize_rows(qtype: int, rows_bytes: np.ndarray, k: int) -> np.ndarray:
    rows_bytes = np.ascontiguousarray(rows_bytes, dtype=np.uint8)
    be, bb = GGML_BLOCK[qtype]
    assert rows_bytes.ndim == 2 and rows_bytes.shape[1] == k // be * bb, rows_bytes.shape
    out = np.empty((rows_bytes.shape[0], k), np.float32)
    check(lib().mio_dequantize_rows(qtype, _ptr(rows_bytes), rows_bytes.shape[0], k, _ptr(out)))
    return out


def debug_matvec(dev: Device, qtype: int, w_rows: np.ndarray, k: int, x: np.ndarray) -> np.ndarray:
    w_rows = np.ascontiguousarray(w_rows)
    x = np.ascontiguousarray(x, dtype=np.float32)
    y = np.empty(w_rows.shape[0], np.float32)
    check(lib().mio_hip_debug_matvec(dev.h, qtype, _ptr(w_rows), w_rows.shape[0], k, _ptr(x), _ptr(y)))
    return y


def debug_mmq(dev: Device, qtype: int, w_rows: np.ndarray, k: int, x: np.ndarray, mode: int = 0,
              y_in: Optional[np.ndarray] = None, up_rows: Optional[np.ndarray] = None) -> np.ndarray:
    w_rows = np.ascontiguousarray(w_rows)
    x = np.ascontiguousarray(x, dtype=np.float32)
    y = np.zeros((x.shape[0], w_rows.shape[0]), np.float32) if y_in is None else np.array(y_in, np.float32)
    up = np.ascontiguousarray(up_rows) if up_rows is not None else None
    check(lib().mio_hip_debug_mmq(dev.h, qtype, _ptr(w_rows), w_rows.shape[0], k, _ptr(x), x.shape[0], mode,
                                  _ptr(up) if up is not None else None, _ptr(y)))
    return y


SENTINEL_F32 = 0x7FC5A5A5
SENTINEL_F16 = 0x7E5A
EPI_STORE, EPI_RESID, EPI_GATED, EPI_SWIGLU, EPI_CONVT, EPI_CONVT_SNAKE, EPI_SNAKE, EPI_HEAD = range(8)


class _DebugGemm(ctypes.Structure):
    _fields_ = [(n, ctypes.c_int) for n in ("a_seg", "a_row_off", "a_rows", "M", "N", "K", "ldc", "c_rows", "f", "trim",
                                            "cout", "rows_out", "m_major", "a_f16", "epi", "kg")]


def sentinel_f32(shape) -> np.ndarray:
    return np.full(shape, SENTINEL_F32, np.uint32).view(np.float32)


def _opt_f32(a):
    return None if a is None else np.ascontiguousarray(a, dtype=np.float32)


def debug_codec_gemm(dev: Device, A: np.ndarray, B: np.ndarray, C: np.ndarray, M: int, epi: int = EPI_STORE,
                     kg: int = 0, a_row_off: int = 0, bias=None, aux=None, aux2=None, f: int = 0, trim: int = 0,
                     cout: int = 0, rows_out: int = 0, a_f16: int = 0, m_major: int = 0):
    A = np.ascontiguousarray(A, dtype=np.float32)
    B = np.ascontiguousarray(B, dtype=np.float32)
    C = np.array(C, dtype=np.float32, order="C")
    bias, aux, aux2 = _opt_f32(bias), _opt_f32(aux), _opt_f32(aux2)
    g = _DebugGemm(a_seg=A.shape[1], a_row_off=a_row_off, a_rows=A.shape[0], M=M, N=B.shape[0], K=B.shape[1],
                   ldc=C.shape[1], c_rows=C.shape[0], f=f, trim=trim, cout=cout, rows_out=rows_out, m_major=m_major,
                   a_f16=a_f16, epi=epi, kg=kg)
    ok = ctypes.c_int(0)
    check(lib().mio_hip_debug_codec_gemm(dev.h, ctypes.addressof(g), _ptr(A), _ptr(B), _ptr(C),
                                         None if bias is None else _ptr(bias), None if aux is None else _ptr(aux),
                                         None if aux2 is None else _ptr(aux2), ctypes.byref(ok)))
    return C, bool(ok.value)


def debug_codec_conv(dev: Device, xa: np.ndarray, w: np.ndarray, bias: np.ndarray, taps: int, pad: int,
                     resid=None, alias: bool = False):
    xa = np.ascontiguousarray(xa, dtype=np.float16)
    w = np.ascontiguousarray(w, dtype=np.float16)
    bias = np.ascontiguousarray(bias, dtype=np.float32)
    L, Cin = xa.shape
    Cout = w.shape[0]
    assert w.shape[1] == taps * Cin and (resid is not None or not alias)
    resid = _opt_f32(resid)
    y = resid.copy() if alias else np.empty((L, Cout), np.float32)
    mode = 0 if resid is None else (2 if alias else 1)
    ok = ctypes.c_int(0)
    check(lib().mio_hip_debug_codec_conv(dev.h, _ptr(xa), L, Cin, taps, pad, _ptr(w), Cout, _ptr(bias), mode,
                                         _ptr(resid) if mode == 1 else None, _ptr(y), ctypes.byref(ok)))
    return y, bool(ok.value)


def debug_codec_rownorm(dev: Device, x: np.ndarray, eps: float, mode: int = 0, p0=None, p1=None,
                        in_place: bool = False):
    x = np.ascontiguousarray(x, dtype=np.float32)
    p0, p1 = _opt_f32(p0), _opt_f32(p1)
    y = np.empty_like(x)
    ok = ctypes.c_int(0)
    check(lib().mio_hip_debug_codec_rownorm(dev.h, _ptr(x), x.shape[0], x.shape[1], eps, mode,
                                            None if p0 is None else _ptr(p0), None if p1 is None else _ptr(p1),
                                            int(in_place), _ptr(y), ctypes.byref(ok)))
    return y, bool(ok.value)


def debug_codec_groupnorm(dev: Device, x: np.ndarray, G: int, eps: float, gamma: np.ndarray, beta: np.ndarray):
    x = np.ascontiguousarray(x, dtype=np.float32)
    gamma = np.ascontiguousarray(gamma, dtype=np.float32)
    beta = np.ascontiguousarray(beta, dtype=np.float32)
    xa = np.empty(x.shape, np.uint16)
    ok = ctypes.c_int(0)
    check(lib().mio_hip_debug_codec_groupnorm(dev.h, _ptr(x), x.shape[0], x.shape[1], G, eps, _ptr(gamma),
                                              _ptr(beta), _ptr(xa), ctypes.byref(ok)))
    return xa.view(np.float16), bool(ok.value)


def debug_codec_band_attention(dev: Device, qkv: np.ndarray, H: int, window: int, rope: np.ndarray):
    qkv = np.ascontiguousarray(qkv, dtype=np.float32)
    rope = np.ascontiguousarray(rope, dtype=np.float32)
    S = qkv.shape[0]
    assert qkv.shape[1] == 3 * H * 64 and rope.shape == (S, 32, 2)
    out = np.empty((S, H * 64), np.float32)
    ok = ctypes.c_int(0)
    check(lib().mio_hip_debug_codec_band_attention(dev.h, _ptr(qkv), S, H, window, _ptr(rope), _ptr(out),
                                                   ctypes.byref(ok)))
    return out, bool(ok.value)


def debug_codec_cond_gemv(dev: Device, W: np.ndarray, b: np.ndarray, e: np.ndarray, e_f16: int = 0):
    W = np.ascontiguousarray(W, dtype=np.float32)
    b = np.ascontiguousarray(b, dtype=np.float32)
    e = np.ascontiguousarray(e, dtype=np.float32)
    y = np.empty(W.shape[0], np.float32)
    ok = ctypes.c_int(0)
    check(lib().mio_hip_debug_codec_cond_gemv(dev.h, _ptr(W), _ptr(b), _ptr(e), W.shape[0], W.shape[1], e_f16,
                                              _ptr(y), ctypes.byref(ok)))
    return y, bool(ok.value)


def debug_codec_embed(dev: Device, table: np.ndarray, codes):
    table = np.ascontiguousarray(table, dtype=np.float32)
    codes = np.ascontiguousarray(codes, dtype=np.int32)
    x = np.empty((len(codes), table.shape[1]), np.float32)
    ok = ctypes.c_int(0)
    check(lib().mio_hip_debug_codec_embed(dev.h, _ptr(table), table.shape[0], table.shape[1], _ptr(codes),
                                          len(codes), _ptr(x), ctypes.byref(ok)))
    return x, bool(ok.value)


class Tokenizer:

    def __init__(self, gguf_path: str):
        h = _vp()
        check(lib().mio_tokenizer_load(gguf_path.encode(), ctypes.byref(h)))
        self.h = h
        info = (ctypes.c_int * 4)()
        check(lib().mio_tokenizer_info(self.h, info))
        self.n_vocab, self.bos, self.eos, self.im_end = list(info)

    def __del__(self):
        if getattr(self, "h", None):
            lib().mio_tokenizer_free(self.h)
            self.h = None

    def tokenize(self, text: str, add_special: bool = True, parse_special: bool = True) -> list:
        b = text.encode("utf-8")
        cap = len(b) + 16
        out = np.zeros(cap, np.int32)
        n = ctypes.c_int(0)
        check(lib().mio_tokenize(self.h, b, int(add_special), int(parse_special), _ptr(out), cap, ctypes.byref(n)))
        return out[: n.value].tolist()

    def piece(self, tok: int) -> bytes:
        cap = 1024
        buf = ctypes.create_string_buffer(cap)
        n = ctypes.c_int(0)
        check(lib().mio_token_piece(self.h, int(tok), buf, cap, ctypes.byref(n)))
        return buf.raw[: n.value]

    def detokenize(self, toks) -> str:
        return b"".join(self.piece(t) for t in toks).decode("utf-8", errors="replace")


def stream_cadence(n_tokens: int):
    c, k = ctypes.c_int(0), ctypes.c_int64(0)
    check(lib().mio_stream_cadence(int(n_tokens), ctypes.byref(c), ctypes.byref(k)))
    return c.value, k.value


def normalize_text(text: str) -> str:
    b = text.encode("utf-8")
    cap = 4 * len(b) + 16
    out = ctypes.create_string_buffer(cap)
    n = ctypes.c_int(0)
    check(lib().mio_normalize_tts_text(b, out, cap, ctypes.byref(n)))
    return out.raw[: n.value].decode("utf-8")


def parse_speech_tokens(text: str) -> np.ndarray:
    b = text.encode("utf-8")
    n = ctypes.c_int(0)
    check(lib().mio_parse_speech_tokens(b, None, 0, ctypes.byref(n)))
    out = np.zeros(max(n.value, 1), np.int32)
    check(lib().mio_parse_speech_tokens(b, _ptr(out), len(out), ctypes.byref(n)))
    return out[: n.value]


def wav_bytes(samples: np.ndarray, sample_rate: int = 44100) -> bytes:
    s = np.ascontiguousarray(samples, dtype=np.float32)
    cap = 44 + 2 * len(s)
    out = np.zeros(cap, np.uint8)
    n = ctypes.c_int(0)
    check(lib().mio_wav_encode(_ptr(s) if len(s) else None, len(s), sample_rate, _ptr(out), cap,
                               ctypes.byref(n)))
    return out[: n.value].tobytes()
```

Measured before the change: 54.71 x realtime (audio s / wall s).

## Spread matvec row epilogues across lanes and restructure q8_K activation quantization

Adds a stream_rows_lanes wrapper that buffers each produced row value in a per-lane register. Each batch of 64 rows is then written by 64 lanes at once, instead of lane 0 issuing one scalar store per row with a readlane for the residual. The q8_K activation quantizer is rewritten to find the wave max with an integer DPP reduction and to quantize and pack all register fragments in one pass. A power-of-two mean is also computed with ldexp. The intent is to cut serialized epilogue stores and quantize overhead in the decode matvecs, at the cost of extra register state and more complex tail handling. Debug and test entry points for swiglu matvec and activation quantization are added alongside.

New measurement: 57.60 x realtime (audio s / wall s), median of 6. 1.05x the previous value.

```diff
diff --git a/miotts-llama.cpp_amd/csrc/hip/llm_attention.h b/miotts-llama.cpp_amd/csrc/hip/llm_attention.h
--- a/miotts-llama.cpp_amd/csrc/hip/llm_attention.h
+++ b/miotts-llama.cpp_amd/csrc/hip/llm_attention.h
@@ -172,14 +172,11 @@
     MIO_TL_MARK1(b);
     plain_quant(xr, K, akind(T), s, MIO_TL_DIAGSLOT(b));
     MIO_TL_MARK(b, 2);
-    stream_rows<T, NP, 1, SU, MIO_SMALL_AUX>(wo, wo, lo, hi, ga, gb, s.a, [&](int row, float v, float) {
-        const float r = lane_value(xres, row - lo);
-        if ((threadIdx.x & 63) == 0) {
-            if constexpr (XS)
-                st1_sc1(b.x, (uint32_t)row * 4u, v + r);
-            else
-                b.x[row] = v + r;
-        }
+    stream_rows_lanes<T, NP, 1, SU, MIO_SMALL_AUX>(wo, wo, lo, hi, ga, gb, s.a, [&](int row, float v, float) {
+        if constexpr (XS)
+            st1_sc1(b.x, (uint32_t)row * 4u, v + xres);
+        else
+            b.x[row] = v + xres;
     });
     if constexpr (XS) {
         asm volatile("s_waitcnt vmcnt(0)" ::: "memory");
diff --git a/miotts-llama.cpp_amd/csrc/hip/llm_attn_in.hip b/miotts-llama.cpp_amd/csrc/hip/llm_attn_in.hip
--- a/miotts-llama.cpp_amd/csrc/hip/llm_attn_in.hip
+++ b/miotts-llama.cpp_amd/csrc/hip/llm_attn_in.hip
@@ -55,9 +55,7 @@
         }
         return false;
     };
-    auto put = [&](int row, float v) {
-        if ((threadIdx.x & 63) == 0) b.qkv[row] = v;
-    };
+    auto put = [&](int row, float v) { b.qkv[row] = v; };
     Frag ga[Cfg<NP, SU>::U], gb[Cfg<NP, SU>::U];
     int lo, hi;
     if ((int)blockIdx.x < g_qk) {
@@ -71,7 +69,7 @@
         rmsnorm_quant(xr, K, d.eps, akind(TQ), s, MIO_TL_DIAGSLOT(b));
         MIO_TRACE(b, 2);
         MIO_TL_MARK(b, 2);
-        stream_rows<TQ, NP, 1, SU, MIO_SMALL_AUX>(wq, wk, lo, hi, ga, gb, s.a, [&](int row, float v, float) {
+        stream_rows_lanes<TQ, NP, 1, SU, MIO_SMALL_AUX>(wq, wk, lo, hi, ga, gb, s.a, [&](int row, float v, float) {
             put(row, v);
         }, o1);
         MIO_TL_END(b);
@@ -84,7 +82,7 @@
         x_after_weights(xr);
         if (!FS && done_now(dn)) return;
         rmsnorm_quant(xr, K, d.eps, akind(TV), s, MIO_TL_DIAGSLOT(b));
-        stream_rows<TV, NP, 1, SU, MIO_SMALL_AUX>(wv, wv, lo, hi, ga, gb, s.a, [&](int row, float v, float) {
+        stream_rows_lanes<TV, NP, 1, SU, MIO_SMALL_AUX>(wv, wv, lo, hi, ga, gb, s.a, [&](int row, float v, float) {
             put(o2 + row, v);
         });
         MIO_TL_END(b);
diff --git a/miotts-llama.cpp_amd/csrc/hip/llm_device.h b/miotts-llama.cpp_amd/csrc/hip/llm_device.h
--- a/miotts-llama.cpp_amd/csrc/hip/llm_device.h
+++ b/miotts-llama.cpp_amd/csrc/hip/llm_device.h
@@ -228,6 +228,63 @@
     return wave_max_f(fmaxf(fmaxf(fabsf(v[0]), fabsf(v[1])), fmaxf(fabsf(v[2]), fabsf(v[3]))), 0.0f);
 }
 
+__device__ __forceinline__ uint32_t wave_max_u(uint32_t v) {
+    v = max(v, (uint32_t)__builtin_amdgcn_update_dpp(0, (int)v, ROW_SHR1, 0xF, 0xF, false));
+    v = max(v, (uint32_t)__builtin_amdgcn_update_dpp(0, (int)v, ROW_SHR2, 0xF, 0xF, false));
+    v = max(v, (uint32_t)__builtin_amdgcn_update_dpp(0, (int)v, ROW_SHR4, 0xF, 0xF, false));
+    v = max(v, (uint32_t)__builtin_amdgcn_update_dpp(0, (int)v, ROW_SHR8, 0xF, 0xF, false));
+    v = max(v, (uint32_t)__builtin_amdgcn_update_dpp(0, (int)v, ROW_BCAST15, 0xA, 0xF, false));
+    v = max(v, (uint32_t)__builtin_amdgcn_update_dpp(0, (int)v, ROW_BCAST31, 0xC, 0xF, false));
+    return (uint32_t)__builtin_amdgcn_readlane((int)v, 63);
+}
+
+template <int XV>
+__device__ __forceinline__ void q8k_regs(const float4 (&v)[XV], int K, const ActL &a) {
+    const int lane = MIO_TIDX & 63, wave = __builtin_amdgcn_readfirstlane(MIO_TIDX >> 6);
+    const int nsb = K >> 8;
+    float mx[XV];
+#pragma unroll
+    for (int j = 0; j < XV; ++j) {
+        const float vv[4] = {v[j].x, v[j].y, v[j].z, v[j].w};
+        const float m = fmaxf(fmaxf(fabsf(vv[0]), fabsf(vv[1])), fmaxf(fabsf(vv[2]), fabsf(vv[3])));
+        const float am = __uint_as_float(wave_max_u(m == m ? __float_as_uint(m) : 0u));
+        float sel = 0.0f;
+        bool has = false;
+#pragma unroll
+        for (int i = 3; i >= 0; --i)
+            if (fabsf(vv[i]) == am) sel = vv[i], has = true;
+        const int src = __builtin_ctzll(__ballot(has) | (1ull << 63));
+        mx[j] = __int_as_float(__builtin_amdgcn_readlane(__float_as_int(sel), src));
+    }
+    float mxl = mx[0];
+#pragma unroll
+    for (int j = 1; j < XV; ++j) mxl = lane == j ? mx[j] : mxl;
+    const float isl = -127.f / mxl;
+#pragma unroll
+    for (int j = 0; j < XV; ++j) {
+        const int b = wave + MW * j;
+        const float is = XV == 1 ? isl : __int_as_float(__builtin_amdgcn_readlane(__float_as_int(isl), j));
+        const float iscale = fabsf(mx[j]) > 0.0f ? is : 0.0f;
+        const float vv[4] = {v[j].x, v[j].y, v[j].z, v[j].w};
+        int q[4];
+#pragma unroll
+        for (int i = 0; i < 4; ++i) {
+            const int t = (int)rintf(iscale * vv[i]);
+            q[i] = t < 127 ? t : 127;
+        }
+        const uint32_t p01 = __builtin_amdgcn_perm((uint32_t)q[1], (uint32_t)q[0], 0x0c0c0400u);
+        const uint32_t p23 = __builtin_amdgcn_perm((uint32_t)q[3], (uint32_t)q[2], 0x0c0c0400u);
+        const int packed = (int)__builtin_amdgcn_perm(p23, p01, 0x05040100u);
+        const int sm = quad_sum_i(sdot4(packed, 0x01010101, 0));
+        if (b < nsb) {
+            *reinterpret_cast<int *>(a.qs + b * 256 + 4 * lane) = packed;
+            if ((lane & 3) == 0) a.bs[b * 16 + (lane >> 2)] = (int16_t)sm;
+        }
+    }
+    const float dd = fabsf(mxl) > 0.0f ? 1.0f / isl : 0.0f;
+    if (lane < XV && wave + MW * lane < nsb) a.d[wave + MW * lane] = dd;
+}
+
 __device__ __forceinline__ void q80_store(const float (&v)[4], int b, bool ok, const ActL &a) {
     const int lane = MIO_TIDX & 63;
     float am = 0.0f;
@@ -297,14 +354,7 @@
 __device__ __forceinline__ void quant_regs(const float4 (&v)[XV], int K, int ak, const ActL &a) {
     const int lane = MIO_TIDX & 63, wave = __builtin_amdgcn_readfirstlane(MIO_TIDX >> 6);
     if (ak == 1) {
-        const int nsb = K >> 8;
-#pragma unroll
-        for (int j = 0; j < XV; ++j) {
-            const int b = wave + MW * j;
-            if (b >= nsb) break;
-            const float vv[4] = {v[j].x, v[j].y, v[j].z, v[j].w};
-            q8k_store(vv, abs_max4(vv), b, a);
-        }
+        q8k_regs<XV>(v, K, a);
     } else if (ak == 2) {
 #pragma unroll
         for (int j = 0; j < XV; ++j) {
@@ -327,7 +377,7 @@
 }
 
 __device__ __forceinline__ float rms_scale(double tot, int K, float eps) {
-    const float mean = (float)((K & (K - 1)) == 0 ? tot * (1.0 / K) : tot / K);
+    const float mean = (float)((K & (K - 1)) == 0 ? __builtin_ldexp(tot, -__builtin_ctz(K)) : tot / K);
     return 1.0f / sqrtf(mean + eps);
 }
 
@@ -794,6 +844,30 @@
     }
 }
 
+template <int T, int NP, int NM, int SU = 0, int AUX = MIO_WEIGHT_AUX, class Fin>
+__device__ __forceinline__ void stream_rows_lanes(const QMat W0, const QMat W1, int lo, int hi,
+                                                  Frag (&A)[Cfg<NP, SU>::U], Frag (&B)[Cfg<NP, SU>::U], const ActL &a,
+                                                  Fin &&fin, int split = INT_MAX, unsigned long long *trace = nullptr) {
+    const int lane = MIO_TIDX & 63;
+    if constexpr (SU != 0 && SU / (NM * NP) == 1) {
+        stream_rows<T, NP, NM, SU, AUX>(W0, W1, lo, hi, A, B, a, [&](int row, float v0, float v1) {
+            if (lane == 0) fin(row, v0, v1);
+        }, split, trace);
+        return;
+    }
+    float p0 = 0.0f, p1 = 0.0f;
+    stream_rows<T, NP, NM, SU, AUX>(W0, W1, lo, hi, A, B, a, [&](int row, float v0, float v1) {
+        const int k = (row - lo) & 63;
+        p0 = lane == k ? v0 : p0;
+        if constexpr (NM == 2) p1 = lane == k ? v1 : p1;
+        if constexpr (SU == 0) {
+            if (k == 63) fin(row - 63 + lane, p0, p1);
+        }
+    }, split, trace);
+    const int rest = SU == 0 ? (hi - lo) & 63 : hi - lo;
+    if (lane < rest) fin(hi - rest + lane, p0, p1);
+}
+
 template <int T, int NP, int NM, int SU = 0, int AUX = MIO_WEIGHT_AUX>
 __device__ __forceinline__ void load_first(const QMat W0, const QMat W1, int lo, int hi, Frag (&A)[Cfg<NP, SU>::U],
                                            Frag (&B)[Cfg<NP, SU>::U], int split = INT_MAX) {
diff --git a/miotts-llama.cpp_amd/csrc/hip/llm_kernels.h b/miotts-llama.cpp_amd/csrc/hip/llm_kernels.h
--- a/miotts-llama.cpp_amd/csrc/hip/llm_kernels.h
+++ b/miotts-llama.cpp_amd/csrc/hip/llm_kernels.h
@@ -215,7 +215,10 @@
 int pick_su(int units, int np);
 void launch_attn_in(const LlmDims &d, const LayerW &L, int il, const QMat &tok_embd, const LlmBuffers &b, bool dg,
                     hipStream_t s);
-void launch_debug_matvec(const QMat &W, const float *x, float *y, int n_wg, hipStream_t s);
+void launch_debug_matvec(const QMat &W, const QMat *up, const float *x, float *y, int n_wg, hipStream_t s);
+size_t debug_act_record_bytes(int K);
+void launch_debug_act_quant(int type, const float *x, const float *w, int K, float eps, bool sc1, void *out,
+                            hipStream_t s);
 size_t debug_act_bytes(int K);
 void launch_debug_mmq(const QMat &W, const QMat &up, int mode, const float *x, int nt, char *act, float *y,
                       hipStream_t s);
diff --git a/miotts-llama.cpp_amd/csrc/hip/llm_kernels.hip b/miotts-llama.cpp_amd/csrc/hip/llm_kernels.hip
--- a/miotts-llama.cpp_amd/csrc/hip/llm_kernels.hip
+++ b/miotts-llama.cpp_amd/csrc/hip/llm_kernels.hip
@@ -34,9 +34,8 @@
     plain_quant(xr, K, akind(T), s, MIO_TL_DIAGSLOT(b));
     MIO_TRACE(b, 2);
     MIO_TL_MARK(b, 2);
-    stream_rows<T, NP, 1, SU, MIO_SMALL_AUX>(wo, wo, lo, hi, ga, gb, s.a, [&](int row, float v, float) {
-        const float r = lane_value(xres, row - lo);
-        if ((threadIdx.x & 63) == 0) b.x[row] = v + r;
+    stream_rows_lanes<T, NP, 1, SU, MIO_SMALL_AUX>(wo, wo, lo, hi, ga, gb, s.a, [&](int row, float v, float) {
+        b.x[row] = v + xres;
     });
     MIO_TL_END(b);
     MIO_TRACE(b, 15);
@@ -70,9 +69,8 @@
                MIO_TL_DIAGSLOT(b));
     MIO_TRACE(b, 2);
     MIO_TL_MARK(b, 2);
-    stream_rows<T, NP, 1, SU>(wo, wo, lo, hi, ga, gb, s.a, [&](int row, float v, float) {
-        const float r = lane_value(xres, row - lo);
-        if ((threadIdx.x & 63) == 0) b.x[row] = v + r;
+    stream_rows_lanes<T, NP, 1, SU>(wo, wo, lo, hi, ga, gb, s.a, [&](int row, float v, float) {
+        b.x[row] = v + xres;
     });
     MIO_TL_END(b);
     MIO_TRACE(b, 15);
@@ -130,8 +128,8 @@
     rmsnorm_quant(xr, K, d.eps, akind(T), s, MIO_TL_DIAGSLOT(b));
     MIO_TRACE(b, 2);
     MIO_TL_MARK(b, 2);
-    stream_rows<T, NP, 2, SU>(gate, up, lo, hi, ga, gb, s.a, [&](int row, float g, float u) {
-        if ((threadIdx.x & 63) == 0) b.h[row] = silu_f(g) * u;
+    stream_rows_lanes<T, NP, 2, SU>(gate, up, lo, hi, ga, gb, s.a, [&](int row, float g, float u) {
+        b.h[row] = silu_f(g) * u;
     }, INT_MAX, DG ? b.trace : nullptr);
     if (adv && blockIdx.x == 0 && MIO_TIDX == 0) advance_state(b.st, d);
     MIO_TL_END(b);
@@ -162,9 +160,8 @@
     plain_quant(xr, K, akind(T), s, MIO_TL_DIAGSLOT(b));
     MIO_TRACE(b, 2);
     MIO_TL_MARK(b, 2);
-    stream_rows<T, NP, 1, SU>(down, down, lo, hi, ga, gb, s.a, [&](int row, float v, float) {
-        const float r = lane_value(xres, row - lo);
-        if ((threadIdx.x & 63) == 0) b.x[row] = v + r;
+    stream_rows_lanes<T, NP, 1, SU>(down, down, lo, hi, ga, gb, s.a, [&](int row, float v, float) {
+        b.x[row] = v + xres;
     }, INT_MAX, DG ? b.trace : nullptr);
     MIO_TL_END(b);
     MIO_TRACE(b, 15);
@@ -202,8 +199,8 @@
         MIO_TL_MARK1(b);
         rmsnorm_quant(xr, K, d.eps, akind(T), s, MIO_TL_DIAGSLOT(b));
         MIO_TL_MARK(b, 2);
-        stream_rows<T, NP, 2, SU>(gate, up, lo, hi, ga, gb, s.a, [&](int row, float g, float u) {
-            if ((threadIdx.x & 63) == 0) st1_sc1(b.h, (uint32_t)row * 4u, silu_f(g) * u);
+        stream_rows_lanes<T, NP, 2, SU>(gate, up, lo, hi, ga, gb, s.a, [&](int row, float g, float u) {
+            st1_sc1(b.h, (uint32_t)row * 4u, silu_f(g) * u);
         });
         if (adv && blockIdx.x == 0 && MIO_TIDX == 0) advance_state(b.st, d);
         asm volatile("s_waitcnt vmcnt(0)" ::: "memory");
@@ -240,9 +237,8 @@
         MIO_TL_MARK1(b);
         plain_quant(xr, K, akind(TD), s, MIO_TL_DIAGSLOT(b));
         MIO_TL_MARK(b, 2);
-        stream_rows<TD, NPD, 1, SUD>(down, down, lo, hi, ga, gb, s.a, [&](int row, float v, float) {
-            const float r = lane_value(xres, row - lo);
-            if ((threadIdx.x & 63) == 0) b.x[row] = v + r;
+        stream_rows_lanes<TD, NPD, 1, SUD>(down, down, lo, hi, ga, gb, s.a, [&](int row, float v, float) {
+            b.x[row] = v + xres;
         });
     }
     MIO_TL_END(b);
diff --git a/miotts-llama.cpp_amd/csrc/hip/llm_layer_att.hip b/miotts-llama.cpp_amd/csrc/hip/llm_layer_att.hip
--- a/miotts-llama.cpp_amd/csrc/hip/llm_layer_att.hip
+++ b/miotts-llama.cpp_amd/csrc/hip/llm_layer_att.hip
@@ -18,9 +18,7 @@
     XRegs<NP> xr;
     load_x(b.x, norm_w, K, xr);
     x_gate();
-    auto put = [&](int row, float v) {
-        if ((threadIdx.x & 63) == 0) st1_sc1(b.qkv, (uint32_t)row * 4, v);
-    };
+    auto put = [&](int row, float v) { st1_sc1(b.qkv, (uint32_t)row * 4, v); };
     Frag ga[Cfg<NP, SU>::U], gb[Cfg<NP, SU>::U];
     int lo, hi, ra, rb;
     const int bid = blockIdx.x;
@@ -33,7 +31,7 @@
         MIO_TL_MARK1(b);
         rmsnorm_quant(xr, K, d.eps, akind(TQ), s, MIO_TL_DIAGSLOT(b));
         MIO_TL_MARK(b, 2);
-        stream_rows<TQ, NP, 1, SU, MIO_SMALL_AUX>(wq, wk, lo, hi, ga, gb, s.a, [&](int row, float v, float) {
+        stream_rows_lanes<TQ, NP, 1, SU, MIO_SMALL_AUX>(wq, wk, lo, hi, ga, gb, s.a, [&](int row, float v, float) {
             put(row, v);
         }, o1);
     } else {
@@ -46,7 +44,7 @@
         MIO_TL_MARK1(b);
         rmsnorm_quant(xr, K, d.eps, akind(TV), s, MIO_TL_DIAGSLOT(b));
         MIO_TL_MARK(b, 2);
-        stream_rows<TV, NP, 1, SU, MIO_SMALL_AUX>(wv, wv, lo, hi, ga, gb, s.a, [&](int row, float v, float) {
+        stream_rows_lanes<TV, NP, 1, SU, MIO_SMALL_AUX>(wv, wv, lo, hi, ga, gb, s.a, [&](int row, float v, float) {
             put(o2 + row, v);
         });
     }
@@ -131,8 +129,8 @@
     MIO_TL_MARK1(b);
     rmsnorm_quant(xr, K, d.eps, akind(T), s, MIO_TL_DIAGSLOT(b));
     MIO_TL_MARK(b, 2);
-    stream_rows<T, NP, 2, SU>(gate, up, lo, hi, ga, gb, s.a, [&](int row, float g, float u) {
-        if ((threadIdx.x & 63) == 0) st1_sc1(b.h, (uint32_t)row * 4u, silu_f(g) * u);
+    stream_rows_lanes<T, NP, 2, SU>(gate, up, lo, hi, ga, gb, s.a, [&](int row, float g, float u) {
+        st1_sc1(b.h, (uint32_t)row * 4u, silu_f(g) * u);
     });
     asm volatile("s_waitcnt vmcnt(0)" ::: "memory");
     __syncthreads();
@@ -167,9 +165,8 @@
     MIO_TL_MARK1(b);
     plain_quant(xr, K, akind(T), s, MIO_TL_DIAGSLOT(b));
     MIO_TL_MARK(b, 2);
-    stream_rows<T, NP, 1, SU>(down, down, lo, hi, ga, gb, s.a, [&](int row, float v, float) {
-        const float rr = lane_value(xres, row - lo);
-        if ((threadIdx.x & 63) == 0) b.x[row] = v + rr;
+    stream_rows_lanes<T, NP, 1, SU>(down, down, lo, hi, ga, gb, s.a, [&](int row, float v, float) {
+        b.x[row] = v + xres;
     });
 }
 
diff --git a/miotts-llama.cpp_amd/csrc/testlib/debug_capi.cpp b/miotts-llama.cpp_amd/csrc/testlib/debug_capi.cpp
--- a/miotts-llama.cpp_amd/csrc/testlib/debug_capi.cpp
+++ b/miotts-llama.cpp_amd/csrc/testlib/debug_capi.cpp
@@ -1,3 +1,4 @@
+#include <cstring>
 #include <vector>
 
 #include "common.h"
@@ -7,11 +8,12 @@
 #include "mio_hip_test.h"
 #include "quant.h"
 
-extern "C" int mio_hip_debug_matvec(mio_hip_device *d, uint32_t type, const void *gguf_rows, int rows, int k,
-                                    const float *x, float *y) {
+namespace {
+int debug_matvec(mio_hip_device *d, uint32_t type, const void *gguf_rows, const void *gguf_up, int rows, int k,
+                 const float *x, float *y) {
     MIO_REQUIRE(d && gguf_rows && x && y && rows > 0 && k > 0, MIO_ERR_INVALID, "debug_matvec: bad args");
     MIO_REQUIRE(type == mio::GGML_Q8_0 || type == mio::GGML_Q4_K || type == mio::GGML_Q5_K ||
-                    type == mio::GGML_Q6_K || type == mio::GGML_BF16 || mio::repacks_to_q8_0(type),
+                    type == mio::GGML_Q6_K || type == mio::GGML_BF16 || (!gguf_up && mio::repacks_to_q8_0(type)),
                 MIO_ERR_UNSUPPORTED, "debug_matvec: type %u", type);
     const bool k32 = type == mio::GGML_Q8_0 || type == mio::GGML_BF16 || mio::repacks_to_q8_0(type);
     MIO_REQUIRE(k % (k32 ? 32 : 256) == 0, MIO_ERR_INVALID, "debug_matvec: k %d", k);
@@ -25,21 +27,68 @@
         type = mio::GGML_Q8_0;
     }
     const mio::SplitLayout L = mio::split_layout(type, rows, k);
-    std::vector<uint8_t> host(L.bytes);
+    const int nm = gguf_up ? 2 : 1;
+    std::vector<uint8_t> host(L.bytes * nm);
     mio::to_split(type, gguf_rows, rows, k, host.data());
+    if (gguf_up) mio::to_split(type, gguf_up, rows, k, host.data() + L.bytes);
     uint8_t *dw = nullptr;
     float *dx = nullptr, *dy = nullptr;
-    MIO_HIP_CHECK(hipMalloc(&dw, L.bytes));
+    MIO_HIP_CHECK(hipMalloc(&dw, L.bytes * nm));
     MIO_HIP_CHECK(hipMalloc(&dx, (size_t)k * 4));
     MIO_HIP_CHECK(hipMalloc(&dy, (size_t)rows * 4));
-    hipMemcpy(dw, host.data(), L.bytes, hipMemcpyHostToDevice);
+    hipMemcpy(dw, host.data(), L.bytes * nm, hipMemcpyHostToDevice);
     hipMemcpy(dx, x, (size_t)k * 4, hipMemcpyHostToDevice);
-    mio::QMat q{(int)type, rows, k, dw + L.off[0], dw + L.off[1], dw + L.off[2], dw + L.off[3]};
-    mio::launch_debug_matvec(q, dx, dy, d->n_cu > 0 ? d->n_cu : 256, d->stream);
+    auto qm = [&](uint8_t *base) {
+        return mio::QMat{(int)type, rows, k, base + L.off[0], base + L.off[1], base + L.off[2], base + L.off[3]};
+    };
+    const mio::QMat q = qm(dw), up = qm(dw + (gguf_up ? L.bytes : 0));
+    mio::launch_debug_matvec(q, gguf_up ? &up : nullptr, dx, dy, d->n_cu > 0 ? d->n_cu : 256, d->stream);
     hipError_t e = hipStreamSynchronize(d->stream);
     if (e == hipSuccess) e = hipMemcpy(y, dy, (size_t)rows * 4, hipMemcpyDeviceToHost);
     hipFree(dw), hipFree(dx), hipFree(dy);
     MIO_HIP_CHECK(e);
+    return MIO_OK;
+}
+}
+
+extern "C" int mio_hip_debug_matvec(mio_hip_device *d, uint32_t type, const void *gguf_rows, int rows, int k,
+                                    const float *x, float *y) {
+    return debug_matvec(d, type, gguf_rows, nullptr, rows, k, x, y);
+}
+
+extern "C" int mio_hip_debug_matvec_swiglu(mio_hip_device *d, uint32_t type, const void *gguf_gate,
+                                           const void *gguf_up, int rows, int k, const float *x, float *y) {
+    MIO_REQUIRE(gguf_up, MIO_ERR_INVALID, "debug_matvec_swiglu: bad args");
+    return debug_matvec(d, type, gguf_gate, gguf_up, rows, k, x, y);
+}
+
+extern "C" int mio_hip_debug_act_quant(mio_hip_device *d, uint32_t type, const float *x, const float *w, int k,
+                                       float eps, int sc1, int8_t *qs, float *dd, int16_t *bs) {
+    MIO_REQUIRE(d && x && qs && dd && bs && k > 0, MIO_ERR_INVALID, "debug_act_quant: bad args");
+    MIO_REQUIRE(type == mio::GGML_Q8_0 || type == mio::GGML_Q4_K || type == mio::GGML_BF16, MIO_ERR_UNSUPPORTED,
+                "debug_act_quant: type %u", type);
+    MIO_REQUIRE(k % (type == mio::GGML_Q4_K ? 256 : 32) == 0 && k <= 12288, MIO_ERR_INVALID,
+                "debug_act_quant: k %d", k);
+    int rc = mio::bind(d);
+    if (rc) return rc;
+    const size_t nb = mio::debug_act_record_bytes(k);
+    float *dx = nullptr, *dw = nullptr;
+    char *dr = nullptr;
+    MIO_HIP_CHECK(hipMalloc(&dx, (size_t)k * 4));
+    MIO_HIP_CHECK(hipMalloc(&dw, (size_t)k * 4));
+    MIO_HIP_CHECK(hipMalloc(&dr, nb));
+    hipMemcpy(dx, x, (size_t)k * 4, hipMemcpyHostToDevice);
+    if (w) hipMemcpy(dw, w, (size_t)k * 4, hipMemcpyHostToDevice);
+    mio::launch_debug_act_quant((int)type, dx, w ? dw : nullptr, k, eps, sc1 != 0, dr, d->stream);
+    hipError_t e = hipGetLastError();
+    if (e == hipSuccess) e = hipStreamSynchronize(d->stream);
+    std::vector<char> rec(nb);
+    if (e == hipSuccess) e = hipMemcpy(rec.data(), dr, nb, hipMemcpyDeviceToHost);
+    hipFree(dx), hipFree(dw), hipFree(dr);
+    MIO_HIP_CHECK(e);
+    memcpy(qs, rec.data(), (size_t)k * 2);
+    memcpy(dd, rec.data() + (size_t)k * 2, (size_t)(k / 32 + 8) * 4);
+    memcpy(bs, rec.data() + (size_t)k * 2 + (size_t)(k / 32 + 8) * 4, (size_t)(k / 16 + 8) * 2);
     return MIO_OK;
 }
 
diff --git a/miotts-llama.cpp_amd/csrc/testlib/debug_kernels.hip b/miotts-llama.cpp_amd/csrc/testlib/debug_kernels.hip
--- a/miotts-llama.cpp_amd/csrc/testlib/debug_kernels.hip
+++ b/miotts-llama.cpp_amd/csrc/testlib/debug_kernels.hip
@@ -4,8 +4,8 @@
 
 namespace mio {
 namespace {
-template <int NP, int T>
-__global__ __launch_bounds__(MT) void k_debug_matvec(QMat W, const float *x, float *y) {
+template <int NP, int T, int NM>
+__global__ __launch_bounds__(MT) void k_debug_matvec(QMat W, QMat U, const float *x, float *y) {
     extern __shared__ __attribute__((aligned(16))) char smem[];
     const int K = W.k;
     const Smem s = carve(smem, K);
@@ -14,20 +14,53 @@
     int lo, hi;
     wave_range(W.rows, lo, hi, blockIdx.x, gridDim.x);
     Frag ga[Cfg<NP>::U], gb[Cfg<NP>::U];
-    load_first<T, NP, 1>(W, W, lo, hi, ga, gb);
+    load_first<T, NP, NM>(W, U, lo, hi, ga, gb);
     plain_quant(xr, K, akind(T), s);
-    stream_rows<T, NP, 1>(W, W, lo, hi, ga, gb, s.a, [&](int row, float v, float) {
-        if ((threadIdx.x & 63) == 0) y[row] = v;
+    stream_rows_lanes<T, NP, NM>(W, U, lo, hi, ga, gb, s.a, [&](int row, float v, float u) {
+        y[row] = NM == 2 ? silu_f(v) * u : v;
     });
+}
+
+template <int NP, int T, int XAUX>
+__global__ __launch_bounds__(MT) void k_debug_act_quant(const float *x, const float *w, int K, float eps,
+                                                        uint32_t *out) {
+    extern __shared__ __attribute__((aligned(16))) char smem[];
+    const Smem s = carve(smem, K);
+    XRegs<NP> xr;
+    load_x<NP, XAUX>(x, w, K, xr);
+    if (w)
+        rmsnorm_quant(xr, K, eps, akind(T), s);
+    else
+        plain_quant(xr, K, akind(T), s);
+    const int n = (int)((smem_bytes(K) - 128) / 4);
+    for (int i = MIO_TIDX; i < n; i += MT) out[i] = reinterpret_cast<const uint32_t *>(smem)[i];
 }
 }
 
-void launch_debug_matvec(const QMat &W, const float *x, float *y, int n_wg, hipStream_t s) {
+size_t debug_act_record_bytes(int K) { return smem_bytes(K) - 128; }
+
+void launch_debug_act_quant(int type, const float *x, const float *w, int K, float eps, bool sc1, void *out,
+                            hipStream_t s) {
+    dispatch_nt(K, type, [&]<int NP, int T>() {
+        if (sc1)
+            hipLaunchKernelGGL((k_debug_act_quant<NP, T, 16>), dim3(1), dim3(MT), matvec_lds(K), s, x, w, K, eps,
+                               (uint32_t *)out);
+        else
+            hipLaunchKernelGGL((k_debug_act_quant<NP, T, 0>), dim3(1), dim3(MT), matvec_lds(K), s, x, w, K, eps,
+                               (uint32_t *)out);
+    });
+}
+
+void launch_debug_matvec(const QMat &W, const QMat *up, const float *x, float *y, int n_wg, hipStream_t s) {
     LlmDims d{};
     d.n_wg = n_wg;
     dispatch_nt(W.k, W.type, [&]<int NP, int T>() {
-        hipLaunchKernelGGL((k_debug_matvec<NP, T>), dim3(matvec_grid(d, W.rows)), dim3(MT), matvec_lds(W.k), s, W, x,
-                           y);
+        if (up)
+            hipLaunchKernelGGL((k_debug_matvec<NP, T, 2>), dim3(matvec_grid(d, W.rows)), dim3(MT), matvec_lds(W.k), s,
+                               W, *up, x, y);
+        else
+            hipLaunchKernelGGL((k_debug_matvec<NP, T, 1>), dim3(matvec_grid(d, W.rows)), dim3(MT), matvec_lds(W.k), s,
+                               W, W, x, y);
     });
 }
 
diff --git a/miotts-llama.cpp_amd/python/miotts_amd/__init__.py b/miotts-llama.cpp_amd/python/miotts_amd/__init__.py
--- a/miotts-llama.cpp_amd/python/miotts_amd/__init__.py
+++ b/miotts-llama.cpp_amd/python/miotts_amd/__init__.py
@@ -139,6 +139,9 @@
                                                    ctypes.c_uint64, c_int, ctypes.c_int32, ctypes.c_int32, _i32p,
                                                    _i32p, _i32p, _vp]),
         "mio_hip_debug_matvec": (c_int, [_vp, ctypes.c_uint32, _vp, c_int, c_int, _vp, _vp]),
+        "mio_hip_debug_matvec_swiglu": (c_int, [_vp, ctypes.c_uint32, _vp, _vp, c_int, c_int, _vp, _vp]),
+        "mio_hip_debug_act_quant": (c_int, [_vp, ctypes.c_uint32, _vp, _vp, c_int, ctypes.c_float, c_int, _vp, _vp,
+                                            _vp]),
         "mio_quantize_rows": (c_int, [ctypes.c_uint32, _vp, c_int, c_int, _vp]),
         "mio_dequantize_rows": (c_int, [ctypes.c_uint32, _vp, c_int, c_int, _vp]),
         "mio_hip_debug_mmq": (c_int, [_vp, ctypes.c_uint32, _vp, c_int, c_int, _vp, c_int, c_int, _vp, _vp]),
@@ -656,6 +659,27 @@
     return y
 
 
+def debug_matvec_swiglu(dev: Device, qtype: int, gate_rows: np.ndarray, up_rows: np.ndarray, k: int,
+                        x: np.ndarray) -> np.ndarray:
+    gate_rows, up_rows = np.ascontiguousarray(gate_rows), np.ascontiguousarray(up_rows)
+    x = np.ascontiguousarray(x, dtype=np.float32)
+    y = np.empty(gate_rows.shape[0], np.float32)
+    check(lib().mio_hip_debug_matvec_swiglu(dev.h, qtype, _ptr(gate_rows), _ptr(up_rows), gate_rows.shape[0], k,
+                                            _ptr(x), _ptr(y)))
+    return y
+
+
+def debug_act_quant(dev: Device, qtype: int, x: np.ndarray, w: Optional[np.ndarray] = None, eps: float = 1e-6,
+                    sc1: bool = False):
+    x = np.ascontiguousarray(x, dtype=np.float32)
+    k = x.shape[0]
+    wv = np.ascontiguousarray(w, dtype=np.float32) if w is not None else None
+    qs, d, bs = np.empty(2 * k, np.int8), np.empty(k // 32 + 8, np.float32), np.empty(k // 16 + 8, np.int16)
+    check(lib().mio_hip_debug_act_quant(dev.h, qtype, _ptr(x), _ptr(wv) if wv is not None else None, k, eps,
+                                        int(sc1), _ptr(qs), _ptr(d), _ptr(bs)))
+    return qs, d, bs
+
+
 def debug_mmq(dev: Device, qtype: int, w_rows: np.ndarray, k: int, x: np.ndarray, mode: int = 0,
               y_in: Optional[np.ndarray] = None, up_rows: Optional[np.ndarray] = None) -> np.ndarray:
     w_rows = np.ascontiguousarray(w_rows)
```
